# xxxupeng/stereo_toolbox

Hardware: AMD Instinct MI355X
Metric: stereo pairs/sec @ 540x960 D=192 (GwcNet_GC fwd+bwd) (higher is better)
Workload: dtype f32; 1 GPU; GwcNet_GC(maxdisp=192) train step: fwd+bwd+allreduce+Adam, 576x960 pairs (reference pad_to_2x shape), batch 1/GPU, fp32, synthetic randn inputs, deterministic filler weights; global_batch=1, parallelism=dp1, grad_sync=none (single rank: flat fp32 buffer packed, no collective), launch=eager, optimizer=torch.optim.Adam(fused=True)

## Files before the change

include/stx_hip.h:

```cpp
#ifndef STX_HIP_H
#define STX_HIP_H
#ifdef __cplusplus
extern "C" {
#endif

const char* stx_last_error(void);
const char* stx_build_info(void);
int stx_get_tuning(const char* name);
int stx_set_tuning(const char* name, int value);

int stx_cost_volume_fwd(const float* Lg, const float* Rg, int Cg, int G, const float* Lc, const float* Rc, int Cc,
                        const float* scale, float* vol, int B, int H, int W, int D, int mask_left, void* stream);
int stx_group_normalize_fwd(const float* x, float* y, int B, int C, int G, int HW, float out_scale, void* stream);
int stx_group_normalize_bwd(const float* x, const float* gy, float* gx, int B, int C, int G, int HW, float out_scale, void* stream);
int stx_cost_volume_bwd(const float* gvol, const float* Lg, const float* Rg, int Cg, int G, int Cc, float* gLg,
                        float* gRg, float* gLc, float* gRc, int B, int H, int W, int D, int mask_left, void* stream);

int stx_head_fwd(const float* cost, float* disp, float* stats, int B, int Dc, int Hc, int Wc, int D, int H, int W,
                 void* stream);
long long stx_head_bwd_workspace_floats(int B, int Dc, int H, int W);
int stx_head_bwd(const float* gdisp, const float* cost, const float* disp, const float* stats, float* gcost,
                 float* workspace, int B, int Dc, int Hc, int Wc, int D, int H, int W, void* stream);
int stx_head_fwd2(const float* cost, float* disp, float* stats, int B, int Dc, int Hc, int Wc, int D, int H, int W,
                  int align_corners, void* stream);
int stx_head_bwd2(const float* gdisp, const float* cost, const float* disp, const float* stats, float* gcost,
                  float* workspace, int B, int Dc, int Hc, int Wc, int D, int H, int W, int align_corners, void* stream);
int stx_softargmax_fwd(const float* x, float* out, int B, int D, int HW, void* stream);
int stx_argmax_fwd(const float* x, long long* out, int B, int D, int HW, void* stream);
int stx_unimodal_fwd(const float* x, float* out, int B, int D, int HW, void* stream);
int stx_dominant_modal_fwd(const float* x, float* out, int B, int D, int HW, void* stream);
int stx_modal_fwd(const float* x, float* out, float* aux, int B, int D, int HW, int kind, void* stream);
int stx_modal_bwd(const float* g, const float* out, const float* aux, float* gx, int B, int D, int HW, void* stream);
int stx_split_mode(const float* x, float* mode, unsigned char* mask, int B, int D, int HW, void* stream);
int stx_softmax_d_fwd(const float* x, float* y, int B, int D, int HW, void* stream);

long long stx_conv3d_packed_floats(int K, int N, int T);
int stx_conv3d_pack_weight(const float* w, float* wp, int A, int B, int T, int mode, void* stream);
int stx_conv3d_fwd_blocks(int Do, int Ho, int Wo);
long long stx_conv3d_fwd_stat_rows(int B, int Di, int Hi, int Wi, int Cin, int Cout, int ks, int stride);
int stx_conv3d_fwd(const float* x, const float* wp, float* out, const float* scale, const float* bias,
                   const float* residual, float* stats, int B, int Di, int Hi, int Wi, int Cin, int Cout, int ks,
                   int stride, int relu, void* stream);
int stx_deconv3d_fwd_blocks(int Di, int Hi, int Wi);
int stx_deconv3d_fwd(const float* x, const float* wp, float* out, const float* scale, const float* bias,
                     const float* residual, float* stats, int B, int Di, int Hi, int Wi, int Cin, int Cout, int Do,
                     int Ho, int Wo, int relu, void* stream);
long long stx_conv3d_wgrad_workspace_floats(int B, int Dc, int Hc, int Wc, int CF, int CC, int ks, int stride);
int stx_conv3d_wgrad(const float* fine, const float* coarse, float* dw, float* workspace, int B, int Df, int Hf, int Wf,
                     int CF, int Dc, int Hc, int Wc, int CC, int ks, int stride, void* stream);

int stx_conv3d_wgrad_bn_supported(int B, int D, int H, int W, int CF, int CC);
int stx_conv3d_wgrad_bn(const float* x, const float* gy, const float* z, const float* scale, const float* shift, const float* mean,
                        const float* invstd, const float* gamma, const float* sums, float inv_n, int act, float* dz, float* dw,
                        float* workspace, int B, int D, int H, int W, int CF, int CC, void* stream);

int stx_conv2d_supported(int Cin, int Cout);
long long stx_conv2d_stat_rows(int groups);
int stx_conv2d_fwd(const float* x, const float* w, float* out, float* stats, int B, int H, int W, int Cin, int Cout, int dgrad,
                   int groups, void* stream);

int stx_conv3d_c1_fwd(const float* x, const float* w, const float* residual, float* out, int B, int D, int H, int W,
                      int Cin, void* stream);
long long stx_conv3d_c1_wgrad_workspace_floats(int Cin);
int stx_conv3d_c1_wgrad(const float* x, const float* gy, float* dw, float* workspace, int B, int D, int H, int W,
                        int Cin, void* stream);
int stx_conv3d_c1_dgrad(const float* gy, const float* w, float* gx, int B, int D, int H, int W, int Cin, void* stream);

int stx_mish_fwd(const float* x, float* y, long long n, void* stream);
int stx_mish_bwd(const float* gy, const float* x, float* gx, long long n, void* stream);
int stx_depth_to_space(const float* y, float* out, int B, int D, int H, int W, int C, int inverse, void* stream);
int stx_gate_fwd(const float* cv, const float* att, float* out, int B, int D, long long HW, int C, void* stream);
int stx_gate_bwd(const float* g, const float* cv, const float* att, float* gcv, float* gatt, int B, int D, long long HW,
                 int C, void* stream);

int stx_concat_channels(const float* in0, const float* in1, const float* in2, const float* in3, int C0, int C1, int C2, int C3,
                        float* out, long long nvox, void* stream);
int stx_split_channels(const float* in, float* out0, float* out1, float* out2, float* out3, int C0, int C1, int C2, int C3,
                       long long nvox, void* stream);
int stx_transpose(const float* in, float* out, int N, int rows, int cols, void* stream);

int stx_dwconv_hw_fwd(const float* x, const float* w, const int* dil, float* out, int B, int D, int H, int W, int C,
                      int flip, void* stream);
long long stx_dwconv_hw_wgrad_workspace_floats(int C);
int stx_dwconv_hw_wgrad(const float* x, const float* gy, const int* dil, float* dw, float* workspace, int B, int D,
                        int H, int W, int C, void* stream);
int stx_cost_volume_scale_bwd(const float* gvol, const float* Lc, const float* Rc, float* gscale, int B, int Cc, int H,
                              int W, int D, int mask_left, void* stream);
int stx_scale_channels(const float* x, const float* s, float* out, long long nvox, int C, void* stream);
int stx_ac_volume_bwd(const float* gvol, const float* Lc, const float* Rc, const float* prob, float* gL, float* gR,
                      float* gprob, int B, int Cc, int H, int W, int D, int mask_left, void* stream);

int stx_bn_reduce_blocks(void);
int stx_bn_stats_rows(long long nvox, int C);
int stx_bn_stats(const float* z, float* partials, long long nvox, int C, int groups, void* stream);
int stx_bn_finalize(const float* partials, int nrows, int C, double count, const float* gamma, const float* beta,
                    float* running_mean, float* running_var, float momentum, float eps, float* scale, float* shift,
                    float* mean, float* invstd, void* stream);
int stx_bn_finalize_groups(const float* partials, int nrows, int C, double count, const float* gamma, const float* beta,
                           float* running_mean, float* running_var, float momentum, float eps, float* out, int groups,
                           void* stream);
int stx_bn_apply(const float* z1, const float* scale1, const float* shift1, const float* z2, const float* scale2,
                 const float* shift2, float* out, long long nvox, int C, int relu, int groups, void* stream);
int stx_bn_bwd_reduce(const float* gy, const float* y, const float* z1, const float* mean1, const float* invstd1,
                      const float* z2, const float* mean2, const float* invstd2, float* partials, float* sums,
                      long long nvox, int C, int relu, void* stream);
int stx_bn_bwd_apply(const float* gy, const float* y, const float* z1, const float* mean1, const float* invstd1,
                     const float* gamma1, const float* z2, const float* mean2, const float* invstd2,
                     const float* gamma2, const float* sums, float* dz1, float* dz2, float* gout, long long nvox, int C,
                     int relu, void* stream);
int stx_bn_bwd_reduce2(const float* gy, const float* y, const float* z1, const float* mean1, const float* invstd1,
                       const float* z2, const float* mean2, const float* invstd2, const float* scale1,
                       const float* shift1, const float* scale2, const float* shift2, float* partials, float* sums,
                       long long nvox, int C, int relu, int groups, void* stream);
int stx_bn_bwd_apply2(const float* gy, const float* y, const float* z1, const float* mean1, const float* invstd1,
                      const float* gamma1, const float* z2, const float* mean2, const float* invstd2,
                      const float* gamma2, const float* scale1, const float* shift1, const float* scale2,
                      const float* shift2, const float* sums, float* dz1, float* dz2, float* gout, long long nvox,
                      int C, int relu, int groups, void* stream);

int stx_pad_normalize_u8(const unsigned char* img, float* out, int B, int H, int W, int Hp, int Wp, int top,
                         const float* mean3, const float* std3, void* stream);

int stx_sampled_volume_fwd(const float* Lg, const float* Rg, int Cg, int G, const float* Lc, const float* Rc, int Cc,
                           const float* samples, float* vol, int B, int H, int W, int S, int CTp, void* stream);
int stx_sampled_volume_bwd(const float* gvol, const float* Lg, const float* Rg, int Cg, int G, int Cc,
                           const float* samples, float* gLg, float* gRg, float* gLc, float* gRc, int B, int H, int W,
                           int S, int CTp, void* stream);

int stx_warp_fwd(const float* x, const float* disp, float* out, int B, int C, int H, int W, void* stream);
int stx_warp_bwd(const float* gout, const float* x, const float* disp, float* gx, float* gdisp, int B, int C, int H, int W,
                 void* stream);
int stx_corr_volume_fwd(const float* ref, const float* tgt, float* vol, int B, int C, int H, int W, int maxdisp, int groups,
                        void* stream);
int stx_corr_volume_bwd(const float* gvol, const float* ref, const float* tgt, float* gref, float* gtgt, int B, int C, int H,
                        int W, int maxdisp, int groups, void* stream);
int stx_disparity_variance_fwd(const float* x, const float* disp, const float* samples, float* out, int B, int D, int HW,
                               void* stream);
int stx_disparity_variance_bwd(const float* g, const float* x, const float* disp, const float* samples, float* gx, float* gdisp,
                               float* gsamples, int B, int D, int HW, void* stream);

long long stx_geo_pyramid_floats(long long rows, int len, int C, int levels);
int stx_geo_corr_fwd(const float* fmap1, const float* fmap2, float* cpyr, int B, int C, int H, int W1, int W2, int levels,
                     void* stream);
int stx_geo_corr_bwd(const float* gcpyr, const float* fmap1, const float* fmap2, float* gfmap1, float* gfmap2, int B, int C, int H,
                     int W1, int W2, int levels, void* stream);
int stx_geo_pyramid_fwd(const float* vol, float* gpyr, int B, int D, int H, int W, int C, int levels, void* stream);
int stx_geo_pyramid_bwd(const float* ggpyr, float* gvol, int B, int D, int H, int W, int C, int levels, void* stream);
int stx_geo_lookup_fwd(const float* gpyr, const float* cpyr, const float* disp, const float* coords, float* out, int B, int H,
                       int W, int D, int C, int W2, int levels, int radius, void* stream);
int stx_geo_lookup_bwd(const float* gout, const float* disp, const float* coords, float* ggpyr, float* gcpyr, int B, int H, int W,
                       int D, int C, int W2, int levels, int radius, void* stream);
int stx_context_upsample_fwd(const float* disp_low, const float* up_weights, float* out, int B, int h, int w, void* stream);
int stx_context_upsample_bwd(const float* g, const float* disp_low, const float* up_weights, float* gdisp, float* gweights, int B,
                             int h, int w, void* stream);

long long stx_corr1d_pyramid_floats(long long rows, int W2, int levels);
int stx_corr1d_pyramid_fwd(const float* fmap1, const float* fmap2, float* cpyr, int B, int C, int H, int W1, int W2, int levels,
                           float scale, void* stream);
int stx_corr1d_pyramid_bwd(const float* gcpyr, const float* fmap1, const float* fmap2, float* gfmap1, float* gfmap2, int B, int C,
                           int H, int W1, int W2, int levels, float scale, void* stream);
int stx_corr1d_lookup_fwd(const float* cpyr, const float* base, const float* disp, const float* jobs, int njobs, float* out, int B,
                          int H, int W1, int W2, int levels, void* stream);
int stx_corr1d_lookup_bwd(const float* gout, const float* base, const float* disp, const float* jobs, int njobs, float* gcpyr,
                          int B, int H, int W1, int W2, int levels, void* stream);

int stx_allpairs_estimates_fwd(const float* vol, int which, float* disp_l, float* conf_l, float* disp_r, float* conf_r, float* stats,
                               int B, int H, int W1, int W2, void* stream);
int stx_allpairs_estimates_bwd(const float* g_disp_l, const float* g_conf_l, const float* g_disp_r, const float* g_conf_r,
                               const float* vol, const float* stats, float* gvol, int B, int H, int W1, int W2, void* stream);
int stx_corr1d_volume_pyramid_fwd(const float* vol, const float* tdisp, const float* tconf, float atten, float* cpyr, int B, int H,
                                  int W1, int W2, int levels, void* stream);
int stx_corr1d_volume_pyramid_bwd(const float* gcpyr, const float* tdisp, const float* tconf, float atten, float* gvol, int B, int H,
                                  int W1, int W2, int levels, void* stream);
int stx_truncate_mask_fwd(const float* disp, const float* conf, int has_th, float conf_th, float atten, float* mask, int B, int H,
                          int W, void* stream);

int stx_photo_warp_fwd(const float* right, const float* disp, float* warped, float* valid, int B, int C, int H, int W, void* stream);
int stx_photo_warp_bwd(const float* gwarped, const float* right, const float* disp, float* gdisp, int B, int C, int H, int W,
                       void* stream);
int stx_ssim_fwd(const float* x, const float* y, float* out, int B, int C, int H, int W, int window, void* stream);
long long stx_ssim_bwd_workspace_floats(int B, int C, int H, int W);
int stx_ssim_bwd(const float* g_out, const float* x, const float* y, float* gx, float* gy, float* workspace, int B, int C, int H, int W,
                 int window, void* stream);
int stx_photometric_fwd(const float* left, const float* right, const float* disp, double ssim_weight, int enable_mask, float* loss,
                        int B, int C, int H, int W, void* stream);
long long stx_photometric_bwd_workspace_floats(int B, int C, int H, int W);
int stx_photometric_bwd(const float* gloss, const float* left, const float* right, const float* disp, double ssim_weight,
                        int enable_mask, float* gdisp, float* workspace, int B, int C, int H, int W, void* stream);
int stx_auto_mask_fwd(const float* left, const float* right, const float* disp, int denorm, unsigned char* mask, int B, int C, int H,
                      int W, void* stream);
long long stx_smoothness_workspace_floats(int B, int H, int W);
int stx_smoothness_fwd(const float* disp, const float* img, float* out, float* stats, float* workspace, int B, int C, int H, int W,
                       void* stream);
int stx_smoothness_bwd(const float* gout, const float* disp, const float* img, const float* stats, float* gdisp, int B, int C, int H,
                       int W, void* stream);

#ifdef __cplusplus
}
#endif
#endif
```

stereo_toolbox_amd/_capi.py:

```python
import ctypes
import os
import threading

import torch

_P = ctypes.c_void_p
_I = ctypes.c_int
_F = ctypes.c_float
_L = ctypes.c_longlong

SIGNATURES = {
    "stx_get_tuning": [ctypes.c_char_p],
    "stx_set_tuning": [ctypes.c_char_p, _I],
    "stx_cost_volume_fwd": [_P, _P, _I, _I, _P, _P, _I, _P, _P, _I, _I, _I, _I, _I, _P],
    "stx_cost_volume_bwd": [_P, _P, _P, _I, _I, _I, _P, _P, _P, _P, _I, _I, _I, _I, _I, _P],
    "stx_group_normalize_fwd": [_P, _P, _I, _I, _I, _I, _F, _P],
    "stx_group_normalize_bwd": [_P, _P, _P, _I, _I, _I, _I, _F, _P],
    "stx_head_fwd": [_P, _P, _P, _I, _I, _I, _I, _I, _I, _I, _P],
    "stx_head_bwd_workspace_floats": [_I, _I, _I, _I],
    "stx_head_bwd": [_P, _P, _P, _P, _P, _P, _I, _I, _I, _I, _I, _I, _I, _P],
    "stx_head_fwd2": [_P, _P, _P, _I, _I, _I, _I, _I, _I, _I, _I, _P],
    "stx_head_bwd2": [_P, _P, _P, _P, _P, _P, _I, _I, _I, _I, _I, _I, _I, _I, _P],
    "stx_softargmax_fwd": [_P, _P, _I, _I, _I, _P],
    "stx_argmax_fwd": [_P, _P, _I, _I, _I, _P],
    "stx_softmax_d_fwd": [_P, _P, _I, _I, _I, _P],
    "stx_unimodal_fwd": [_P, _P, _I, _I, _I, _P],
    "stx_dominant_modal_fwd": [_P, _P, _I, _I, _I, _P],
    "stx_modal_fwd": [_P, _P, _P, _I, _I, _I, _I, _P],
    "stx_modal_bwd": [_P, _P, _P, _P, _I, _I, _I, _P],
    "stx_split_mode": [_P, _P, _P, _I, _I, _I, _P],
    "stx_conv3d_packed_floats": [_I, _I, _I],
    "stx_conv3d_pack_weight": [_P, _P, _I, _I, _I, _I, _P],
    "stx_conv3d_fwd_blocks": [_I, _I, _I],
    "stx_conv3d_fwd_stat_rows": [_I, _I, _I, _I, _I, _I, _I, _I],
    "stx_deconv3d_fwd_blocks": [_I, _I, _I],
    "stx_conv3d_fwd": [_P, _P, _P, _P, _P, _P, _P, _I, _I, _I, _I, _I, _I, _I, _I, _I, _P],
    "stx_deconv3d_fwd": [_P, _P, _P, _P, _P, _P, _P, _I, _I, _I, _I, _I, _I, _I, _I, _I, _I, _P],
    "stx_conv3d_wgrad_workspace_floats": [_I, _I, _I, _I, _I, _I, _I, _I],
    "stx_conv3d_wgrad": [_P, _P, _P, _P, _I, _I, _I, _I, _I, _I, _I, _I, _I, _I, _I, _P],
    "stx_conv3d_wgrad_bn_supported": [_I, _I, _I, _I, _I, _I],
    "stx_conv3d_wgrad_bn": [_P] * 9 + [_F, _I, _P, _P, _P, _I, _I, _I, _I, _I, _I, _P],
    "stx_conv2d_supported": [_I, _I],
    "stx_conv2d_stat_rows": [_I],
    "stx_conv2d_fwd": [_P, _P, _P, _P, _I, _I, _I, _I, _I, _I, _I, _P],
    "stx_conv3d_c1_fwd": [_P, _P, _P, _P, _I, _I, _I, _I, _I, _P],
    "stx_conv3d_c1_wgrad_workspace_floats": [_I],
    "stx_conv3d_c1_wgrad": [_P, _P, _P, _P, _I, _I, _I, _I, _I, _P],
    "stx_conv3d_c1_dgrad": [_P, _P, _P, _I, _I, _I, _I, _I, _P],
    "stx_mish_fwd": [_P, _P, _L, _P],
    "stx_mish_bwd": [_P, _P, _P, _L, _P],
    "stx_depth_to_space": [_P, _P, _I, _I, _I, _I, _I, _I, _P],
    "stx_gate_fwd": [_P, _P, _P, _I, _I, _L, _I, _P],
    "stx_gate_bwd": [_P, _P, _P, _P, _P, _I, _I, _L, _I, _P],
    "stx_concat_channels": [_P, _P, _P, _P, _I, _I, _I, _I, _P, _L, _P],
    "stx_split_channels": [_P, _P, _P, _P, _P, _I, _I, _I, _I, _L, _P],
    "stx_transpose": [_P, _P, _I, _I, _I, _P],
    "stx_dwconv_hw_fwd": [_P, _P, _P, _P, _I, _I, _I, _I, _I, _I, _P],
    "stx_dwconv_hw_wgrad_workspace_floats": [_I],
    "stx_dwconv_hw_wgrad": [_P, _P, _P, _P, _P, _I, _I, _I, _I, _I, _P],
    "stx_cost_volume_scale_bwd": [_P, _P, _P, _P, _I, _I, _I, _I, _I, _I, _P],
    "stx_scale_channels": [_P, _P, _P, _L, _I, _P],
    "stx_ac_volume_bwd": [_P, _P, _P, _P, _P, _P, _P, _I, _I, _I, _I, _I, _I, _P],
    "stx_pad_normalize_u8": [_P, _P, _I, _I, _I, _I, _I, _I, _P, _P, _P],
    "stx_warp_fwd": [_P, _P, _P, _I, _I, _I, _I, _P],
    "stx_warp_bwd": [_P, _P, _P, _P, _P, _I, _I, _I, _I, _P],
    "stx_corr_volume_fwd": [_P, _P, _P, _I, _I, _I, _I, _I, _I, _P],
    "stx_corr_volume_bwd": [_P, _P, _P, _P, _P, _I, _I, _I, _I, _I, _I, _P],
    "stx_disparity_variance_fwd": [_P, _P, _P, _P, _I, _I, _I, _P],
    "stx_disparity_variance_bwd": [_P, _P, _P, _P, _P, _P, _P, _I, _I, _I, _P],
    "stx_sampled_volume_fwd": [_P, _P, _I, _I, _P, _P, _I, _P, _P, _I, _I, _I, _I, _I, _P],
    "stx_sampled_volume_bwd": [_P, _P, _P, _I, _I, _I, _P, _P, _P, _P, _P, _I, _I, _I, _I, _I, _P],
    "stx_geo_pyramid_floats": [_L, _I, _I, _I],
    "stx_geo_corr_fwd": [_P, _P, _P, _I, _I, _I, _I, _I, _I, _P],
    "stx_geo_corr_bwd": [_P, _P, _P, _P, _P, _I, _I, _I, _I, _I, _I, _P],
    "stx_geo_pyramid_fwd": [_P, _P, _I, _I, _I, _I, _I, _I, _P],
    "stx_geo_pyramid_bwd": [_P, _P, _I, _I, _I, _I, _I, _I, _P],
    "stx_geo_lookup_fwd": [_P, _P, _P, _P, _P, _I, _I, _I, _I, _I, _I, _I, _I, _P],
    "stx_geo_lookup_bwd": [_P, _P, _P, _P, _P, _I, _I, _I, _I, _I, _I, _I, _I, _P],
    "stx_context_upsample_fwd": [_P, _P, _P, _I, _I, _I, _P],
    "stx_context_upsample_bwd": [_P, _P, _P, _P, _P, _I, _I, _I, _P],
    "stx_corr1d_pyramid_floats": [_L, _I, _I],
    "stx_corr1d_pyramid_fwd": [_P, _P, _P, _I, _I, _I, _I, _I, _I, _F, _P],
    "stx_corr1d_pyramid_bwd": [_P, _P, _P, _P, _P, _I, _I, _I, _I, _I, _I, _F, _P],
    "stx_corr1d_lookup_fwd": [_P, _P, _P, _P, _I, _P, _I, _I, _I, _I, _I, _P],
    "stx_corr1d_lookup_bwd": [_P, _P, _P, _P, _I, _P, _I, _I, _I, _I, _I, _P],
    "stx_allpairs_estimates_fwd": [_P, _I, _P, _P, _P, _P, _P, _I, _I, _I, _I, _P],
    "stx_allpairs_estimates_bwd": [_P, _P, _P, _P, _P, _P, _P, _I, _I, _I, _I, _P],
    "stx_corr1d_volume_pyramid_fwd": [_P, _P, _P, _F, _P, _I, _I, _I, _I, _I, _P],
    "stx_corr1d_volume_pyramid_bwd": [_P, _P, _P, _F, _P, _I, _I, _I, _I, _I, _P],
    "stx_truncate_mask_fwd": [_P, _P, _I, _F, _F, _P, _I, _I, _I, _P],
    "stx_photo_warp_fwd": [_P, _P, _P, _P, _I, _I, _I, _I, _P],
    "stx_photo_warp_bwd": [_P, _P, _P, _P, _I, _I, _I, _I, _P],
    "stx_ssim_fwd": [_P, _P, _P, _I, _I, _I, _I, _I, _P],
    "stx_ssim_bwd_workspace_floats": [_I, _I, _I, _I],
    "stx_ssim_bwd": [_P, _P, _P, _P, _P, _P, _I, _I, _I, _I, _I, _P],
    "stx_photometric_fwd": [_P, _P, _P, ctypes.c_double, _I, _P, _I, _I, _I, _I, _P],
    "stx_photometric_bwd_workspace_floats": [_I, _I, _I, _I],
    "stx_photometric_bwd": [_P, _P, _P, _P, ctypes.c_double, _I, _P, _P, _I, _I, _I, _I, _P],
    "stx_auto_mask_fwd": [_P, _P, _P, _I, _P, _I, _I, _I, _I, _P],
    "stx_smoothness_workspace_floats": [_I, _I, _I],
    "stx_smoothness_fwd": [_P, _P, _P, _P, _P, _I, _I, _I, _I, _P],
    "stx_smoothness_bwd": [_P, _P, _P, _P, _P, _I, _I, _I, _I, _P],
    "stx_bn_reduce_blocks": [],
    "stx_bn_stats_rows": [_L, _I],
    "stx_bn_stats": [_P, _P, _L, _I, _I, _P],
    "stx_bn_finalize": [_P, _I, _I, ctypes.c_double, _P, _P, _P, _P, _F, _F, _P, _P, _P, _P, _P],
    "stx_bn_finalize_groups": [_P, _I, _I, ctypes.c_double, _P, _P, _P, _P, _F, _F, _P, _I, _P],
    "stx_bn_apply": [_P, _P, _P, _P, _P, _P, _P, _L, _I, _I, _I, _P],
    "stx_bn_bwd_reduce": [_P, _P, _P, _P, _P, _P, _P, _P, _P, _P, _L, _I, _I, _P],
    "stx_bn_bwd_apply": [_P, _P, _P, _P, _P, _P, _P, _P, _P, _P, _P, _P, _P, _P, _L, _I, _I, _P],
    "stx_bn_bwd_reduce2": [_P] * 14 + [_L, _I, _I, _I, _P],
    "stx_bn_bwd_apply2": [_P] * 18 + [_L, _I, _I, _I, _P],
}
_RET_CHARP = ("stx_last_error", "stx_build_info")


class StxError(RuntimeError):
    pass


class StxLib:

    def __init__(self, path):
        if not os.path.exists(path):
            raise StxError(
                f"HIP library not found: {path}. Build it with `python -m stereo_toolbox_amd.build` "
                "(hipcc, gfx950). There is no CPU fallback for the cost-volume hot path.")
        self.path = path
        self._dll = ctypes.CDLL(path)
        for name in _RET_CHARP:
            fn = getattr(self._dll, name)
            fn.restype = ctypes.c_char_p
            fn.argtypes = []
        self._fns = {}
        for name, argtypes in SIGNATURES.items():
            fn = getattr(self._dll, name, None)
            if fn is None:
                continue
            fn.restype = ctypes.c_longlong if name.endswith(("_floats", "_stat_rows")) else _I
            fn.argtypes = argtypes
            self._fns[name] = fn

    def has(self, name):
        return name in self._fns

    def build_info(self):
        return self._dll.stx_build_info().decode()

    def get_tuning(self, name):
        return self._fns["stx_get_tuning"](name.encode())

    def set_tuning(self, name, value):
        old = self.get_tuning(name)
        if old < 0 or self._fns["stx_set_tuning"](name.encode(), int(value)) != 0:
            raise StxError(f"unknown tuning switch {name}")
        return old

    def raw(self, name):
        return self._fns[name]

    def call(self, name, *args):
        fn = self._fns.get(name)
        if fn is None:
            raise StxError(f"{self.path} does not export {name}")
        rc = fn(*args)
        if rc != 0:
            raise StxError(f"{name} failed ({rc}): {self._dll.stx_last_error().decode()}")


_LIB = None
_LOCK = threading.Lock()
LIB_PATH = os.environ.get("STX_HIP_LIB") or os.path.join(os.path.dirname(os.path.abspath(__file__)), "lib", "libstx_hip.so")


def get_lib():
    global _LIB
    if _LIB is None:
        with _LOCK:
            if _LIB is None:
                _LIB = StxLib(LIB_PATH)
    return _LIB
```

stereo_toolbox_amd/csrc/bn.hip:

```cpp
#include "stx_common.h"
#include <stdlib.h>

namespace {

constexpr int BN_THREADS = 256;
constexpr int BN_RED_BLOCKS = 1024;

__device__ __forceinline__ double bn_block_sum(double v, double* red, int tid) {
    red[tid] = v;
    __syncthreads();
    for (int s = BN_THREADS / 2; s > 0; s >>= 1) {
        if (tid < s) red[tid] += red[tid + s];
        __syncthreads();
    }
    const double r = red[0];
    __syncthreads();
    return r;
}

__global__ __launch_bounds__(BN_THREADS) void bn_finalize_kernel(
    const float* __restrict__ partials, int nrows, int C, double count, const float* __restrict__ gamma,
    const float* __restrict__ beta, float* __restrict__ running_mean, float* __restrict__ running_var,
    float momentum, float eps, float* __restrict__ scale, float* __restrict__ shift, float* __restrict__ mean_out,
    float* __restrict__ invstd_out, int groups) {
// ... 257 lines not shown
        const size_t go = (size_t)blockIdx.y * nquads * 4, gc = (size_t)blockIdx.y * C;
        gy += go; z1 += go; dz1 += go; mean1 += gc; invstd1 += gc; sums += 3 * gc;
        if (y) y += go;
        if (z2) z2 += go;
        if (dz2) dz2 += go;
        if (gout) gout += go;
        if (mean2) { mean2 += gc; invstd2 += gc; }
        if (sc1) { sc1 += gc; sh1 += gc; }
        if (sc2) { sc2 += gc; sh2 += gc; }
    }
    const bool has2 = z2 && mean2 && dz2;
    const bool remask = relu && !y;
    for (size_t i = (size_t)blockIdx.x * BN_THREADS + threadIdx.x; i < nquads; i += (size_t)gridDim.x * BN_THREADS) {
        const int c = (int)(i % CQ) * 4;
        float4 g = stx_ld4(gy + i * 4);
        const float4 a = stx_ld4(z1 + i * 4);
        float4 a2v = make_float4(0.f, 0.f, 0.f, 0.f);
        if (has2) a2v = stx_ld4(z2 + i * 4);
        if (relu) {
            float4 yy;
            if (remask) {
                const float4 p1 = stx_ld4(sc1 + c), q1 = stx_ld4(sh1 + c);
                yy.x = fmaf(a.x, p1.x, q1.x); yy.y = fmaf(a.y, p1.y, q1.y); yy.z = fmaf(a.z, p1.z, q1.z); yy.w = fmaf(a.w, p1.w, q1.w);
                if (has2) {
                    const float4 p2 = stx_ld4(sc2 + c), q2 = stx_ld4(sh2 + c);
                    yy.x += fmaf(a2v.x, p2.x, q2.x); yy.y += fmaf(a2v.y, p2.y, q2.y);
                    yy.z += fmaf(a2v.z, p2.z, q2.z); yy.w += fmaf(a2v.w, p2.w, q2.w);
                }
            } else {
                yy = stx_ld4(y + i * 4);
            }
            g.x = stx_act_bwd(g.x, yy.x, relu); g.y = stx_act_bwd(g.y, yy.y, relu);
            g.z = stx_act_bwd(g.z, yy.z, relu); g.w = stx_act_bwd(g.w, yy.w, relu);
        }
        if (gout) stx_st4(gout + i * 4, g);
        const float4 sg = stx_ld4(sums + c);
        {
            const float4 m = stx_ld4(mean1 + c), is = stx_ld4(invstd1 + c);
            const float4 gm = gamma1 ? stx_ld4(gamma1 + c) : make_float4(1.f, 1.f, 1.f, 1.f);
            const float4 sx = stx_ld4(sums + C + c);
            float4 d;
            d.x = gm.x * is.x * (g.x - sg.x * inv_n - (a.x - m.x) * is.x * sx.x * inv_n);
            d.y = gm.y * is.y * (g.y - sg.y * inv_n - (a.y - m.y) * is.y * sx.y * inv_n);
            d.z = gm.z * is.z * (g.z - sg.z * inv_n - (a.z - m.z) * is.z * sx.z * inv_n);
            d.w = gm.w * is.w * (g.w - sg.w * inv_n - (a.w - m.w) * is.w * sx.w * inv_n);
            stx_st4(dz1 + i * 4, d);
        }
        if (has2) {
            const float4 a = a2v, m = stx_ld4(mean2 + c), is = stx_ld4(invstd2 + c);
            const float4 gm = gamma2 ? stx_ld4(gamma2 + c) : make_float4(1.f, 1.f, 1.f, 1.f);
            const float4 sx = stx_ld4(sums + 2 * C + c);
            float4 d;
            d.x = gm.x * is.x * (g.x - sg.x * inv_n - (a.x - m.x) * is.x * sx.x * inv_n);
            d.y = gm.y * is.y * (g.y - sg.y * inv_n - (a.y - m.y) * is.y * sx.y * inv_n);
            d.z = gm.z * is.z * (g.z - sg.z * inv_n - (a.z - m.z) * is.z * sx.z * inv_n);
            d.w = gm.w * is.w * (g.w - sg.w * inv_n - (a.w - m.w) * is.w * sx.w * inv_n);
            stx_st4(dz2 + i * 4, d);
        }
    }
}

int bn_grid(size_t nquads) {
    size_t g = (nquads + BN_THREADS - 1) / BN_THREADS;
    return (int)(g > 4096 ? 4096 : (g < 1 ? 1 : g));
}

}

extern "C" int stx_bn_reduce_blocks(void) {
    stx_begin(); return BN_RED_BLOCKS; }

static int bn_finalize_launch(const float* partials, int nrows, int C, double count, const float* gamma, const float* beta,
                              float* running_mean, float* running_var, float momentum, float eps, float* scale, float* shift,
                              float* mean, float* invstd, int groups, void* stream) {
    if (C % 4 == 0 && nrows >= 256)
        hipLaunchKernelGGL(bn_finalize4_kernel, dim3(C / 4), dim3(BN_FIN_THREADS), 0, (hipStream_t)stream, partials, nrows, C,
                           count, gamma, beta, running_mean, running_var, momentum, eps, scale, shift, mean, invstd, groups);
    else
        hipLaunchKernelGGL(bn_finalize_kernel, dim3(C), dim3(BN_THREADS), 0, (hipStream_t)stream, partials, nrows, C, count,
                           gamma, beta, running_mean, running_var, momentum, eps, scale, shift, mean, invstd, groups);
    return stx_check_launch("bn_finalize");
}

extern "C" int stx_bn_finalize(const float* partials, int nrows, int C, double count, const float* gamma,
                               const float* beta, float* running_mean, float* running_var, float momentum, float eps,
                               float* scale, float* shift, float* mean, float* invstd, void* stream) {
    stx_begin();
    STX_REQUIRE(partials && nrows > 0 && C > 0 && count > 0 && scale && shift && mean && invstd, "bn_finalize: bad args");
    return bn_finalize_launch(partials, nrows, C, count, gamma, beta, running_mean, running_var, momentum, eps, scale, shift,
                              mean, invstd, 1, stream);
}

extern "C" int stx_bn_finalize_groups(const float* partials, int nrows, int C, double count, const float* gamma,
                                      const float* beta, float* running_mean, float* running_var, float momentum, float eps,
                                      float* out, int groups, void* stream) {
    stx_begin();
    STX_REQUIRE(partials && nrows > 0 && C > 0 && count > 0 && out && groups >= 1, "bn_finalize_groups: bad args");
    const size_t gc = (size_t)groups * C;
    return bn_finalize_launch(partials, nrows, C, count, gamma, beta, running_mean, running_var, momentum, eps, out, out + gc,
                              out + 2 * gc, out + 3 * gc, groups, stream);
}

extern "C" int stx_bn_stats_rows(long long nvox, int C) {
    stx_begin();
    if (C < 4 || C % 4 != 0 || C / 4 > BN_THREADS || nvox < 1) return 0;
    const long long vpb = BN_THREADS / (C / 4);
    const long long g = (nvox + 4 * vpb - 1) / (4 * vpb);
    return (int)(g > 256 ? 256 : (g < 1 ? 1 : g));
}

extern "C" int stx_bn_stats(const float* z, float* partials, long long nvox, int C, int groups, void* stream) {
    stx_begin();
    STX_REQUIRE(z && partials && nvox > 0 && groups >= 1 && groups <= 65535, "bn_stats: bad args");
    STX_REQUIRE(C >= 4 && C % 4 == 0 && C / 4 <= BN_THREADS, "bn_stats: C=%d unsupported (a multiple of 4, at most 1024)", C);
    hipLaunchKernelGGL(bn_stats_kernel, dim3(stx_bn_stats_rows(nvox, C), groups), dim3(BN_THREADS), 0, (hipStream_t)stream, z,
                       partials, (size_t)nvox, C);
    return stx_check_launch("bn_stats");
}

extern "C" int stx_bn_apply(const float* z1, const float* scale1, const float* shift1, const float* z2,
                            const float* scale2, const float* shift2, float* out, long long nvox, int C, int relu,
                            int groups, void* stream) {
    stx_begin();
    STX_REQUIRE(z1 && scale1 && shift1 && out && nvox > 0 && C > 0 && C % 4 == 0, "bn_apply: bad args (C=%d)", C);
    STX_REQUIRE(!scale2 || (z2 && shift2), "bn_apply: second affine needs z2 and shift2");
    STX_REQUIRE(groups >= 1 && groups <= 65535, "bn_apply: groups=%d", groups);
    const size_t nquads = (size_t)nvox * (C / 4);
    hipLaunchKernelGGL(bn_apply_kernel, dim3(bn_grid(nquads), groups), dim3(BN_THREADS), 0, (hipStream_t)stream, z1, scale1,
                       shift1, z2, scale2, shift2, out, nquads, C / 4, relu);
    return stx_check_launch("bn_apply");
}

extern "C" int stx_bn_bwd_reduce2(const float* gy, const float* y, const float* z1, const float* mean1,
                                  const float* invstd1, const float* z2, const float* mean2, const float* invstd2,
                                  const float* scale1, const float* shift1, const float* scale2, const float* shift2,
                                  float* partials, float* sums, long long nvox, int C, int relu, int groups, void* stream) {
    stx_begin();
    STX_REQUIRE(gy && z1 && mean1 && invstd1 && partials && sums && nvox > 0, "bn_bwd_reduce: null operand");
    STX_REQUIRE(groups >= 1 && groups <= 65535, "bn_bwd_reduce: groups=%d", groups);
    STX_REQUIRE(C >= 4 && C % 4 == 0 && C / 4 <= BN_THREADS, "bn_bwd_reduce: C=%d unsupported (a multiple of 4, at most 1024)", C);
    STX_REQUIRE(!relu || y || (scale1 && shift1 && (!(z2 && mean2) || (scale2 && shift2))),
                "bn_bwd_reduce: the relu mask needs y or the forward pass's scale / shift vectors");
    STX_REQUIRE(relu != 2 || !y, "bn_bwd_reduce: Mish (activation code 2) differentiates the pre-activation value: pass y = NULL and the scale / shift vectors");
    hipStream_t st = (hipStream_t)stream;
    const int nblk = ((long long)nvox * C <= (9ll << 19)) ? BN_RED_BLOCKS / 4 : BN_RED_BLOCKS;
    hipLaunchKernelGGL(bn_bwd_reduce_kernel, dim3(nblk, groups), dim3(BN_THREADS), 0, st, gy, y, z1, mean1, invstd1,
                       z2, mean2, invstd2, scale1, shift1, scale2, shift2, partials, (size_t)nvox, C, relu);
    int rc = stx_check_launch("bn_bwd_reduce");
    if (rc) return rc;
    hipLaunchKernelGGL(bn_colsum_kernel, dim3(3 * C), dim3(BN_THREADS), 0, st, partials, nblk, 3 * C, sums, groups);
    return stx_check_launch("bn_colsum");
}

extern "C" int stx_bn_bwd_apply2(const float* gy, const float* y, const float* z1, const float* mean1,
                                 const float* invstd1, const float* gamma1, const float* z2, const float* mean2,
                                 const float* invstd2, const float* gamma2, const float* scale1, const float* shift1,
                                 const float* scale2, const float* shift2, const float* sums, float* dz1, float* dz2,
                                 float* gout, long long nvox, int C, int relu, int groups, void* stream) {
    stx_begin();
    STX_REQUIRE(gy && z1 && mean1 && invstd1 && sums && dz1 && nvox > 0 && C % 4 == 0, "bn_bwd_apply: bad args");
    STX_REQUIRE(groups >= 1 && groups <= 65535, "bn_bwd_apply: groups=%d", groups);
    STX_REQUIRE(!relu || y || (scale1 && shift1 && (!(z2 && mean2 && dz2) || (scale2 && shift2))),
                "bn_bwd_apply: the relu mask needs y or the forward pass's scale / shift vectors");
    STX_REQUIRE(relu != 2 || !y, "bn_bwd_apply: Mish (activation code 2) differentiates the pre-activation value: pass y = NULL and the scale / shift vectors");
    const size_t nquads = (size_t)nvox * (C / 4);
    hipLaunchKernelGGL(bn_bwd_apply_kernel, dim3(bn_grid(nquads), groups), dim3(BN_THREADS), 0, (hipStream_t)stream, gy, y, z1,
                       mean1, invstd1, gamma1, z2, mean2, invstd2, gamma2, scale1, shift1, scale2, shift2, sums, dz1, dz2,
                       gout, nquads, C, relu, (float)(1.0 / (double)nvox));
    return stx_check_launch("bn_bwd_apply");
}

extern "C" int stx_bn_bwd_reduce(const float* gy, const float* y, const float* z1, const float* mean1,
                                 const float* invstd1, const float* z2, const float* mean2, const float* invstd2,
                                 float* partials, float* sums, long long nvox, int C, int relu, void* stream) {
    return stx_bn_bwd_reduce2(gy, y, z1, mean1, invstd1, z2, mean2, invstd2, nullptr, nullptr, nullptr, nullptr, partials,
                              sums, nvox, C, relu, 1, stream);
}

extern "C" int stx_bn_bwd_apply(const float* gy, const float* y, const float* z1, const float* mean1,
                                const float* invstd1, const float* gamma1, const float* z2, const float* mean2,
                                const float* invstd2, const float* gamma2, const float* sums, float* dz1, float* dz2,
                                float* gout, long long nvox, int C, int relu, void* stream) {
    return stx_bn_bwd_apply2(gy, y, z1, mean1, invstd1, gamma1, z2, mean2, invstd2, gamma2, nullptr, nullptr, nullptr,
                             nullptr, sums, dz1, dz2, gout, nvox, C, relu, 1, stream);
}
```

stereo_toolbox_amd/csrc/conv3d.hip:

```cpp
#include "stx_common.h"
#include <stdlib.h>

namespace {

constexpr int CONV_THREADS = 256;

struct ConvArgs {
    const float* x;
    const float* wp;
    float* out;
    const float* scale;
    const float* bias;
    const float* residual;
    float* stats;
    int Di, Hi, Wi, Cin;
    int Do, Ho, Wo, Cout;
    int relu;
    int nDt, nHt, nWt;
};

__device__ __forceinline__ int xcd_remap(int bid, int nblk) {
    const int q = nblk >> 3, r = nblk & 7;
    const int xcd = bid & 7, k = bid >> 3;
    const int base = (xcd < r) ? xcd * (q + 1) : r * (q + 1) + (xcd - r) * q;
// ... 290 lines not shown
#pragma unroll
                    for (int nt = 0; nt < NT; ++nt) bcur[q][nt] = bnxt[q][nt];
#pragma unroll
                    for (int m = 0; m < MT; ++m) acur[q][m] = anxt[q][m];
                }
            }
        }
    }

    float s1[NTW], s2[NTW];
#pragma unroll
    for (int nt = 0; nt < NTW; ++nt) { s1[nt] = 0.f; s2[nt] = 0.f; }
#pragma unroll
    for (int m = 0; m < MT; ++m) {
        const int mtile = wrow * MT + m;
        const int od = od0 + mtile / TH, oh = oh0 + mtile % TH;
        int nrows = (od < a.Do && oh < a.Ho) ? (a.Wo - ow0) : 0;
        nrows = nrows > 32 ? 32 : nrows;
        const size_t vox0 = (((size_t)b * a.Do + od) * a.Ho + oh) * a.Wo + ow0;
#pragma unroll
        for (int nt = 0; nt < NTW; ++nt) {
            const int n = (wcol * NTW + nt) * 32 + i;
            const float sc = (a.scale && n < a.Cout) ? a.scale[n] : 1.f;
            const float bs = (a.bias && n < a.Cout) ? a.bias[n] : 0.f;
            conv_epilogue_block(a, acc[m][nt], vox0, 1, nrows, n, sc, bs, lane, s1[nt], s2[nt]);
        }
    }
    if (a.stats) conv_write_stats<NT, WN>(a, s1, s2, tile, tid, (size_t)blockIdx.y * gridDim.x + blockIdx.x);
}

template <int KS, int S, int TD, int TH, int NT, int CK, int WN = 1>
__global__ __launch_bounds__(CONV_THREADS, (CK == 8 && S == 1) ? 2 : 1) void conv3d_pgemm_kernel(ConvArgs a, int ntiles_total) {
    constexpr int PAD = KS / 2;
    constexpr int ED = (TD - 1) * S + KS, EH = (TH - 1) * S + KS, EW = 31 * S + KS;
    constexpr int EWH = (EW + 1) / 2;
    constexpr int EWS = (S == 2) ? 2 * EWH : EW;
    constexpr int MT = TD * TH / 4 * WN;
    constexpr int NTW = NT / WN;
    constexpr int VS = CK + 4;
    constexpr int NF4 = CK / 4;
    constexpr int NE = ED * EH * EW * NF4;
    constexpr int NST = (NE + CONV_THREADS - 1) / CONV_THREADS;
    constexpr int T = KS * KS * KS, NQC = CK / 8;
    static_assert(TD * TH % 4 == 0, "tile must split over 4 waves");
    static_assert(NT % WN == 0 && 4 % WN == 0, "wave grid");
    STX_DYN_SMEM(smem);
    float* tile = reinterpret_cast<float*>(smem);

    const int tid = threadIdx.x, lane = tid & 63, wave = __builtin_amdgcn_readfirstlane(tid >> 6);
    const int i = lane & 31, half = lane >> 5;
    const int NQ = a.Cin / 8, nchunk = a.Cin / CK;
    const int tiles_per_b = a.nDt * a.nHt * a.nWt;
    const long long wg = xcd_remap(blockIdx.x, gridDim.x);
    const int t_lo = __builtin_amdgcn_readfirstlane((int)((long long)ntiles_total * wg / gridDim.x));
    const int t_hi = __builtin_amdgcn_readfirstlane((int)((long long)ntiles_total * (wg + 1) / gridDim.x));

    const int wrow = wave / WN, wcol = wave % WN;
    int abase[MT];
#pragma unroll
    for (int m = 0; m < MT; ++m) {
        const int mtile = wrow * MT + m;
        const int td = mtile / TH, th = mtile % TH;
        abase[m] = ((td * S * EH + th * S) * EWS + i) * VS + 4 * half;
    }
    float4 stg[NST];
    auto tile_origin = [&](int t, int& b, int& od0, int& oh0, int& ow0) {
        b = t / tiles_per_b;
        const int r = t - b * tiles_per_b;
        const int wt = r % a.nWt, ht = (r / a.nWt) % a.nHt, dt = r / (a.nWt * a.nHt);
        od0 = dt * TD; oh0 = ht * TH; ow0 = wt * 32;
    };
    using HM = HaloMap<ED, EH, EW, NF4>;
    HM hm;
    hm.init(tid, a.Hi, a.Wi, a.Cin);
    auto load_item = [&](int t, int c0) {
        int b, od0, oh0, ow0;
        tile_origin(t, b, od0, oh0, ow0);
        const int id0 = od0 * S - PAD, ih0 = oh0 * S - PAD, iw0 = ow0 * S - PAD;
        unsigned vo[NST];
        hm.offsets(id0, ih0, iw0, a.Di, a.Hi, a.Wi, vo);
        const stx_bufrsrc xrs = HM::rsrc(a.x, b, id0, ih0, iw0, a.Di, a.Hi, a.Wi, a.Cin);
#pragma unroll
        for (int k = 0; k < NST; ++k) stg[k] = stx_buf_ld4(xrs, vo[k], (unsigned)c0 * 4u);
    };
    auto store_item = [&]() {
#pragma unroll
        for (int k = 0; k < NST; ++k) {
            const int e = tid + k * CONV_THREADS;
            const int v = e / NF4, f = e - v * NF4;
            const int wx = v % EW, hy = (v / EW) % EH, dz = v / (EW * EH);
            const int slot = (S == 2) ? (wx & 1) * EWH + (wx >> 1) : wx;
            if (e < NE) stx_st4(tile + ((dz * EH + hy) * EWS + slot) * VS + 4 * f, stg[k]);
        }
    };

    float s1[NTW], s2[NTW];
#pragma unroll
    for (int nt = 0; nt < NTW; ++nt) { s1[nt] = 0.f; s2[nt] = 0.f; }
    f32x16 acc[MT][NTW];
    float4 bring[3][NQC][NTW];
    static_assert(KS == 3, "the pipelined kernel serves 3x3x3 only");
    const float* wbase = a.wp + (size_t)lane * 4 + (size_t)wcol * NTW * 256;
    if (t_lo < t_hi) {
        load_item(t_lo, 0);
        conv_ring_prologue<NTW, NQC, NT>(wbase, NQ, bring);
    }
    for (int t = t_lo; t < t_hi; ++t) {
#pragma unroll
        for (int m = 0; m < MT; ++m)
#pragma unroll
            for (int nt = 0; nt < NTW; ++nt) acc[m][nt] = zero16();
        for (int ch = 0; ch < nchunk; ++ch) {
            __syncthreads();
            store_item();
            __syncthreads();
            {
                const int nch = ch + 1 < nchunk ? ch + 1 : 0;
                const int ntl = ch + 1 < nchunk ? t : t + 1;
                if (ntl < t_hi) load_item(ntl, nch * CK);
            }
            const float* wq = wbase + (size_t)(ch * (CK / 8)) * NT * 256;
            const float* wq_next = ch + 1 < nchunk ? wq + (size_t)NQC * NT * 256 : (t + 1 < t_hi ? wbase : nullptr);
            conv_chunk_taps27<S, MT, NTW, NQC, EH, EWS, EWH, VS, NT>(tile, abase, wq, wq_next, NQ, acc, bring);
        }
        int b, od0, oh0, ow0;
        tile_origin(t, b, od0, oh0, ow0);
#pragma unroll
        for (int m = 0; m < MT; ++m) {
            const int mtile = wrow * MT + m;
            const int od = od0 + mtile / TH, oh = oh0 + mtile % TH;
            int nrows = (od < a.Do && oh < a.Ho) ? (a.Wo - ow0) : 0;
            nrows = nrows > 32 ? 32 : nrows;
            const size_t vox0 = (((size_t)b * a.Do + od) * a.Ho + oh) * a.Wo + ow0;
#pragma unroll
            for (int nt = 0; nt < NTW; ++nt) {
                const int n = (wcol * NTW + nt) * 32 + i;
                const float sc = (a.scale && n < a.Cout) ? a.scale[n] : 1.f;
                const float bs = (a.bias && n < a.Cout) ? a.bias[n] : 0.f;
                conv_epilogue_block(a, acc[m][nt], vox0, 1, nrows, n, sc, bs, lane, s1[nt], s2[nt]);
            }
        }
    }
    if (a.stats) conv_write_stats<NT, WN>(a, s1, s2, tile, tid, (size_t)blockIdx.x);
}

struct MarchArgs {
    ConvArgs c;
    int ncols;
    int ablate;
    int xs, xo;
    int os, oo, ncout;
    int wq_total, wq_off, wnt_total, wnt_off;
    const float* acc_in;
};

constexpr int MW2_MW = 16, MW2_R = 2, MW2_TH = 8, MW2_EH = 10, MW2_EW = 18, MW2_VS = 36;
constexpr int MW2_SLOT = MW2_EH * MW2_EW * MW2_VS;
constexpr int MW2_NF4 = (MW2_EH * MW2_EW * 8 + 255) / 256;
constexpr int MW2_WFLOATS = 27 * 4 * 256;

template <int BS, int EPI = 1>
__global__ __launch_bounds__(256) void conv3d_marchw_kernel(MarchArgs ma) {
    const ConvArgs& a = ma.c;
    STX_DYN_SMEM(smem);
    float* wl = reinterpret_cast<float*>(smem);
    float* planes = wl + MW2_WFLOATS;
    const int tid = threadIdx.x, lane = tid & 63, wave = tid >> 6;
    const int i = lane & 31, half = lane >> 5;
    const int th = wave;
    auto n_lane = [&]() { return i; };

    for (int e = tid; e < MW2_WFLOATS / 4; e += 256) {
        const int tq = e >> 6, l4 = e & 63;
        const int tap = tq >> 2, q = tq & 3;
        const size_t src = (((size_t)tap * ma.wq_total + ma.wq_off + q) * ma.wnt_total + ma.wnt_off) * 256 + 4 * l4;
        stx_st4(wl + 4 * e, stx_ld4(a.wp + src));
    }

    int b = 0, oh0 = 0, ow0 = 0;
    const long long units = (long long)ma.ncols * a.Do;
    const long long wg = xcd_remap(blockIdx.x, gridDim.x);
    int u = __builtin_amdgcn_readfirstlane((int)(units * wg / gridDim.x));
    const int u_end = __builtin_amdgcn_readfirstlane((int)(units * (wg + 1) / gridDim.x));

    float4 stg[MW2_NF4];
    unsigned svoff[MW2_NF4], ovoff = 0, ovalid = 0;
    const unsigned xplane_bytes = (unsigned)a.Hi * (unsigned)a.Wi * (unsigned)ma.xs * 4u;
    const unsigned oplane_bytes = (unsigned)a.Ho * (unsigned)a.Wo * (unsigned)ma.os * 4u;
    auto column_offsets = [&]() {
#pragma unroll
        for (int k = 0; k < MW2_NF4; ++k) {
            const int idx = tid + k * 256;
            const int v = idx >> 3, f = idx & 7;
            const int wx = v % MW2_EW, hy = v / MW2_EW;
            const int gh = oh0 - 1 + hy, gw = ow0 - 1 + wx;
            const bool ok = v < MW2_EH * MW2_EW && gh >= 0 && gh < a.Hi && gw >= 0 && gw < a.Wi;
            svoff[k] = ok ? (unsigned)(((gh * a.Wi + gw) * ma.xs + ma.xo + 4 * f) * 4) : STX_BUF_OOB;
        }
        const int ohb = oh0 + th * MW2_R, owb = ow0 + 4 * half;
        ovoff = (unsigned)((((ohb * a.Wo + owb) * ma.os) + ma.oo + n_lane()) * 4);
        ovalid = 0;
#pragma unroll
        for (int r = 0; r < 16; ++r) {
            const int c = (r & 3) + 8 * ((r >> 2) & 1), dh = r >> 3;
            if (ohb + dh < a.Ho && owb + c < a.Wo && n_lane() < ma.ncout) ovalid |= 1u << r;
        }
    };
    auto load_plane = [&](int pd, bool on) {
        const bool in = on && pd >= 0 && pd < a.Di;
        const stx_bufrsrc rs = stx_make_rsrc(a.x + ((size_t)b * a.Di + (in ? pd : 0)) * a.Hi * a.Wi * ma.xs, in ? xplane_bytes : 0u);
#pragma unroll
        for (int k = 0; k < MW2_NF4; ++k) stg[k] = stx_buf_ld4(rs, svoff[k], 0u);
    };
    auto store_plane = [&](float* buf) {
#pragma unroll
        for (int k = 0; k < MW2_NF4; ++k) {
            const int idx = tid + k * 256;
            const int v = idx >> 3, f = idx & 7;
            if (v < MW2_EH * MW2_EW) stx_st4(buf + v * MW2_VS + 4 * f, stg[k]);
        }
    };

    float s1 = 0.f, s2 = 0.f;
    const int abase = ((th * MW2_R + i / MW2_MW) * MW2_EW + i % MW2_MW) * MW2_VS + 4 * half;
    const float* wlane = wl + lane * 4;
    const int n = i;
    const float sc = (a.scale && n < ma.ncout) ? a.scale[ma.oo + n] : 1.f;
    const float bs = (a.bias && n < ma.ncout) ? a.bias[ma.oo + n] : 0.f;

    auto emit_row = [&](const f32x16& done0, const f32x16& done1, const f32x16& done, int r, int dprev) {
        const int row = (r & 3) + 8 * (r >> 2) + 4 * half;
        const int oh = oh0 + th * MW2_R + row / MW2_MW, ow = ow0 + row % MW2_MW;
        if (oh < a.Ho && ow < a.Wo && n < ma.ncout && ma.ablate != 2) {
            const size_t idx = ((((size_t)b * a.Do + dprev) * a.Ho + oh) * a.Wo + ow) * ma.os + ma.oo + n;
            float v = BS ? (done0[r] + done1[r]) + done[r] : done[r];
            if (ma.acc_in) v += ma.acc_in[idx];
            s1 += v;
            s2 = fmaf(v, v, s2);
            v = fmaf(v, sc, bs);
            if (a.residual) v += a.residual[idx];
            v = stx_act(v, a.relu);
            a.out[idx] = v;
        }
    };
    const bool relu_on = a.relu == 1;
    float accp[16];
    auto load_partials = [&](unsigned vmask, const stx_bufrsrc& rs) {
#pragma unroll
        for (int r = 0; r < 16; ++r) {
            const int c = (r & 3) + 8 * ((r >> 2) & 1), dh = r >> 3;
            accp[r] = stx_buf_ld1(rs, ((vmask >> r) & 1u) ? ovoff : STX_BUF_OOB, (unsigned)((dh * a.Wo + c) * ma.os * 4));
        }
    };
    auto emit_row_plain = [&](const f32x16& done0, const f32x16& done1, const f32x16& done, int r, unsigned vmask,
                              const stx_bufrsrc& ors) {
        const int c = (r & 3) + 8 * ((r >> 2) & 1), dh = r >> 3;
        const bool ok = EPI == 5 ? vmask != 0u : (bool)((vmask >> r) & 1u);
        float v = BS ? (done0[r] + done1[r]) + done[r] : done[r];
        if (EPI == 2) v += accp[r];
        v = ok ? v : 0.f;
        s1 += v;
        s2 = fmaf(v, v, s2);
        if (EPI != 4 && EPI != 5) {
            v = fmaf(v, sc, bs);
            if (EPI == 3) v += accp[r];
            const float vr = fmaxf(v, 0.f);
            v = relu_on ? vr : v;
        }
        stx_buf_st1(ors, (EPI == 5 || ok) ? ovoff : STX_BUF_OOB, (unsigned)((dh * a.Wo + c) * ma.os * 4), v);
    };

    auto tap_plane = [&](const float* pbuf, int kd, f32x16& acc, bool fresh, bool with_epi, const f32x16& done0, const f32x16& done1,
                         const f32x16& done, int dprev, int epi0, unsigned vmask, const stx_bufrsrc& ors) {
        float4 av[2][4], bv[2][4];
        auto load_tap = [&](int t9, int buf) {
            const int kh = t9 / 3, kw = t9 % 3;
            const float* sl = pbuf + abase + (kh * MW2_EW + kw) * MW2_VS;
            const float* wt = wlane + (kd * 9 + t9) * 1024;
#pragma unroll
            for (int q = 0; q < 4; ++q) {
                av[buf][q] = stx_ld4(sl + 8 * q);
                bv[buf][q] = stx_ld4(wt + q * 256);
            }
        };
        load_tap(0, 0);
#pragma unroll
        for (int t9 = 0; t9 < 9; ++t9) {
            if (t9 + 1 < 9) load_tap(t9 + 1, (t9 + 1) & 1);
            const int cb = t9 & 1;
#pragma unroll
            for (int q = 0; q < 4; ++q) {
                acc = __builtin_amdgcn_mfma_f32_32x32x2f32(av[cb][q].x, bv[cb][q].x, (fresh && t9 == 0 && q == 0) ? zero16() : acc, 0, 0, 0);
                acc = __builtin_amdgcn_mfma_f32_32x32x2f32(av[cb][q].y, bv[cb][q].y, acc, 0, 0, 0);
                acc = __builtin_amdgcn_mfma_f32_32x32x2f32(av[cb][q].z, bv[cb][q].z, acc, 0, 0, 0);
                acc = __builtin_amdgcn_mfma_f32_32x32x2f32(av[cb][q].w, bv[cb][q].w, acc, 0, 0, 0);
            }
            const int r = epi0 + t9;
            if (EPI != 1) {
                if (epi0 >= 0 && r < 16) emit_row_plain(done0, done1, done, r, vmask, ors);
            }
            if (t9 + 1 < 9) {
#pragma unroll
                for (int g = 0; g < 8; ++g) {
                    STX_SCHED_GROUP(0x008, 2);
                    STX_SCHED_GROUP(0x100, 1);
                    if (EPI != 1) STX_SCHED_GROUP(0x002, 2);
                }
            }
            if (EPI == 1 && with_epi && r < 16) emit_row(done0, done1, done, r, dprev);
            STX_SCHED_BARRIER();
        }
    };
    auto step = [&](int p, int d_lo, int d_hi, const float* pbuf, float* nbuf, bool stage, f32x16& pA, f32x16& pB,
                    f32x16& pC, f32x16& pD, f32x16& pE, f32x16& pF) {
        const bool live = p >= 0 && p < a.Di;
        const bool vOld = p - 1 >= d_lo && p - 1 < d_hi, vMid = p >= d_lo && p < d_hi, vNew = p + 1 >= d_lo && p + 1 < d_hi;
        const bool st_on = vOld && ma.ablate != 2;
        const unsigned vmask = st_on ? ovalid : 0u;
        const stx_bufrsrc ors = stx_make_rsrc(a.out + ((size_t)b * a.Do + (st_on ? p - 1 : 0)) * a.Ho * a.Wo * ma.os,
                                              st_on ? oplane_bytes : 0u);
        if (EPI == 2) load_partials(vmask, ors);
        if (EPI == 3)
            load_partials(vmask, stx_make_rsrc(a.residual + ((size_t)b * a.Do + (st_on ? p - 1 : 0)) * a.Ho * a.Wo * ma.os,
                                               st_on ? oplane_bytes : 0u));
        if (live && vOld) tap_plane(pbuf, 2, pC, BS != 0, false, pA, pB, pC, 0, -1, 0u, ors);
        else if (BS) pC = zero16();
        if (stage) store_plane(nbuf);
        if (live && vMid) tap_plane(pbuf, 1, pE, BS != 0, vOld, pA, pB, pC, p - 1, 0, vmask, ors);
        else if (BS) pE = zero16();
        if (!(live && vMid) && vOld) {
#pragma unroll
            for (int r = 0; r < 9; ++r) {
                if (EPI != 1) emit_row_plain(pA, pB, pC, r, vmask, ors);
                else emit_row(pA, pB, pC, r, p - 1);
            }
        }
        if (live && vNew) tap_plane(pbuf, 0, pF, true, vOld, pA, pB, pC, p - 1, 9, vmask, ors);
        else pF = zero16();
        if (!(live && vNew) && vOld) {
#pragma unroll
            for (int r = 9; r < 16; ++r) {
                if (EPI != 1) emit_row_plain(pA, pB, pC, r, vmask, ors);
                else emit_row(pA, pB, pC, r, p - 1);
            }
        }
    };

    __syncthreads();
    f32x16 r0 = zero16(), r1 = zero16(), r2 = zero16(), r3 = zero16(), r4 = zero16(), r5 = zero16();
    while (u < u_end) {
        int d_lo, d_hi;
        {
            const int col = u / a.Do;
            d_lo = u - col * a.Do;
            const int left = u_end - u;
            d_hi = (a.Do - d_lo < left) ? a.Do : d_lo + left;
            u += d_hi - d_lo;
            const int wt = col % a.nWt, ht = (col / a.nWt) % a.nHt;
            b = col / (a.nWt * a.nHt);
            oh0 = ht * MW2_TH; ow0 = wt * MW2_MW;
        }
        column_offsets();
        __syncthreads();
        load_plane(d_lo - 1, true);
        store_plane(planes);
        __syncthreads();
        int par = 0;
        auto advance = [&](int p, f32x16& pA, f32x16& pB, f32x16& pC, f32x16& pD, f32x16& pE, f32x16& pF) {
            const bool stage = p + 1 <= d_hi && ma.ablate != 1;
            load_plane(p + 1, stage);
            step(p, d_lo, d_hi, planes + par * MW2_SLOT, planes + (par ^ 1) * MW2_SLOT, stage, pA, pB, pC, pD, pE, pF);
            __syncthreads();
            par ^= 1;
        };
        if (BS) {
            for (int p = d_lo - 1; p <= d_hi; p += 3) {
                advance(p, r0, r1, r2, r3, r4, r5);
                if (p + 1 <= d_hi) advance(p + 1, r3, r4, r1, r5, r2, r0);
                if (p + 2 <= d_hi) advance(p + 2, r5, r2, r4, r0, r1, r3);
            }
        } else {
            for (int p = d_lo - 1; p <= d_hi; p += 3) {
                advance(p, r3, r4, r0, r5, r1, r2);
                if (p + 1 <= d_hi) advance(p + 1, r3, r4, r1, r5, r2, r0);
                if (p + 2 <= d_hi) advance(p + 2, r3, r4, r2, r5, r0, r1);
            }
        }
    }
    if (a.stats) {
        s1 += __shfl_xor(s1, 32);
        s2 += __shfl_xor(s2, 32);
        __syncthreads();
        if (lane < 32) {
            planes[(wave * 32 + lane) * 2 + 0] = s1;
            planes[(wave * 32 + lane) * 2 + 1] = s2;
        }
        __syncthreads();
        if (tid < 32 && tid < ma.ncout) {
            float t1 = 0.f, t2 = 0.f;
#pragma unroll
            for (int w = 0; w < 4; ++w) {
                t1 += planes[(w * 32 + tid) * 2 + 0];
                t2 += planes[(w * 32 + tid) * 2 + 1];
            }
            const size_t slab = (size_t)blockIdx.x;
            a.stats[slab * 2 * a.Cout + ma.oo + tid] = t1;
            a.stats[slab * 2 * a.Cout + a.Cout + ma.oo + tid] = t2;
        }
    }
}

struct DcEntries { int n; int slot[14], tap[14], dd[14], dh[14], dw[14]; };
constexpr DcEntries dc_entries(int cset) {
    DcEntries e{};
    const int tab[2][4] = {{7, 4, 2, 0}, {3, 5, 6, 1}};
    int n = 0;
    for (int c = 0; c < 4; ++c) {
        const int cls = tab[cset][c];
        const int pd = (cls >> 2) & 1, ph = (cls >> 1) & 1, pw = cls & 1;
        for (int sd = 0; sd <= pd; ++sd)
            for (int sh = 0; sh <= ph; ++sh)
                for (int sw = 0; sw <= pw; ++sw) {
                    const int kd = pd ? (sd ? 2 : 0) : 1, kh = ph ? (sh ? 2 : 0) : 1, kw = pw ? (sw ? 2 : 0) : 1;
                    e.slot[n] = c;
                    e.tap[n] = (kd * 3 + kh) * 3 + kw;
                    e.dd[n] = pd ? (sd ? 0 : 1) : 0;
                    e.dh[n] = ph ? (sh ? 0 : 1) : 0;
                    e.dw[n] = pw ? (sw ? 0 : 1) : 0;
                    ++n;
                }
    }
    e.n = n;
    return e;
}

template <int CSET, int NT, int CK>
__device__ __forceinline__ void deconv_chunk_taps(const float* atile, const float* wq, int NQ, f32x16 (&acc)[4][NT]) {
    constexpr DcEntries E = dc_entries(CSET);
    constexpr int EH = 3, EW = 33, VS = CK + 4, QS = CK / 8;
    float4 bv[2][QS][NT], av[2][QS];
    auto load_b = [&](int t, int buf) {
        const float* wtap = wq + (size_t)E.tap[t] * NQ * NT * 256;
#pragma unroll
        for (int q = 0; q < QS; ++q)
#pragma unroll
            for (int nt = 0; nt < NT; ++nt) bv[buf][q][nt] = stx_ld4(wtap + (size_t)(q * NT + nt) * 256);
    };
    auto load_a = [&](int t, int buf) {
        const int toff = ((E.dd[t] * EH + E.dh[t]) * EW + E.dw[t]) * VS;
#pragma unroll
        for (int q = 0; q < QS; ++q) av[buf][q] = stx_ld4(atile + toff + q * 8);
    };
    load_b(0, 0);
#pragma unroll
    for (int t = 0; t < E.n; ++t) {
        if (t + 1 < E.n) load_b(t + 1, (t + 1) & 1);
        STX_SCHED_BARRIER();
        load_a(t, t & 1);
#pragma unroll
        for (int q = 0; q < QS; ++q) {
            const float4 a4 = av[t & 1][q];
#pragma unroll
            for (int nt = 0; nt < NT; ++nt) {
                const float4 b = bv[t & 1][q][nt];
                acc[E.slot[t]][nt] = __builtin_amdgcn_mfma_f32_32x32x2f32(a4.x, b.x, acc[E.slot[t]][nt], 0, 0, 0);
                acc[E.slot[t]][nt] = __builtin_amdgcn_mfma_f32_32x32x2f32(a4.y, b.y, acc[E.slot[t]][nt], 0, 0, 0);
                acc[E.slot[t]][nt] = __builtin_amdgcn_mfma_f32_32x32x2f32(a4.z, b.z, acc[E.slot[t]][nt], 0, 0, 0);
                acc[E.slot[t]][nt] = __builtin_amdgcn_mfma_f32_32x32x2f32(a4.w, b.w, acc[E.slot[t]][nt], 0, 0, 0);
            }
        }
        STX_SCHED_BARRIER();
    }
}

template <int NT, int CK>
__global__ __launch_bounds__(CONV_THREADS, NT == 1 ? 3 : 2) void deconv3d_igemm_kernel(ConvArgs a) {
    constexpr int TH = 2;
    constexpr int ED = 2, EH = TH + 1, EW = 33;
    constexpr int VS = CK + 4, NF4 = CK / 4;
    STX_DYN_SMEM(smem);
    float* tile = reinterpret_cast<float*>(smem);

    const int tid = threadIdx.x, lane = tid & 63;
    const int wave = NT == 1 ? __builtin_amdgcn_readfirstlane(tid >> 6) : (tid >> 6);
    const int i = lane & 31, half = lane >> 5;
    const int bid = xcd_remap(blockIdx.x, gridDim.x), b = blockIdx.y;
    const int wt = bid % a.nWt, ht = (bid / a.nWt) % a.nHt, dt = bid / (a.nWt * a.nHt);
    const int md0 = dt, mh0 = ht * TH, mw0 = wt * 32;
    const int NQ = a.Cin / 8;
    const int th = wave >> 1, cset = wave & 1;
    const int cls_tab[2][4] = {{7, 4, 2, 0}, {3, 5, 6, 1}};

    f32x16 acc[4][NT];
#pragma unroll
    for (int c = 0; c < 4; ++c)
#pragma unroll
        for (int nt = 0; nt < NT; ++nt) acc[c][nt] = zero16();
    const int abase = ((th * EW) + i) * VS + 4 * half;
// ... 182 lines not shown
            }
#pragma unroll
        for (int k = 0; k < NCL; ++k) {
            const int idx = tid + k * NTHR;
            if (idx < NV * 8) stx_st4(ctile + (idx >> 3) * 32 + 4 * (idx & 7), sc[k]);
        }
    };

    if (PIPE && (int)blockIdx.x < a.ntiles) load_tile(blockIdx.x, a.ablate != 1);
    for (int tile = blockIdx.x; tile < a.ntiles; tile += gridDim.x) {
        if (!PIPE) load_tile(tile, a.ablate != 1);
        __syncthreads();
        if (a.ablate != 1) store_tile();
        __syncthreads();
        if (PIPE) {
            const int nxt = tile + (int)gridDim.x;
            load_tile(nxt < a.ntiles ? nxt : tile, nxt < a.ntiles && a.ablate != 1);
        }
        if (a.ablate == 2) continue;
        if (KS == 1) {
            for (int p = wave; p < NV / 2; p += NW) {
                const int v = 2 * p + half;
                const int lw = v % TW, lh = v / TW;
                const float bv = ctile[v * 32 + i];
                const float av = ftile[(lh * EWS + lw) * 32 + i];
                acc[0] = __builtin_amdgcn_mfma_f32_32x32x2f32(av, bv, acc[0], 0, 0, 0);
            }
        } else {
            int toff[NTAP];
#pragma unroll
            for (int t = 0; t < NTAP; ++t) {
                const int tap = (t * NW + wave < T) ? t * NW + wave : 0;
                const int kd = tap / 9, kh = (tap / 3) % 3, kw = tap % 3;
                toff[t] = (S == 2) ? ((kd * EH + kh) * EWS + (kw & 1) * EWH + (kw >> 1)) * 32
                                   : ((kd * EH + kh) * EWS + kw) * 32;
            }
            float av[2][NTAP], bv[2];
            auto load_pair = [&](int p, int buf) {
                const int v = 2 * p + half;
                const int lw = v % TW, lh = v / TW;
                const int vb = ((lh * S) * EWS + lw) * 32 + i;
                bv[buf] = ctile[v * 32 + i];
#pragma unroll
                for (int t = 0; t < NTAP; ++t) av[buf][t] = ftile[vb + toff[t]];
            };
            auto mma_pair = [&](int buf) {
#pragma unroll
                for (int t = 0; t < NTAP; ++t)
                    if (t * NW + wave < T) acc[t] = __builtin_amdgcn_mfma_f32_32x32x2f32(av[buf][t], bv[buf], acc[t], 0, 0, 0);
            };
            load_pair(0, 0);
            for (int p = 0; p < NV / 2; p += 2) {
                load_pair(p + 1, 1);
                STX_SCHED_BARRIER();
                mma_pair(0);
                STX_SCHED_BARRIER();
                load_pair((p + 2 < NV / 2) ? p + 2 : 0, 0);
                STX_SCHED_BARRIER();
                mma_pair(1);
                STX_SCHED_BARRIER();
            }
        }
    }
    constexpr int ROWS = (KS == 1) ? NW : T;
    float* dst = a.slab + ((size_t)blockIdx.y * gridDim.x + blockIdx.x) * ROWS * 1024;
#pragma unroll
    for (int t = 0; t < NTAP; ++t) {
        const int row = (KS == 1) ? wave : t * NW + wave;
        if (KS == 1 ? (t == 0) : (row < T)) {
#pragma unroll
            for (int r = 0; r < 16; ++r) {
                const int cf = (r & 3) + 8 * (r >> 2) + 4 * half;
                dst[(size_t)row * 1024 + cf * 32 + i] = acc[t][r];
            }
        }
    }
}

__global__ __launch_bounds__(CONV_THREADS) void conv3d_wgrad_reduce4_kernel(const float* __restrict__ slab,
                                                                            float* __restrict__ dw, int CF, int CC,
                                                                            int T, int nchunks, int rows_per_chunk) {
    __shared__ float red[16][64];
    const int lane = threadIdx.x & 63, wave = threadIdx.x >> 6;
    const int part = wave * 4 + (lane >> 4), ql = lane & 15;
    const int idx0 = blockIdx.x * 64 + ql * 4;
    const int cc_l = idx0 & 31, cf_l = (idx0 >> 5) & 31;
    const int tap = (idx0 >> 10) % T, pair = (idx0 >> 10) / T;
    const float* p;
    size_t stride;
    int n;
    if (rows_per_chunk == T) {
        p = slab + ((size_t)pair * nchunks * T + tap) * 1024 + cf_l * 32 + cc_l;
        stride = (size_t)T * 1024; n = nchunks;
    } else {
        p = slab + ((size_t)pair * nchunks * rows_per_chunk) * 1024 + cf_l * 32 + cc_l;
        stride = 1024; n = nchunks * rows_per_chunk;
    }
    float4 s = make_float4(0.f, 0.f, 0.f, 0.f);
#pragma unroll 4
    for (int c = part; c < n; c += 16) {
        const float4 v = stx_ld4(p + (size_t)c * stride);
        s.x += v.x; s.y += v.y; s.z += v.z; s.w += v.w;
    }
    stx_st4(&red[part][ql * 4], s);
    __syncthreads();
    if (wave == 0) {
        float t = 0.f;
#pragma unroll
        for (int k = 0; k < 16; ++k) t += red[k][lane];
        const int idx = blockIdx.x * 64 + lane;
        const int cc = idx & 31, cf = (idx >> 5) & 31;
        const int ncf = CF / 32, cfb = pair % ncf, ccb = pair / ncf;
        dw[((size_t)(ccb * 32 + cc) * CF + cfb * 32 + cf) * T + tap] = t;
    }
}

template <typename K, typename... Args>
int launch_with_lds(K kernel, dim3 grid, size_t lds, hipStream_t st, Args... args) {
    if (int rc = stx_lds_require((const void*)kernel, lds, "conv3d")) return rc;
    static const bool report = getenv("STX_REPORT_OCCUPANCY") != nullptr;
    if (report) {
        int nb = -1;
        hipOccupancyMaxActiveBlocksPerMultiprocessor(&nb, (const void*)kernel, CONV_THREADS, lds);
        fprintf(stderr, "[stx] conv3d launch: grid %u x %u, %zu B LDS, %d workgroups per CU\n", grid.x, grid.y, lds, nb);
    }
    hipLaunchKernelGGL(kernel, grid, dim3(CONV_THREADS), lds, st, args...);
    return 0;
}

constexpr int CONV_TD = 2, CONV_TH = 2;

template <int KS, int S>
size_t conv_lds_bytes(int CK, int NT) {
    const int ED = (CONV_TD - 1) * S + KS, EH = (CONV_TH - 1) * S + KS, EW = 31 * S + KS;
    const int EWS = (S == 2) ? 2 * ((EW + 1) / 2) : EW;
    size_t t = (size_t)ED * EH * EWS * (CK + 4) * 4;
    size_t red = (size_t)4 * NT * 32 * 2 * 4;
    return t > red ? t : red;
}

template <int S>
void (*pgemm_kernel(int wn))(ConvArgs, int) {
    return wn == 4 ? conv3d_pgemm_kernel<3, S, CONV_TD, CONV_TH, 4, 8, 4>
         : wn == 2 ? conv3d_pgemm_kernel<3, S, CONV_TD, CONV_TH, 4, 8, 2> : conv3d_pgemm_kernel<3, S, CONV_TD, CONV_TH, 4, 8>;
}

void (*march_kernel(int bs, int epi))(MarchArgs) {
    switch (epi) {
    case 0: return bs ? conv3d_marchw_kernel<1, 0> : conv3d_marchw_kernel<0, 0>;
    case 2: return bs ? conv3d_marchw_kernel<1, 2> : conv3d_marchw_kernel<0, 2>;
    case 3: return bs ? conv3d_marchw_kernel<1, 3> : conv3d_marchw_kernel<0, 3>;
    case 4: return bs ? conv3d_marchw_kernel<1, 4> : conv3d_marchw_kernel<0, 4>;
    case 5: return bs ? conv3d_marchw_kernel<1, 5> : conv3d_marchw_kernel<0, 5>;
    default: return bs ? conv3d_marchw_kernel<1, 1> : conv3d_marchw_kernel<0, 1>;
    }
}

template <int KS, int S>
int conv_dispatch(const ConvArgs& a, int NT, int CK, dim3 grid, hipStream_t st) {
    const size_t lds = conv_lds_bytes<KS, S>(CK, NT);
#define CONV_CASE(NT_, CK_)                                                                                        \
    if (NT == NT_ && CK == CK_)                                                                                    \
        return launch_with_lds(conv3d_igemm_kernel<KS, S, CONV_TD, CONV_TH, NT_, CK_>, grid, lds, st, a);
    if constexpr (KS == 1) { CONV_CASE(1, 32) CONV_CASE(2, 32) CONV_CASE(4, 32) }
    if constexpr (KS == 3) {
        if (NT == 2 && CK == 8 && stx_tune(STX_TUNE_CONV_WN) >= 2)
            return launch_with_lds(conv3d_igemm_kernel<KS, S, CONV_TD, CONV_TH, 2, 8, 4, 2>, grid, lds, st, a);
    }
    CONV_CASE(1, 8) CONV_CASE(2, 8) CONV_CASE(4, 8)
#undef CONV_CASE
    return stx_set_error(STX_ERR_ARG, "conv3d: unsupported NT=%d CK=%d", NT, CK);
}

}

static int conv_pick_ck(int Cin, int ks) { return (ks == 1 && Cin % 32 == 0) ? 32 : 8; }
static int conv_nt(int N) { return N <= 32 ? 1 : (N <= 64 ? 2 : 4); }

extern "C" long long stx_conv3d_packed_floats(int K, int N, int T) {
    return (long long)T * (K / 8) * conv_nt(N) * 256;
}

extern "C" int stx_conv3d_pack_weight(const float* w, float* wp, int A, int Bd, int T, int mode, void* stream) {
    stx_begin();
    STX_REQUIRE(w && wp && A > 0 && Bd > 0 && (T == 1 || T == 27), "conv3d_pack_weight: bad args");
    STX_REQUIRE(mode >= 0 && mode <= 2, "conv3d_pack_weight: mode %d", mode);
    const int K = (mode == 0) ? Bd : A, N = (mode == 0) ? A : Bd;
    STX_REQUIRE(K % 8 == 0 && N <= 128, "conv3d_pack_weight: GEMM-K channels (%d) must be a multiple of 8, N (%d) <= 128", K, N);
    const int NT = conv_nt(N);
    const size_t total = (size_t)T * (K / 8) * NT * 256;
    hipLaunchKernelGGL(conv3d_pack_kernel, dim3((unsigned)((total + CONV_THREADS - 1) / CONV_THREADS)),
                       dim3(CONV_THREADS), 0, (hipStream_t)stream, w, wp, A, Bd, T, mode, K, N, NT, total);
    return stx_check_launch("conv3d_pack_weight");
}

static int march_wgs(long long units) {
    long long g = 256;
    if (g > units / 3) g = units / 3;
    return g < 1 ? 1 : (int)g;
}

extern "C" int stx_conv3d_fwd_blocks(int Do, int Ho, int Wo) {
    stx_begin();
    const int a = stx_cdiv(Do, CONV_TD) * stx_cdiv(Ho, CONV_TH) * stx_cdiv(Wo, 32);
    const int m = Do * stx_cdiv(Ho, 4) * stx_cdiv(Wo, 32);
    const int m16 = Do * stx_cdiv(Ho, 8) * stx_cdiv(Wo, 16);
    return a > m ? (a > m16 ? a : m16) : (m > m16 ? m : m16);
}
extern "C" int stx_deconv3d_fwd_blocks(int Di, int Hi, int Wi) {
    stx_begin(); return Di * stx_cdiv(Hi, 2) * stx_cdiv(Wi, 32); }

struct ConvPlan { int kind; int march_wgs; int pgrid; long long rows; };
static int persistent_grid(size_t lds, long long ntiles) {
    int per_cu = (int)(STX_LDS_MAX / (lds + 512));
    per_cu = per_cu < 1 ? 1 : (per_cu > 2 ? 2 : per_cu);
    const long long g = 256ll * per_cu;
    return (int)(g > ntiles ? ntiles : g);
}
static ConvPlan conv_plan(int B, int Di, int Hi, int Wi, int Cin, int Cout, int ks, int stride) {
    const int pad = ks / 2;
    const int Do = (Di + 2 * pad - ks) / stride + 1, Ho = (Hi + 2 * pad - ks) / stride + 1, Wo = (Wi + 2 * pad - ks) / stride + 1;
    ConvPlan p{2, 0, 0, 0};
    if (ks == 3 && stride == 1 && ((Cin == 32 && Cout <= 64) || (Cin == 64 && Cout <= 32) ||
                                   (Cin == 64 && Cout <= 64 && stx_tune(STX_TUNE_CONV_L1_MARCH)))) {
        const long long ncols = (long long)B * stx_cdiv(Ho, MW2_TH) * stx_cdiv(Wo, MW2_MW);
        if (ncols * Do < (1ll << 31) && (long long)Hi * Wi * Cin * 4 < (1ll << 31) && (long long)Ho * Wo * Cout * 4 < (1ll << 31)) {
            p.kind = 0; p.march_wgs = march_wgs(ncols * Do); p.rows = p.march_wgs;
            return p;
        }
    }
    const long long tiles = (long long)stx_cdiv(Do, CONV_TD) * stx_cdiv(Ho, CONV_TH) * stx_cdiv(Wo, 32);
    if (conv_nt(Cout) == 4 && ks == 3 && tiles * B < (1ll << 31)) {
        const size_t lds = stride == 1 ? conv_lds_bytes<3, 1>(8, 4) : conv_lds_bytes<3, 2>(8, 4);
        p.kind = 1; p.pgrid = persistent_grid(lds, tiles * B); p.rows = p.pgrid;
        return p;
    }
    p.rows = tiles * B;
    return p;
}

extern "C" long long stx_conv3d_fwd_stat_rows(int B, int Di, int Hi, int Wi, int Cin, int Cout, int ks, int stride) {
    stx_begin();
    if (B < 1 || Di < 1 || Hi < 1 || Wi < 1 || Cin < 1 || Cout < 1 || !((ks == 3 && (stride == 1 || stride == 2)) || (ks == 1 && stride == 1)))
        return 0;
    return conv_plan(B, Di, Hi, Wi, Cin, Cout, ks, stride).rows;
}

extern "C" int stx_conv3d_fwd(const float* x, const float* wp, float* out, const float* scale, const float* bias,
                              const float* residual, float* stats, int B, int Di, int Hi, int Wi, int Cin, int Cout,
                              int ks, int stride, int relu, void* stream) {
    stx_begin();
    STX_REQUIRE(x && wp && out && B > 0 && Di > 0 && Hi > 0 && Wi > 0, "conv3d_fwd: bad shape");
    STX_REQUIRE(Cin % 8 == 0 && Cout >= 1 && Cout <= 128, "conv3d_fwd: Cin=%d (need %%8) Cout=%d (need <=128)", Cin, Cout);
    STX_REQUIRE((ks == 3 && (stride == 1 || stride == 2)) || (ks == 1 && stride == 1),
                "conv3d_fwd: kernel %d stride %d unsupported", ks, stride);
    ConvArgs a;
    a.x = x; a.wp = wp; a.out = out; a.scale = scale; a.bias = bias; a.residual = residual; a.stats = stats;
    a.Di = Di; a.Hi = Hi; a.Wi = Wi; a.Cin = Cin; a.Cout = Cout; a.relu = relu;
    const int pad = ks / 2;
    a.Do = (Di + 2 * pad - ks) / stride + 1;
    a.Ho = (Hi + 2 * pad - ks) / stride + 1;
    a.Wo = (Wi + 2 * pad - ks) / stride + 1;
    a.nDt = stx_cdiv(a.Do, CONV_TD); a.nHt = stx_cdiv(a.Ho, CONV_TH); a.nWt = stx_cdiv(a.Wo, 32);
    const int NT = conv_nt(Cout);
    hipStream_t st = (hipStream_t)stream;
    const ConvPlan plan = conv_plan(B, Di, Hi, Wi, Cin, Cout, ks, stride);
    if (plan.kind == 0) {
        MarchArgs m2;
        m2.c = a;
        m2.c.nHt = stx_cdiv(a.Ho, MW2_TH);
        m2.c.nWt = stx_cdiv(a.Wo, MW2_MW);
        m2.ncols = B * m2.c.nHt * m2.c.nWt;
        m2.ablate = stx_tune(STX_TUNE_MARCH_ABLATE);
        {
            const int nb2 = plan.march_wgs;
            const size_t lds2 = ((size_t)MW2_WFLOATS + 2 * (size_t)MW2_SLOT) * 4;
            const int bs = stx_tune(STX_TUNE_MARCH_BS), epi_fast = stx_tune(STX_TUNE_MARCH_EPI);
            const bool whole = a.Ho % MW2_TH == 0 && a.Wo % MW2_MW == 0;
            m2.xs = Cin; m2.os = Cout; m2.wq_total = Cin / 8; m2.wnt_total = conv_nt(Cout);
            const int nk = Cin / 32, nn = stx_cdiv(Cout, 32);
            for (int ns = 0; ns < nn; ++ns)
                for (int kslice = 0; kslice < nk; ++kslice) {
                    MarchArgs m = m2;
                    m.xo = 32 * kslice; m.wq_off = 4 * kslice;
                    m.oo = 32 * ns; m.wnt_off = ns; m.ncout = Cout - 32 * ns < 32 ? Cout - 32 * ns : 32;
                    m.acc_in = kslice > 0 ? out : nullptr;
                    if (kslice + 1 < nk) {
                        m.c.scale = nullptr; m.c.bias = nullptr; m.c.residual = nullptr; m.c.stats = nullptr; m.c.relu = 0;
                    }
                    const bool plain = epi_fast && !(m.c.residual && m.acc_in) && m.c.relu < 2;
                    const bool raw = !m.acc_in && !m.c.residual && !m.c.scale && !m.c.bias && m.c.relu == 0;
                    const int epi = plain ? (raw ? (whole && m.ncout == 32 ? 5 : 4) : m.acc_in ? 2 : (m.c.residual ? 3 : 0)) : 1;
                    if (int rc = launch_with_lds(march_kernel(bs, epi), dim3(nb2), lds2, st, m)) return rc;
                }
            return stx_check_launch("conv3d_fwd(march)");
        }
    }
    STX_REQUIRE(halo_range_ok(Di, Hi, Wi, Cin), "conv3d_fwd: a batch item of %d x %d x %d x %d floats exceeds the 2 GiB "
                "buffer-descriptor range", Di, Hi, Wi, Cin);
    const int CK = (stride == 2) ? 8 : conv_pick_ck(Cin, ks);
    dim3 grid(a.nDt * a.nHt * a.nWt, B);
    int rc;
    if (plan.kind == 1) {
        const long long nt_all = (long long)grid.x * B;
        {
            const size_t lds = stride == 1 ? conv_lds_bytes<3, 1>(8, 4) : conv_lds_bytes<3, 2>(8, 4);
            const int wn = stx_tune(STX_TUNE_CONV_WN) == 4 ? 4 : (stx_tune(STX_TUNE_CONV_WN) == 3 ? 2 : 1);
            rc = launch_with_lds(stride == 1 ? pgemm_kernel<1>(wn) : pgemm_kernel<2>(wn), dim3(plan.pgrid), lds, st, a, (int)nt_all);
            if (rc) return rc;
            return stx_check_launch("conv3d_fwd(pipelined)");
        }
    }
    if (ks == 3 && stride == 1) rc = conv_dispatch<3, 1>(a, NT, CK, grid, st);
    else if (ks == 3 && NT == 2 && stx_tune(STX_TUNE_CONV_S2_DENSE)) {
        if (stx_tune(STX_TUNE_CONV_WN) >= 2)
            rc = launch_with_lds(conv3d_igemm_kernel<3, 2, CONV_TD, CONV_TH, 2, 8, 0, 2>, grid, (size_t)5 * 5 * 66 * 8 * 4, st, a);
        else
        rc = launch_with_lds(conv3d_igemm_kernel<3, 2, CONV_TD, CONV_TH, 2, 8, 0>, grid, (size_t)5 * 5 * 66 * 8 * 4, st, a);
    }
    else if (ks == 3) rc = conv_dispatch<3, 2>(a, NT, CK, grid, st);
    else rc = conv_dispatch<1, 1>(a, NT, CK, grid, st);
    if (rc) return rc;
    return stx_check_launch("conv3d_fwd");
}

extern "C" int stx_deconv3d_fwd(const float* x, const float* wp, float* out, const float* scale, const float* bias,
                                const float* residual, float* stats, int B, int Di, int Hi, int Wi, int Cin, int Cout,
                                int Do, int Ho, int Wo, int relu, void* stream) {
    stx_begin();
    STX_REQUIRE(x && wp && out && B > 0 && Di > 0 && Hi > 0 && Wi > 0, "deconv3d_fwd: bad shape");
    STX_REQUIRE(Cin % 32 == 0 && Cout >= 1 && Cout <= 64, "deconv3d_fwd: Cin=%d (need %%32) Cout=%d (need <=64)", Cin, Cout);
    STX_REQUIRE(Do <= 2 * Di && Do >= 2 * Di - 1 && Ho <= 2 * Hi && Ho >= 2 * Hi - 1 && Wo <= 2 * Wi && Wo >= 2 * Wi - 1,
                "deconv3d_fwd: output dims must be 2*in or 2*in-1");
    ConvArgs a;
    a.x = x; a.wp = wp; a.out = out; a.scale = scale; a.bias = bias; a.residual = residual; a.stats = stats;
    a.Di = Di; a.Hi = Hi; a.Wi = Wi; a.Cin = Cin; a.Cout = Cout; a.relu = relu;
    a.Do = Do; a.Ho = Ho; a.Wo = Wo;
    a.nDt = Di; a.nHt = stx_cdiv(Hi, 2); a.nWt = stx_cdiv(Wi, 32);
    STX_REQUIRE(halo_range_ok(Di, Hi, Wi, Cin), "deconv3d_fwd: a batch item of %d x %d x %d x %d floats exceeds the 2 GiB "
                "buffer-descriptor range", Di, Hi, Wi, Cin);
    dim3 grid(a.nDt * a.nHt * a.nWt, B);
    hipStream_t st = (hipStream_t)stream;
    const size_t lds = (size_t)2 * 3 * 33 * (8 + 4) * 4;
    int rc = conv_nt(Cout) == 1 ? launch_with_lds(deconv3d_igemm_kernel<1, 8>, grid, lds, st, a)
                                : launch_with_lds(deconv3d_igemm_kernel<2, 8>, grid, lds, st, a);
    if (rc) return rc;
    return stx_check_launch("deconv3d_fwd");
}

static bool wgrad_pipe(int ks, int stride, int npairs) { return ks == 3 && (stride == 2 || npairs <= 2); }
static void wgrad_tile(int ks, int stride, int Wc, bool pipe, int* TH, int* TW) {
    *TH = pipe ? 4 : 2; *TW = (stride == 2) ? 16 : 32;
    if (ks == 3 && stride == 1 && stx_cdiv(Wc, 16) * 16 < stx_cdiv(Wc, 32) * 32) { *TH = 4; *TW = 16; }
}
static int wgrad_chunks(int ntiles, int npairs, bool pipe) {
    int c = (pipe ? 256 : 512) / npairs;
    if (c < 1) c = 1;
    if (c > ntiles) c = ntiles;
    const int forced = stx_tune(STX_TUNE_WGRAD_GRID);
    if (forced > 0 && forced < c) c = forced;
    return c;
}

struct StxWgradBn {
    const float* z; float* dz;
    const float *scale, *shift, *mean, *invstd, *gamma, *sum_g, *sum_gx;
    float inv_n; int act;
};
int stx_wgrad_march_launch(const float* x, const float* gy, float* slab, int B, int D, int H, int W, int CF, int CC, int nchunks,
                           void* stream, const StxWgradBn* bn);
int stx_wgrad_march_chunks(int B, int D, int H, int W, int npairs);
int stx_wgrad_march_s2_launch(const float* f, const float* c, float* slab, int B, int Df, int Hf, int Wf, int CF, int Dc, int Hc,
                              int Wc, int CC, int nchunks, void* stream);

extern "C" long long stx_conv3d_wgrad_workspace_floats(int B, int Dc, int Hc, int Wc, int CF, int CC, int ks,
                                                       int stride) {
    const int npairs = (CF / 32) * (CC / 32);
    if (npairs < 1 || B < 1 || Dc < 1 || Hc < 1 || Wc < 1) return 0;
    const int rows = (ks == 1) ? 8 : 27;
    const bool pipe = wgrad_pipe(ks, stride, npairs);
    int TH, TW;
    wgrad_tile(ks, stride, Wc, pipe, &TH, &TW);
    int c = wgrad_chunks(B * Dc * stx_cdiv(Hc, TH) * stx_cdiv(Wc, TW), npairs, pipe);
    if (ks == 3) {
        const int cm = stx_wgrad_march_chunks(B, Dc, Hc, Wc, npairs);
        if (cm > c) c = cm;
    }
    return (long long)npairs * c * rows * 1024;
}

extern "C" int stx_conv3d_wgrad(const float* f, const float* c, float* dw, float* workspace, int B, int Df, int Hf,
                                int Wf, int CF, int Dc, int Hc, int Wc, int CC, int ks, int stride, void* stream) {
    stx_begin();
    STX_REQUIRE(f && c && dw && workspace && B > 0, "conv3d_wgrad: null operand");
    STX_REQUIRE(CF >= 32 && CC >= 32 && CF % 32 == 0 && CC % 32 == 0,
                "conv3d_wgrad: channel counts (%d, %d) must be positive multiples of 32", CF, CC);
    STX_REQUIRE(Dc > 0 && Hc > 0 && Wc > 0, "conv3d_wgrad: empty volume");
    STX_REQUIRE((ks == 3 && (stride == 1 || stride == 2)) || (ks == 1 && stride == 1), "conv3d_wgrad: ks/stride");
    STX_REQUIRE((long long)Hf * Wf * CF * 4 < (1ll << 31) && (long long)Hc * Wc * CC * 4 < (1ll << 31),
                "conv3d_wgrad: a plane of %d x %d voxels exceeds the 2 GiB buffer-descriptor range", Hf, Wf);
    WgradArgs a;
    a.f = f; a.c = c; a.slab = workspace;
    a.B = B; a.Df = Df; a.Hf = Hf; a.Wf = Wf; a.CF = CF; a.Dc = Dc; a.Hc = Hc; a.Wc = Wc; a.CC = CC;
    const int npairs = (CF / 32) * (CC / 32);
    const bool pipe = wgrad_pipe(ks, stride, npairs);
    a.ablate = stx_tune(STX_TUNE_WGRAD_ABLATE);
    int TH, TW;
    wgrad_tile(ks, stride, Wc, pipe, &TH, &TW);
    a.nHt = stx_cdiv(Hc, TH); a.nWt = stx_cdiv(Wc, TW);
    a.ntiles = B * Dc * a.nHt * a.nWt;
    int nchunks = wgrad_chunks(a.ntiles, npairs, pipe);
    hipStream_t st = (hipStream_t)stream;
    const int T = ks == 1 ? 1 : 27;
    if (ks == 3 && (stx_tune(STX_TUNE_WGRAD_MARCH) & (stride == 1 ? 1 : 2))) {
        int mc = stx_wgrad_march_chunks(B, Dc, Hc, Wc, npairs);
        const int forced = stx_tune(STX_TUNE_WGRAD_GRID);
        if (forced > 0 && forced < mc) mc = forced;
        const int rc = stride == 1 ? stx_wgrad_march_launch(f, c, workspace, B, Dc, Hc, Wc, CF, CC, mc, stream, nullptr)
                                   : stx_wgrad_march_s2_launch(f, c, workspace, B, Df, Hf, Wf, CF, Dc, Hc, Wc, CC, mc, stream);
        if (rc > 0) return rc;
        if (rc == 0) {
            const int total = npairs * T * 1024;
            hipLaunchKernelGGL(conv3d_wgrad_reduce4_kernel, dim3(total / 64), dim3(CONV_THREADS), 0, st, workspace, dw, CF, CC, T,
                               mc, 27);
            return stx_check_launch("conv3d_wgrad_reduce");
        }
    }
    dim3 grid(nchunks, npairs);
#define WG_LAUNCH(KS_, S_, TH_, TW_, NW_, PIPE_, LDS_)                                                           \
    {                                                                                                             \
        const size_t lds = (LDS_);                                                                                \
        void (*wk)(WgradArgs) = conv3d_wgrad_kernel<KS_, S_, TH_, TW_, NW_, PIPE_>;                               \
        if (int rc = stx_lds_require((const void*)wk, lds, "conv3d_wgrad")) return rc;                            \
        hipLaunchKernelGGL(wk, grid, dim3(NW_ * 64), lds, st, a);                                                 \
    }
    if (ks == 3 && stride == 1) {
        if (TW == 16 && pipe) WG_LAUNCH(3, 1, 4, 16, 8, true, ((size_t)3 * 6 * 18 + 64) * 32 * 4)
        else if (TW == 16) WG_LAUNCH(3, 1, 4, 16, 8, false, ((size_t)3 * 6 * 18 + 64) * 32 * 4)
        else if (pipe) WG_LAUNCH(3, 1, 4, 32, 8, true, ((size_t)3 * 6 * 34 + 128) * 32 * 4)
        else WG_LAUNCH(3, 1, 2, 32, 8, false, ((size_t)3 * 4 * 34 + 64) * 32 * 4)
    } else if (ks == 3) {
        WG_LAUNCH(3, 2, 4, 16, 8, true, ((size_t)3 * 9 * 34 + 64) * 32 * 4)
    } else {
        WG_LAUNCH(1, 1, 2, 32, 4, false, ((size_t)2 * 32 + 64) * 32 * 4)
    }
#undef WG_LAUNCH
    int rc = stx_check_launch("conv3d_wgrad");
    if (rc) return rc;
    const int total = npairs * T * 1024;
    hipLaunchKernelGGL(conv3d_wgrad_reduce4_kernel, dim3(total / 64), dim3(CONV_THREADS), 0, st, workspace, dw, CF, CC, T,
                       nchunks, ks == 1 ? 4 : 27);
    return stx_check_launch("conv3d_wgrad_reduce");
}

extern "C" int stx_conv3d_wgrad_bn_supported(int B, int D, int H, int W, int CF, int CC) {
    stx_begin();
    return (stx_tune(STX_TUNE_WGRAD_MARCH) & 1) && B > 0 && D > 0 && H > 0 && W > 0 && CF >= 32 && CC >= 32 && CF % 32 == 0 &&
           CC % 32 == 0 && (long long)H * W * CF * 4 < (1ll << 31) && (long long)H * W * CC * 4 < (1ll << 31) &&
           (long long)B * stx_cdiv(H, 4) * stx_cdiv(W, 16) < (1ll << 31);
}

extern "C" int stx_conv3d_wgrad_bn(const float* x, const float* gy, const float* z, const float* scale, const float* shift,
                                   const float* mean, const float* invstd, const float* gamma, const float* sums, float inv_n,
                                   int act, float* dz, float* dw, float* workspace, int B, int D, int H, int W, int CF, int CC,
                                   void* stream) {
    stx_begin();
    STX_REQUIRE(x && gy && z && scale && shift && mean && invstd && sums && dz && dw && workspace, "conv3d_wgrad_bn: null operand");
    STX_REQUIRE(act == 0 || act == 1, "conv3d_wgrad_bn: activation code %d (0 or 1)", act);
    STX_REQUIRE(stx_conv3d_wgrad_bn_supported(B, D, H, W, CF, CC), "conv3d_wgrad_bn: shape (%d x %d x %d x %d, %d -> %d channels) is "
                "not served by the march kernel (ask stx_conv3d_wgrad_bn_supported)", B, D, H, W, CF, CC);
    const int npairs = (CF / 32) * (CC / 32);
    int mc = stx_wgrad_march_chunks(B, D, H, W, npairs);
    const int forced = stx_tune(STX_TUNE_WGRAD_GRID);
    if (forced > 0 && forced < mc) mc = forced;
    StxWgradBn bn;
    bn.z = z; bn.dz = dz; bn.scale = scale; bn.shift = shift; bn.mean = mean; bn.invstd = invstd; bn.gamma = gamma;
// ... 10 lines not shown
```

stereo_toolbox_amd/csrc/conv_c1.hip:

```cpp
#include "stx_common.h"
#include <stdlib.h>

namespace {

constexpr int C1_THREADS = 256;
constexpr int C1_TD = 2, C1_TH = 4, C1_TW = 32;
constexpr int C1_ED = C1_TD + 2, C1_EH = C1_TH + 2, C1_EW = C1_TW + 2;
constexpr int C1_CK = 16, C1_VS = C1_CK + 4;

struct C1Args {
    const float* x;
    const float* w;
    const float* gy;
    const float* res;
    float* out;
    int B, D, H, W, Cin;
    int nDt, nHt, nWt, ntiles;
};

__device__ __forceinline__ void c1_stage(const C1Args& a, float* tile, int b, int d0, int h0, int w0, int c0, int tid) {
    for (int idx = tid; idx < C1_ED * C1_EH * C1_EW * (C1_CK / 4); idx += C1_THREADS) {
        const int v = idx / (C1_CK / 4), f = idx - v * (C1_CK / 4);
        const int wx = v % C1_EW, hy = (v / C1_EW) % C1_EH, dz = v / (C1_EW * C1_EH);
        const int gd = d0 - 1 + dz, gh = h0 - 1 + hy, gw = w0 - 1 + wx;
// ... 86 lines not shown
                }
                acc[ck][0] += sA;
                acc[ck][1] += sB;
            }
        }
    }
    float* dst = a.out + (size_t)blockIdx.x * a.Cin * 27;
#pragma unroll
    for (int ck = 0; ck < 4; ++ck) {
        if (ck < nchunk) {
            dst[(ck * C1_CK + cl) * 27 + tapA] = acc[ck][0];
            if (tapB < 27) dst[(ck * C1_CK + cl) * 27 + tapB] = acc[ck][1];
        }
    }
}

__global__ __launch_bounds__(C1_THREADS) void c1_colsum_kernel(const float* __restrict__ partials, int nrows, int M,
                                                               float* __restrict__ sums) {
    __shared__ double red[C1_THREADS];
    const int m = blockIdx.x, tid = threadIdx.x;
    double s = 0.0;
    for (int r = tid; r < nrows; r += C1_THREADS) s += (double)partials[(size_t)r * M + m];
    red[tid] = s;
    __syncthreads();
    for (int k = C1_THREADS / 2; k > 0; k >>= 1) {
        if (tid < k) red[tid] += red[tid + k];
        __syncthreads();
    }
    if (tid == 0) sums[m] = (float)red[0];
}

constexpr size_t C1_TILE_BYTES = (size_t)C1_ED * C1_EH * C1_EW * C1_VS * 4;
constexpr int C1_WGRAD_BLOCKS = 512;


constexpr int C1D_TH = 4, C1D_TW = 32;
constexpr int C1D_EH = C1D_TH + 2, C1D_EW = C1D_TW + 2;

__global__ __launch_bounds__(C1_THREADS) void conv_c1_dgrad_kernel(const float* __restrict__ gy,
                                                                   const float* __restrict__ w, float* __restrict__ gx,
                                                                   int B, int D, int H, int W, int Cin, int nHt, int nWt) {
    __shared__ float gys[3 * C1D_EH * C1D_EW];
    __shared__ float ws[27 * 64];
    const int tid = threadIdx.x;
    int r = blockIdx.x;
    const int wt = r % nWt; r /= nWt;
    const int ht = r % nHt; r /= nHt;
    const int d = r % D;
    const int b = r / D;
    const int h0 = ht * C1D_TH, w0 = wt * C1D_TW;
    for (int idx = tid; idx < 3 * C1D_EH * C1D_EW; idx += C1_THREADS) {
        const int wx = idx % C1D_EW, hy = (idx / C1D_EW) % C1D_EH, dz = idx / (C1D_EW * C1D_EH);
        const int gd = d - 1 + dz, gh = h0 - 1 + hy, gw = w0 - 1 + wx;
        gys[idx] = (gd >= 0 && gd < D && gh >= 0 && gh < H && gw >= 0 && gw < W)
                       ? gy[(((size_t)b * D + gd) * H + gh) * W + gw] : 0.f;
    }
    for (int idx = tid; idx < 27 * Cin; idx += C1_THREADS) {
        const int c = idx % Cin, tap = idx / Cin;
        ws[tap * Cin + c] = w[(size_t)c * 27 + tap];
    }
    __syncthreads();
    const int CQ = Cin >> 2;
    for (int item = tid; item < CQ * (C1D_TH * C1D_TW / 4); item += C1_THREADS) {
        const int q = item % CQ, grp = item / CQ;
        const int lw = (grp % (C1D_TW / 4)) * 4, lh = grp / (C1D_TW / 4);
        float4 acc[4];
#pragma unroll
        for (int j = 0; j < 4; ++j) acc[j] = make_float4(0.f, 0.f, 0.f, 0.f);
#pragma unroll
        for (int kd = 0; kd < 3; ++kd)
#pragma unroll
            for (int kh = 0; kh < 3; ++kh) {
                const float* gp = gys + (((2 - kd) * C1D_EH) + (lh + 2 - kh)) * C1D_EW + lw;
                float g6[6];
#pragma unroll
                for (int j = 0; j < 6; ++j) g6[j] = gp[j];
#pragma unroll
                for (int kw = 0; kw < 3; ++kw) {
                    const float4 wv = stx_ld4(ws + ((kd * 3 + kh) * 3 + kw) * Cin + 4 * q);
#pragma unroll
                    for (int j = 0; j < 4; ++j) {
                        const float g = g6[j + 2 - kw];
                        acc[j].x = fmaf(g, wv.x, acc[j].x);
                        acc[j].y = fmaf(g, wv.y, acc[j].y);
                        acc[j].z = fmaf(g, wv.z, acc[j].z);
                        acc[j].w = fmaf(g, wv.w, acc[j].w);
                    }
                }
            }
        const int oh = h0 + lh;
        if (oh < H) {
            float* o = gx + ((((size_t)b * D + d) * H + oh) * W + w0 + lw) * Cin + 4 * q;
#pragma unroll
            for (int j = 0; j < 4; ++j)
                if (w0 + lw + j < W) stx_st4(o + (size_t)j * Cin, acc[j]);
        }
    }
}


__global__ __launch_bounds__(C1_THREADS) void conv_c1_dgrad_mfma_kernel(const float* __restrict__ gy,
                                                                        const float* __restrict__ w, float* __restrict__ gx,
                                                                        int B, int D, int H, int W, int nHt, int nWt, int ntiles) {
    __shared__ float gys[3 * C1D_EH * C1D_EW];
    const int tid = threadIdx.x, lane = tid & 63, wave = tid >> 6;
    const int i = lane & 31, half = lane >> 5;
    float wreg[14];
    int aoff[14];
#pragma unroll
    for (int j = 0; j < 14; ++j) {
        const int tap = 2 * j + half;
        const int tp = tap < 27 ? tap : 26;
        const int kd = tp / 9, kh = (tp / 3) % 3, kw = tp % 3;
        wreg[j] = tap < 27 ? w[(size_t)i * 27 + tap] : 0.f;
        aoff[j] = ((2 - kd) * C1D_EH + (wave + 2 - kh)) * C1D_EW + i + 2 - kw;
    }
    const unsigned plane_bytes = (unsigned)H * (unsigned)W * 128u;
    for (int tile = blockIdx.x; tile < ntiles; tile += gridDim.x) {
        int r_ = tile;
        const int wt = r_ % nWt; r_ /= nWt;
        const int ht = r_ % nHt; r_ /= nHt;
        const int d = r_ % D;
        const int b = r_ / D;
        const int h0 = ht * C1D_TH, w0 = wt * C1D_TW;
        __syncthreads();
        for (int idx = tid; idx < 3 * C1D_EH * C1D_EW; idx += C1_THREADS) {
            const int wx = idx % C1D_EW, hy = (idx / C1D_EW) % C1D_EH, dz = idx / (C1D_EW * C1D_EH);
            const int gd = d - 1 + dz, gh = h0 - 1 + hy, gw = w0 - 1 + wx;
            gys[idx] = (gd >= 0 && gd < D && gh >= 0 && gh < H && gw >= 0 && gw < W)
                           ? gy[(((size_t)b * D + gd) * H + gh) * W + gw] : 0.f;
        }
        __syncthreads();
        f32x16 acc;
#pragma unroll
        for (int r = 0; r < 16; ++r) acc[r] = 0.f;
        float av[14];
#pragma unroll
        for (int j = 0; j < 14; ++j) av[j] = gys[aoff[j]];
#pragma unroll
        for (int j = 0; j < 14; ++j) acc = __builtin_amdgcn_mfma_f32_32x32x2f32(av[j], wreg[j], acc, 0, 0, 0);
        const int oh = h0 + wave;
        const stx_bufrsrc ors = stx_make_rsrc(gx + ((size_t)b * D + d) * H * W * 32, plane_bytes);
        const unsigned vbase = (unsigned)((((oh < H ? oh : 0) * W + w0 + 4 * half) * 32 + i) * 4);
#pragma unroll
        for (int r = 0; r < 16; ++r) {
            const int m = (r & 3) + 8 * (r >> 2);
            const bool ok = oh < H && w0 + 4 * half + m < W;
            stx_buf_st1(ors, ok ? vbase : STX_BUF_OOB, (unsigned)(m * 128), acc[r]);
        }
    }
}


constexpr int C1M_TD = 2, C1M_TH = 8, C1M_TW = 32;
constexpr int C1M_ED = C1M_TD + 2, C1M_EH = C1M_TH + 2, C1M_EW = C1M_TW + 2;
constexpr int C1M_BLOCKS = 1024;

__global__ __launch_bounds__(C1_THREADS) void conv_c1_wgrad_mfma_kernel(const float* __restrict__ x,
                                                                        const float* __restrict__ gy,
                                                                        float* __restrict__ slab, int B, int D, int H,
                                                                        int W, int Cin, int nDt, int nHt, int nWt,
                                                                        int ntiles) {
    __shared__ float gys[C1M_ED * C1M_EH * C1M_EW];
    __shared__ float red[4][1024];
    const int tid = threadIdx.x, lane = tid & 63, wave = tid >> 6;
    const int i = lane & 31, half = lane >> 5;
    const int cb = blockIdx.y;
    const int kd = i / 9, kh = (i / 3) % 3, kw = i % 3;
    const int toff = (i < 27) ? ((2 - kd) * C1M_EH + (2 - kh)) * C1M_EW + (2 - kw) + half : half;
    f32x16 acc;
#pragma unroll
    for (int r = 0; r < 16; ++r) acc[r] = 0.f;
    for (int t = blockIdx.x; t < ntiles; t += gridDim.x) {
        int r = t;
        const int wt = r % nWt; r /= nWt;
        const int ht = r % nHt; r /= nHt;
        const int dt = r % nDt;
        const int b = r / nDt;
        const int d0 = dt * C1M_TD, h0 = ht * C1M_TH, w0 = wt * C1M_TW;
        __syncthreads();
        for (int idx = tid; idx < C1M_ED * C1M_EH * C1M_EW; idx += C1_THREADS) {
            const int wx = idx % C1M_EW, hy = (idx / C1M_EW) % C1M_EH, dz = idx / (C1M_EW * C1M_EH);
            const int gd = d0 - 1 + dz, gh = h0 - 1 + hy, gw = w0 - 1 + wx;
            gys[idx] = (gd >= 0 && gd < D && gh >= 0 && gh < H && gw >= 0 && gw < W)
                           ? gy[(((size_t)b * D + gd) * H + gh) * W + gw] : 0.f;
        }
        __syncthreads();
#pragma unroll 1
        for (int k = 0; k < 4; ++k) {
            const int row = wave * 4 + k;
            const int ld = row / C1M_TH, lh = row % C1M_TH;
            const int gd = d0 + ld, gh = h0 + lh;
            const bool rowok = gd < D && gh < H;
            const float* xr = x + ((((size_t)b * D + gd) * H + gh) * W + w0 + half) * Cin + cb * 32 + i;
            float av[16];
#pragma unroll
            for (int p = 0; p < 16; ++p)
                av[p] = (rowok && w0 + 2 * p + half < W) ? xr[(size_t)(2 * p) * Cin] : 0.f;
            const float* gp = gys + (ld * C1M_EH + lh) * C1M_EW + toff;
#pragma unroll
            for (int p = 0; p < 16; ++p) {
                float bv = gp[2 * p];
                bv = (i < 27) ? bv : 0.f;
                acc = __builtin_amdgcn_mfma_f32_32x32x2f32(av[p], bv, acc, 0, 0, 0);
            }
        }
    }
#pragma unroll
    for (int r = 0; r < 16; ++r) red[wave][((r & 3) + 8 * (r >> 2) + 4 * half) * 32 + i] = acc[r];
    __syncthreads();
    float* dst = slab + ((size_t)cb * gridDim.x + blockIdx.x) * 1024;
    for (int idx = tid; idx < 1024; idx += C1_THREADS)
        dst[idx] = (red[0][idx] + red[1][idx]) + (red[2][idx] + red[3][idx]);
}

__global__ __launch_bounds__(C1_THREADS) void c1m_reduce_kernel(const float* __restrict__ slab, int nrows,
                                                                float* __restrict__ dw) {
    __shared__ double red[C1_THREADS];
    const int m = blockIdx.x, tid = threadIdx.x;
    const int tap = m % 27, cfull = m / 27, cb = cfull >> 5, c = cfull & 31;
    const float* p = slab + (size_t)cb * nrows * 1024 + c * 32 + tap;
    double s = 0.0;
    for (int r = tid; r < nrows; r += C1_THREADS) s += (double)p[(size_t)r * 1024];
    red[tid] = s;
    __syncthreads();
    for (int k = C1_THREADS / 2; k > 0; k >>= 1) {
        if (tid < k) red[tid] += red[tid + k];
        __syncthreads();
    }
    if (tid == 0) dw[m] = (float)red[0];
}


constexpr int C1F_TH = 8, C1F_TW = 32;
constexpr int C1F_EH = C1F_TH + 2, C1F_EW = C1F_TW + 2, C1F_NV = C1F_EH * C1F_EW;
constexpr int C1F_MT = (C1F_NV + 31) / 32;
constexpr int C1F_WGS = 512;

__global__ __launch_bounds__(C1_THREADS) void conv_c1_fwd_mfma_kernel(const float* __restrict__ x,
                                                                      const float* __restrict__ w,
                                                                      const float* __restrict__ res,
                                                                      float* __restrict__ out, int B, int D, int H, int W,
                                                                      int nHt, int nWt, int ncols) {
    STX_DYN_SMEM(smem);
    float* Ps = reinterpret_cast<float*>(smem);
    const int tid = threadIdx.x, lane = tid & 63, wave = __builtin_amdgcn_readfirstlane(tid >> 6);
    const int i = lane & 31, half = lane >> 5;
    float wreg[16];
#pragma unroll
    for (int s_ = 0; s_ < 16; ++s_) wreg[s_] = (i < 27) ? w[(size_t)(16 * half + s_) * 27 + i] : 0.f;
    const int lh = tid / C1F_TW, lw = tid % C1F_TW;

    constexpr int MTW = (C1F_MT + 3) / 4;
    const long long units = (long long)ncols * D;
    int u = __builtin_amdgcn_readfirstlane((int)(units * blockIdx.x / gridDim.x));
    const int u_end = __builtin_amdgcn_readfirstlane((int)(units * (blockIdx.x + 1) / gridDim.x));
    const unsigned plane_bytes = (unsigned)H * (unsigned)W * 32u * 4u;
    while (u < u_end) {
        const int col = u / D;
        const int d_lo = u - col * D;
        const int left = u_end - u;
        const int d_hi = (D - d_lo < left) ? D : d_lo + left;
        u += d_hi - d_lo;
        const int wt = col % nWt, ht = (col / nWt) % nHt, b = col / (nWt * nHt);
        const int h0 = ht * C1F_TH, w0 = wt * C1F_TW;
        const int oh = h0 + lh, ow = w0 + lw;
        const bool ook = oh < H && ow < W;
        unsigned voff[MTW];
#pragma unroll
        for (int t = 0; t < MTW; ++t) {
            const int hv = (wave + 4 * t) * 32 + i;
            const int hy = hv / C1F_EW, wx = hv - hy * C1F_EW;
            const int gh = h0 - 1 + hy, gw = w0 - 1 + wx;
            const bool ok = wave + 4 * t < C1F_MT && hv < C1F_NV && gh >= 0 && gh < H && gw >= 0 && gw < W;
            voff[t] = ok ? (unsigned)(((gh * W + gw) * 32 + 16 * half) * 4) : STX_BUF_OOB;
        }
        float4 nxt[MTW][4];
        auto load_plane = [&](int p) {
            const bool in = p >= 0 && p < D && p <= d_hi;
            const stx_bufrsrc rs = stx_make_rsrc(x + ((size_t)b * D + (in ? p : 0)) * H * W * 32, in ? plane_bytes : 0u);
#pragma unroll
            for (int t = 0; t < MTW; ++t)
#pragma unroll
                for (int q = 0; q < 4; ++q) nxt[t][q] = stx_buf_ld4(rs, voff[t], 16u * q);
        };
        float accA = 0.f, accB = 0.f;
        load_plane(d_lo - 1);
        __syncthreads();
        for (int p = d_lo - 1; p <= d_hi; ++p) {
            float* Pb = Ps + ((p + 2) & 1) * (C1F_NV * 27);
            const bool pin = p >= 0 && p < D;
            float4 cur[MTW][4];
#pragma unroll
            for (int t = 0; t < MTW; ++t)
#pragma unroll
                for (int q = 0; q < 4; ++q) cur[t][q] = nxt[t][q];
            load_plane(p + 1);
            if (pin) {
#pragma unroll
                for (int t = 0; t < MTW; ++t) {
                    const int m = wave + 4 * t;
                    if (m < C1F_MT) {
                        f32x16 acc;
#pragma unroll
                        for (int r = 0; r < 16; ++r) acc[r] = 0.f;
#pragma unroll
                        for (int q = 0; q < 4; ++q) {
                            acc = __builtin_amdgcn_mfma_f32_32x32x2f32(cur[t][q].x, wreg[4 * q + 0], acc, 0, 0, 0);
                            acc = __builtin_amdgcn_mfma_f32_32x32x2f32(cur[t][q].y, wreg[4 * q + 1], acc, 0, 0, 0);
                            acc = __builtin_amdgcn_mfma_f32_32x32x2f32(cur[t][q].z, wreg[4 * q + 2], acc, 0, 0, 0);
                            acc = __builtin_amdgcn_mfma_f32_32x32x2f32(cur[t][q].w, wreg[4 * q + 3], acc, 0, 0, 0);
                        }
                        if (i < 27) {
#pragma unroll
                            for (int r = 0; r < 16; ++r) {
                                const int v = m * 32 + (r & 3) + 8 * (r >> 2) + 4 * half;
                                if (v < C1F_NV) Pb[v * 27 + i] = acc[r];
                            }
                        }
                    }
                }
            }
            __syncthreads();
            float s0 = 0.f, s1 = 0.f, s2 = 0.f;
            if (pin) {
#pragma unroll
                for (int kh = 0; kh < 3; ++kh)
#pragma unroll
                    for (int kw = 0; kw < 3; ++kw) {
                        const float* pp = Pb + ((lh + kh) * C1F_EW + lw + kw) * 27 + kh * 3 + kw;
                        s0 += pp[0];
                        s1 += pp[9];
                        s2 += pp[18];
                    }
            }
            const float done = accA + s2;
            const int od = p - 1;
            if (od >= d_lo && od < d_hi && ook) {
                const size_t o = (((size_t)b * D + od) * H + oh) * W + ow;
                out[o] = res ? done + res[o] : done;
            }
            accA = accB + s1;
            accB = s0;
        }
    }
}

}

extern "C" int stx_conv3d_c1_fwd(const float* x, const float* w, const float* residual, float* out, int B, int D,
                                 int H, int W, int Cin, void* stream) {
    stx_begin();
    STX_REQUIRE(x && w && out && B > 0 && D > 0 && H > 0 && W > 0, "conv3d_c1_fwd: bad shape");
    STX_REQUIRE(Cin % C1_CK == 0, "conv3d_c1_fwd: Cin=%d must be a multiple of %d", Cin, C1_CK);
    if (Cin == 32 && (long long)H * W * 128 < (1ll << 31)) {
        const int nHt = stx_cdiv(H, C1F_TH), nWt = stx_cdiv(W, C1F_TW);
        const long long ncols = (long long)B * nHt * nWt, units = ncols * D;
        STX_REQUIRE(units < (1ll << 31), "conv3d_c1_fwd: volume too large");
        long long g = C1F_WGS;
        if (g > units / 4) g = units / 4 > 0 ? units / 4 : 1;
        const size_t lds = (size_t)2 * C1F_NV * 27 * 4;
        if (int rc = stx_lds_require((const void*)conv_c1_fwd_mfma_kernel, lds, "conv3d_c1_fwd(mfma)")) return rc;
        hipLaunchKernelGGL(conv_c1_fwd_mfma_kernel, dim3((unsigned)g), dim3(C1_THREADS), lds, (hipStream_t)stream, x, w,
                           residual, out, B, D, H, W, nHt, nWt, (int)ncols);
        return stx_check_launch("conv3d_c1_fwd(mfma)");
    }
    C1Args a;
    a.x = x; a.w = w; a.gy = nullptr; a.res = residual; a.out = out;
    a.B = B; a.D = D; a.H = H; a.W = W; a.Cin = Cin;
    a.nDt = stx_cdiv(D, C1_TD); a.nHt = stx_cdiv(H, C1_TH); a.nWt = stx_cdiv(W, C1_TW);
    a.ntiles = B * a.nDt * a.nHt * a.nWt;
    if (int rc = stx_lds_require((const void*)conv_c1_fwd_kernel, C1_TILE_BYTES, "conv3d_c1_fwd")) return rc;
    hipLaunchKernelGGL(conv_c1_fwd_kernel, dim3(a.ntiles), dim3(C1_THREADS), C1_TILE_BYTES, (hipStream_t)stream, a);
    return stx_check_launch("conv3d_c1_fwd");
}

extern "C" long long stx_conv3d_c1_wgrad_workspace_floats(int Cin) {
    const long long valu = (long long)C1_WGRAD_BLOCKS * Cin * 27;
    const long long mfma = (long long)C1M_BLOCKS * 1024 * ((Cin + 31) / 32);
    return valu > mfma ? valu : mfma;
}

extern "C" int stx_conv3d_c1_wgrad(const float* x, const float* gy, float* dw, float* workspace, int B, int D, int H,
                                   int W, int Cin, void* stream) {
    stx_begin();
    STX_REQUIRE(x && gy && dw && workspace && B > 0, "conv3d_c1_wgrad: null operand");
    STX_REQUIRE(Cin % C1_CK == 0 && Cin <= 4 * C1_CK, "conv3d_c1_wgrad: Cin=%d must be 16..64 in steps of 16", Cin);
    if (Cin % 32 == 0) {
        const int nDt = stx_cdiv(D, C1M_TD), nHt = stx_cdiv(H, C1M_TH), nWt = stx_cdiv(W, C1M_TW);
        const long long nt = (long long)B * nDt * nHt * nWt;
        STX_REQUIRE(nt < (1ll << 31), "conv3d_c1_wgrad: volume too large");
        const int nblk = nt < C1M_BLOCKS ? (int)nt : C1M_BLOCKS;
        hipStream_t st = (hipStream_t)stream;
        hipLaunchKernelGGL(conv_c1_wgrad_mfma_kernel, dim3(nblk, Cin / 32), dim3(C1_THREADS), 0, st, x, gy, workspace, B,
                           D, H, W, Cin, nDt, nHt, nWt, (int)nt);
        int rc = stx_check_launch("conv3d_c1_wgrad(mfma)");
        if (rc) return rc;
        hipLaunchKernelGGL(c1m_reduce_kernel, dim3(Cin * 27), dim3(C1_THREADS), 0, st, workspace, nblk, dw);
        return stx_check_launch("conv3d_c1_wgrad(reduce)");
    }
    C1Args a;
    a.x = x; a.w = nullptr; a.gy = gy; a.res = nullptr; a.out = workspace;
    a.B = B; a.D = D; a.H = H; a.W = W; a.Cin = Cin;
    a.nDt = stx_cdiv(D, C1_TD); a.nHt = stx_cdiv(H, C1_TH); a.nWt = stx_cdiv(W, C1_TW);
    a.ntiles = B * a.nDt * a.nHt * a.nWt;
    const int nblk = a.ntiles < C1_WGRAD_BLOCKS ? a.ntiles : C1_WGRAD_BLOCKS;
    const size_t lds = C1_TILE_BYTES + 256 * 4;
    hipStream_t st = (hipStream_t)stream;
    if (int rc = stx_lds_require((const void*)conv_c1_wgrad_kernel, lds, "conv3d_c1_wgrad")) return rc;
    hipLaunchKernelGGL(conv_c1_wgrad_kernel, dim3(nblk), dim3(C1_THREADS), lds, st, a);
    if (int rc = stx_check_launch("conv3d_c1_wgrad")) return rc;
    hipLaunchKernelGGL(c1_colsum_kernel, dim3(Cin * 27), dim3(C1_THREADS), 0, st, workspace, nblk, Cin * 27, dw);
    return stx_check_launch("conv3d_c1_colsum");
}

extern "C" int stx_conv3d_c1_dgrad(const float* gy, const float* w, float* gx, int B, int D, int H, int W, int Cin,
                                   void* stream) {
    stx_begin();
    STX_REQUIRE(gy && w && gx && B > 0 && D > 0 && H > 0 && W > 0, "conv3d_c1_dgrad: bad shape");
    STX_REQUIRE(Cin % 4 == 0 && Cin <= 64, "conv3d_c1_dgrad: Cin=%d must be a multiple of 4, <= 64", Cin);
    const int nHt = stx_cdiv(H, C1D_TH), nWt = stx_cdiv(W, C1D_TW);
    const long long nt = (long long)B * D * nHt * nWt;
    if (Cin == 32 && (long long)H * W * 128 < (1ll << 31) && nt < (1ll << 31)) {
        const long long g = nt < 256 * 8 ? nt : 256 * 8;
        hipLaunchKernelGGL(conv_c1_dgrad_mfma_kernel, dim3((unsigned)g), dim3(C1_THREADS), 0, (hipStream_t)stream, gy, w, gx, B, D,
                           H, W, nHt, nWt, (int)nt);
        return stx_check_launch("conv3d_c1_dgrad(mfma)");
    }
    hipLaunchKernelGGL(conv_c1_dgrad_kernel, dim3((unsigned)((size_t)B * D * nHt * nWt)), dim3(C1_THREADS), 0,
                       (hipStream_t)stream, gy, w, gx, B, D, H, W, Cin, nHt, nWt);
    return stx_check_launch("conv3d_c1_dgrad");
}
```

stereo_toolbox_amd/ops.py:

```python
import ctypes

import torch

from ._capi import StxError, get_lib

_P = ctypes.c_void_p


class _DevPtr(ctypes.c_void_p):
    """A device pointer that remembers the device of the tensor it came from: _call() reads the launch device off its
    own arguments, so nothing survives between launches (an exception between building the arguments and the launch
    cannot leak state into the next one)."""


def _stream(dev=None):
    return _P(torch.cuda.current_stream(dev).cuda_stream)


def _p(t):
    if t is None:
        return None
    p = _DevPtr(t.data_ptr())
    p.dev = t.device
    return p


def on_device(t):
    return t.is_cuda


def _chk(t, name, dims=None):
    if t is None:
        return
    if not t.is_cuda:
        raise StxError(f"{name}: expected a ROCm device tensor, got {t.device} -- the cost-volume hot path has "
                       "no CPU fallback (the CPU oracle lives in oracle/ and is test-only)")
    if t.dtype != torch.float32:
        raise StxError(f"{name}: expected float32, got {t.dtype}")
    if not t.is_contiguous():
        raise StxError(f"{name}: expected a dense contiguous tensor, strides {t.stride()}")
    if dims is not None and t.dim() != dims:
        raise StxError(f"{name}: expected {dims} dims, got shape {tuple(t.shape)}")


def _call(name, *args):
    dev = None
    for a in args:
        if isinstance(a, _DevPtr):
            if dev is None:
                dev = a.dev
            elif a.dev != dev:
                raise StxError(f"{name}: operands live on different devices ({dev} and {a.dev})")
    if dev is not None and dev.type == "cuda" and dev.index != torch.cuda.current_device():
        with torch.cuda.device(dev):
            get_lib().call(name, *args, _stream(dev))
    else:
        get_lib().call(name, *args, _stream(dev))


_LOW = (torch.float16, torch.bfloat16)


def _to_fp32(v):
    if isinstance(v, torch.Tensor):
        return v.float() if v.dtype in _LOW else v
    if isinstance(v, dict):
        return {k: _to_fp32(x) for k, x in v.items()}
    if isinstance(v, (list, tuple)):
        return type(v)(_to_fp32(x) for x in v)
    return v


def autocast_active():
    return torch.is_autocast_enabled("cuda") or torch.is_autocast_enabled("cpu")


def fp32_region(fn):
    import functools

    @functools.wraps(fn)
    def wrapped(*args, **kwargs):
        if not autocast_active():
            return fn(*args, **kwargs)
        with torch.autocast("cuda", enabled=False), torch.autocast("cpu", enabled=False):
            return fn(*_to_fp32(args), **_to_fp32(kwargs))
    return wrapped


def to_ncdhw(x):
    return x.permute(0, 4, 1, 2, 3)


def to_ndhwc(x):
    return x.permute(0, 2, 3, 4, 1).contiguous()


class _Workspace:

    def __init__(self):
        self.bufs = {}

    def get(self, tag, nfloats, device):
        sid = torch.cuda.current_stream(device).cuda_stream if device.type == "cuda" else 0
        key = (device.index, sid, tag)
        b = self.bufs.get(key)
        if b is None or b.numel() < nfloats:
            b = torch.empty(int(nfloats), dtype=torch.float32, device=device)
            self.bufs[key] = b
        return b


_WS = _Workspace()


_CACHE_ENABLED = True


def set_weight_cache(enabled):
    global _CACHE_ENABLED
    _CACHE_ENABLED = bool(enabled)


def invalidate_caches(model):
    for m in model.modules():
        m.__dict__.pop("_stx_fold", None)
    for p in model.parameters():
        p.__dict__.pop("_stx_packed", None)


def pack_weight(w, mode, owner=None):
    _chk(w, "weight", 5)
    if owner is not None and _CACHE_ENABLED:
        cache = owner.__dict__.setdefault("_stx_packed", {})
        hit = cache.get(mode)
        if hit is not None and hit[0] == (owner._version, owner.data_ptr()):
            return hit[1]
    A, Bd = w.shape[0], w.shape[1]
    T = w.shape[2] * w.shape[3] * w.shape[4]
    K, N = (Bd, A) if mode == 0 else (A, Bd)
    n = get_lib().raw("stx_conv3d_packed_floats")(K, N, T)
    wp = torch.empty(n, dtype=torch.float32, device=w.device)
    _call("stx_conv3d_pack_weight", _p(w), _p(wp), A, Bd, T, mode)
    if owner is not None and _CACHE_ENABLED:
        cache[mode] = ((owner._version, owner.data_ptr()), wp)
    return wp


def _pad_channels(t, C):
    if t.shape[-1] == C:
        return t
    out = t.new_zeros(*t.shape[:-1], C)
    out[..., : t.shape[-1]] = t
    return out


def pad_input_channels(x, w):
    Cin = x.shape[-1]
    Cp = (Cin + 7) // 8 * 8
    if Cp == Cin:
        return x, w
    wp = w.new_zeros(w.shape[0], Cp, *w.shape[2:])
    wp[:, :Cin] = w
    return _pad_channels(x, Cp), wp


def pad_weight_channels(w, Cp):
    if w.shape[1] == Cp:
        return w
    wp = w.new_zeros(w.shape[0], Cp, *w.shape[2:])
    wp[:, : w.shape[1]] = w
    return wp


def conv_out_dims(D, H, W, ks, stride):
    pad = ks // 2
    return tuple((d + 2 * pad - ks) // stride + 1 for d in (D, H, W))


def conv3d_forward(x, wp, Cout, ks, stride, scale=None, bias=None, residual=None, relu=False, want_stats=False):
    _chk(x, "x", 5)
    B, D, H, W, Cin = x.shape
    Do, Ho, Wo = conv_out_dims(D, H, W, ks, stride)
    out = torch.empty(B, Do, Ho, Wo, Cout, dtype=torch.float32, device=x.device)
    stats = None
    if want_stats:
        rows = get_lib().raw("stx_conv3d_fwd_stat_rows")(B, D, H, W, Cin, Cout, ks, stride)
        stats = torch.empty(rows, 2, Cout, dtype=torch.float32, device=x.device)
    _call("stx_conv3d_fwd", _p(x), _p(wp), _p(out), _p(scale), _p(bias), _p(residual), _p(stats), B, D, H, W, Cin,
          Cout, ks, stride, int(relu))
    return out, stats


def deconv3d_forward(x, wp, Cout, out_dims=None, scale=None, bias=None, residual=None, relu=False, want_stats=False):
    _chk(x, "x", 5)
    B, D, H, W, Cin = x.shape
    Do, Ho, Wo = out_dims if out_dims is not None else (2 * D, 2 * H, 2 * W)
    if Cout > 64:
        if Cout % 64 != 0:
            raise StxError(f"deconv3d_forward: Cout={Cout} > 64 must be a multiple of 64")
        nt = Cout // 32
        wv = wp.view(-1, Cin // 8, nt, 256)
        outs, sts = [], []
        for h in range(Cout // 64):
            sl = slice(64 * h, 64 * h + 64)
            o, st_ = deconv3d_forward(x, wv[:, :, 2 * h:2 * h + 2].contiguous(), 64, (Do, Ho, Wo),
                                      None if scale is None else scale[sl].contiguous(),
                                      None if bias is None else bias[sl].contiguous(),
                                      None if residual is None else residual[..., sl].contiguous(), relu, want_stats)
            outs.append(o)
            sts.append(st_)
        return torch.cat(outs, -1), (torch.cat(sts, -1) if want_stats else None)
    out = torch.empty(B, Do, Ho, Wo, Cout, dtype=torch.float32, device=x.device)
    stats = None
    if want_stats:
        nb = get_lib().raw("stx_deconv3d_fwd_blocks")(D, H, W)
        stats = torch.empty(B * nb, 2, Cout, dtype=torch.float32, device=x.device)
    _call("stx_deconv3d_fwd", _p(x), _p(wp), _p(out), _p(scale), _p(bias), _p(residual), _p(stats), B, D, H, W, Cin,
          Cout, Do, Ho, Wo, int(relu))
    return out, stats


def conv3d_wgrad(fine, coarse, ks, stride):
    B, Df, Hf, Wf, CF = fine.shape
    _, Dc, Hc, Wc, CC = coarse.shape
    n = get_lib().raw("stx_conv3d_wgrad_workspace_floats")(B, Dc, Hc, Wc, CF, CC, ks, stride)
    ws = _WS.get("wgrad", n, fine.device)
    dw = torch.empty(CC, CF, ks ** 3, dtype=torch.float32, device=fine.device)
    _call("stx_conv3d_wgrad", _p(fine), _p(coarse), _p(dw), _p(ws), B, Df, Hf, Wf, CF, Dc, Hc, Wc, CC, ks, stride)
    return dw


def conv3d_wgrad_bn(x, gy, pend):
    B, D, H, W, CF = x.shape
    CC = gy.shape[-1]
    n = get_lib().raw("stx_conv3d_wgrad_workspace_floats")(B, D, H, W, CF, CC, 3, 1)
    ws = _WS.get("wgrad", n, x.device)
    dw = torch.empty(CC, CF, 27, dtype=torch.float32, device=x.device)
    dz = torch.empty_like(gy)
    _call("stx_conv3d_wgrad_bn", _p(x), _p(gy), _p(pend.z), _p(pend.scale), _p(pend.shift), _p(pend.mean), _p(pend.invstd),
          _p(pend.gamma), _p(pend.sums), float(pend.inv_n), int(pend.act), _p(dz), _p(dw), _p(ws), B, D, H, W, CF, CC)
    return dw, dz


class _PendingBn:
    __slots__ = ("g", "z", "scale", "shift", "mean", "invstd", "gamma", "sums", "inv_n", "act")

    def materialize(self):
        C = self.z.shape[-1]
        nvox = self.z.numel() // C
        dz = torch.empty_like(self.z)
        _call("stx_bn_bwd_apply2", _p(self.g), None, _p(self.z), _p(self.mean), _p(self.invstd), _p(self.gamma), None, None,
              None, None, _p(self.scale), _p(self.shift), None, None, _p(self.sums), _p(dz), None, None, nvox, C, int(self.act), 1)
        return dz


_BN_DEFER = {"outstanding": 0, "armed": False}


def _bn_defer_check():
    n, _BN_DEFER["outstanding"], _BN_DEFER["armed"] = _BN_DEFER["outstanding"], 0, False
    if n:
        raise StxError(f"{n} deferred BatchNorm-backward record(s) were not consumed by their convolution's backward node: "
                       "the gradients of this backward pass are wrong (set STX_BN_BWD_IN_WGRAD=0 and report)")


def _defer_pending_bn(g, pend):
    g._stx_pending_bn = pend
    _BN_DEFER["outstanding"] += 1
    if not _BN_DEFER["armed"]:
        _BN_DEFER["armed"] = True
        torch.autograd.Variable._execution_engine.queue_callback(_bn_defer_check)


def bn_defer_reset_if_stale():
    if not _BN_DEFER["armed"]:
        return
    task_id = getattr(torch._C, "_current_graph_task_id", None)
    if task_id is None or task_id() == -1:
        _BN_DEFER["outstanding"], _BN_DEFER["armed"] = 0, False


def _take_pending_bn(g):
    pend = getattr(g, "_stx_pending_bn", None) if g is not None else None
    if pend is not None:
        del g._stx_pending_bn
        _BN_DEFER["outstanding"] -= 1
        if pend.g is not g:
            raise StxError("deferred BatchNorm backward: record attached to a different gradient tensor")
    return pend


def _is_c1(w, ks, stride, transposed):
    return (not transposed) and ks == 3 and stride == 1 and w.shape[0] == 1 and w.shape[1] % 16 == 0 and w.shape[1] <= 64


def conv3d_c1_forward(x, w, residual=None):
    _chk(x, "x", 5)
    _chk(w, "weight", 5)
    B, D, H, W, Cin = x.shape
    out = torch.empty(B, D, H, W, 1, dtype=torch.float32, device=x.device)
    _call("stx_conv3d_c1_fwd", _p(x), _p(w), _p(residual), _p(out), B, D, H, W, Cin)
    return out


def conv3d_c1_wgrad(x, gy):
    B, D, H, W, Cin = x.shape
    ws = _WS.get("c1wgrad", get_lib().raw("stx_conv3d_c1_wgrad_workspace_floats")(Cin), x.device)
    dw = torch.empty(1, Cin, 3, 3, 3, dtype=torch.float32, device=x.device)
    _call("stx_conv3d_c1_wgrad", _p(x), _p(gy), _p(dw), _p(ws), B, D, H, W, Cin)
    return dw


def conv3d_c1_dgrad(gy, w, Cin):
    B, D, H, W, _ = gy.shape
    gx = torch.empty(B, D, H, W, Cin, dtype=torch.float32, device=gy.device)
    _call("stx_conv3d_c1_dgrad", _p(gy), _p(w), _p(gx), B, D, H, W, Cin)
    return gx


class ConvRawFn(torch.autograd.Function):

    @staticmethod
    def forward(ctx, x, w, ks, stride, transposed, want_stats):
        _chk(x, "x", 5)
        ctx.cin_true = None
        ctx.x_prepadded = False
        if not transposed and x.shape[-1] != w.shape[1]:
            if x.shape[-1] != (w.shape[1] + 7) // 8 * 8:
                raise StxError(f"conv: input has {x.shape[-1]} channels, weight expects {w.shape[1]}")
            ctx.cin_true, ctx.x_prepadded = w.shape[1], True
            w = pad_weight_channels(w, x.shape[-1])
        elif not transposed and x.shape[-1] % 8 != 0:
            ctx.cin_true = x.shape[-1]
            x, w = pad_input_channels(x, w)
        if _is_c1(w, ks, stride, transposed) and not want_stats:
            z, stats = conv3d_c1_forward(x, w.contiguous()), None
        elif transposed:
            Cout = w.shape[1]
            z, stats = deconv3d_forward(x, pack_weight(w, 2), Cout, want_stats=want_stats)
        else:
            Cout = w.shape[0]
            z, stats = conv3d_forward(x, pack_weight(w, 0), Cout, ks, stride, want_stats=want_stats)
        ctx.save_for_backward(x, w)
        ctx.cfg = (ks, stride, transposed)
        if stats is None:
            stats = x.new_empty(0)
        ctx.mark_non_differentiable(stats)
        return z, stats

    @staticmethod
    def backward(ctx, gz, _gstats):
        x, w = ctx.saved_tensors
        ks, stride, transposed = ctx.cfg
        pend = _take_pending_bn(gz)
        gx = gw = None
        B, D, H, W, Cin = x.shape
        if pend is not None:
            if (ctx.needs_input_grad[1] and not transposed and ks == 3 and stride == 1 and ctx.cin_true is None
                    and get_lib().raw("stx_conv3d_wgrad_bn_supported")(B, D, H, W, Cin, w.shape[0])):
                gw_pre, gz = conv3d_wgrad_bn(x, gz, pend)
                gw_pre = gw_pre.reshape(w.shape)
            else:
                gw_pre, gz = None, pend.materialize()
        else:
            gw_pre = None
        gz = gz.contiguous()
        if transposed:
            Ci, Co = w.shape[0], w.shape[1]
            if ctx.needs_input_grad[0]:
                gx, _ = conv3d_forward(gz, pack_weight(w, 0), Ci, 3, 2)
            if ctx.needs_input_grad[1]:
                gz_w = gz if Co % 32 == 0 else _pad_channels(gz, (Co + 31) // 32 * 32)
                x_w = x if Ci % 32 == 0 else _pad_channels(x, (Ci + 31) // 32 * 32)
                gw = conv3d_wgrad(gz_w, x_w, 3, 2)[:Ci, :Co].reshape(w.shape)
        else:
            Co, Ci = w.shape[0], w.shape[1]
            c1 = _is_c1(w, ks, stride, transposed)
            gz_k, w_k = gz, w
            if Co % 8 != 0 and not c1:
                Cp = (Co + 7) // 8 * 8
                gz_k = _pad_channels(gz, Cp)
                w_k = w.new_zeros(Cp, *w.shape[1:])
                w_k[:Co] = w
            if ctx.needs_input_grad[0]:
                if c1:
                    gx = conv3d_c1_dgrad(gz, w.contiguous(), Ci)
                elif stride == 1 and Ci > 128:
                    parts = []
                    for lo in range(0, Ci, 128):
                        hi = min(Ci, lo + 128)
                        g, _ = conv3d_forward(gz_k, pack_weight(w_k[:, lo:hi].contiguous(), 1), hi - lo, ks, 1)
                        parts.append(g)
                    gx = torch.cat(parts, -1)
                elif stride == 1:
                    gx, _ = conv3d_forward(gz_k, pack_weight(w_k, 1), Ci, ks, 1)
                else:
                    if Co % 32:
                        Cp = (Co + 31) // 32 * 32
                        gz_k = _pad_channels(gz, Cp)
                        w_k = w.new_zeros(Cp, *w.shape[1:])
                        w_k[:Co] = w
                    gx, _ = deconv3d_forward(gz_k, pack_weight(w_k, 2), Ci, out_dims=(D, H, W))
            if gw_pre is not None:
                gw = gw_pre
            elif ctx.needs_input_grad[1]:
                if c1:
                    gw = conv3d_c1_wgrad(x, gz)
                else:
                    gz_w = gz if Co % 32 == 0 else _pad_channels(gz, (Co + 31) // 32 * 32)
                    x_w = x if Ci % 32 == 0 else _pad_channels(x, (Ci + 31) // 32 * 32)
                    gw = conv3d_wgrad(x_w, gz_w, ks, stride)[:Co, :Ci].reshape(w.shape)
        if ctx.cin_true is not None:
            if gx is not None and not ctx.x_prepadded:
                gx = gx[..., :ctx.cin_true].contiguous()
            if gw is not None:
                gw = gw[:, :ctx.cin_true].contiguous()
        return gx, gw, None, None, None, None


class SharedInputConvsFn(torch.autograd.Function):

    @staticmethod
    def forward(ctx, x, cfgs, *ws):
        _chk(x, "x", 5)
        outs = []
        for (ks, stride, want), w in zip(cfgs, ws):
            if x.shape[-1] != w.shape[1] or w.shape[1] % 8 or w.shape[0] % 8 or _is_c1(w, ks, stride, False):
                raise StxError(f"SharedInputConvsFn: weight {tuple(w.shape)} on an input of {x.shape[-1]} channels")
            z, stats = conv3d_forward(x, pack_weight(w, 0), w.shape[0], ks, stride, want_stats=want)
            if stats is None:
                stats = x.new_empty(0)
            ctx.mark_non_differentiable(stats)
            outs += [z, stats]
        ctx.save_for_backward(x, *ws)
        ctx.cfgs = cfgs
        return tuple(outs)

    @staticmethod
    def backward(ctx, *grads):
        x, ws = ctx.saved_tensors[0], ctx.saved_tensors[1:]
        B, D, H, W, Ci = x.shape
        gws = [None] * len(ws)
        gzs = []
        for k, g in enumerate(grads[0::2]):
            pend = _take_pending_bn(g)
            if pend is not None:
                ks, stride, _ = ctx.cfgs[k]
                if (ctx.needs_input_grad[2 + k] and ks == 3 and stride == 1
                        and get_lib().raw("stx_conv3d_wgrad_bn_supported")(B, D, H, W, Ci, ws[k].shape[0])):
                    gw, g = conv3d_wgrad_bn(x, g, pend)
                    gws[k] = gw.reshape(ws[k].shape)
                else:
                    g = pend.materialize()
            gzs.append(None if g is None else g.contiguous())
        gx = None
        if ctx.needs_input_grad[0]:
            rank = lambda k: (0 if ctx.cfgs[k][0] == 3 and ctx.cfgs[k][1] == 1 else (1 if ctx.cfgs[k][1] == 2 else 2))
            for k in sorted((k for k in range(len(ws)) if gzs[k] is not None), key=rank):
                (ks, stride, _), w, gz = ctx.cfgs[k], ws[k], gzs[k]
                if stride == 1:
                    gx, _ = conv3d_forward(gz, pack_weight(w, 1), Ci, ks, 1, residual=gx)
                else:
                    Co = w.shape[0]
                    gz_k, w_k = gz, w
                    if Co % 32:
                        Cp = (Co + 31) // 32 * 32
                        gz_k = _pad_channels(gz, Cp)
                        w_k = w.new_zeros(Cp, *w.shape[1:])
                        w_k[:Co] = w
                    gx, _ = deconv3d_forward(gz_k, pack_weight(w_k, 2), Ci, out_dims=(D, H, W), residual=gx)
        for k, (w, gz) in enumerate(zip(ws, gzs)):
            if gz is None or not ctx.needs_input_grad[2 + k] or gws[k] is not None:
                continue
            ks, stride, _ = ctx.cfgs[k]
            Co = w.shape[0]
            gz_w = gz if Co % 32 == 0 else _pad_channels(gz, (Co + 31) // 32 * 32)
            x_w = x if Ci % 32 == 0 else _pad_channels(x, (Ci + 31) // 32 * 32)
            gws[k] = conv3d_wgrad(x_w, gz_w, ks, stride)[:Co, :Ci].reshape(w.shape)
        return (gx, None, *gws)


_D4_SEL = ((3, 1, 4), (4, 2, 0))


def embed_deconv4_weight(w):
    Ci, Co = w.shape[0], w.shape[1]
    wz = torch.cat((w, w.new_zeros(Ci, Co, 1, 4, 4)), 2)
    wz = torch.cat((wz, wz.new_zeros(Ci, Co, 5, 1, 4)), 3)
    wz = torch.cat((wz, wz.new_zeros(Ci, Co, 5, 5, 1)), 4)
    parts = []
    for pd in (0, 1):
        for ph in (0, 1):
            for pw in (0, 1):
                sel = wz[:, :, list(_D4_SEL[pd])][:, :, :, list(_D4_SEL[ph])][:, :, :, :, list(_D4_SEL[pw])]
                parts.append(sel.transpose(0, 1))
    return torch.cat(parts, 0).contiguous()


class DepthToSpaceFn(torch.autograd.Function):

    @staticmethod
    def forward(ctx, y):
        y = y.contiguous()
        _chk(y, "y", 5)
        B, D, H, W, C8 = y.shape
        C = C8 // 8
        out = torch.empty(B, 2 * D, 2 * H, 2 * W, C, dtype=torch.float32, device=y.device)
        _call("stx_depth_to_space", _p(y), _p(out), B, D, H, W, C, 0)
        return out

    @staticmethod
    def backward(ctx, g):
        g = g.contiguous()
        B, D2, H2, W2, C = g.shape
        gy = torch.empty(B, D2 // 2, H2 // 2, W2 // 2, 8 * C, dtype=torch.float32, device=g.device)
        _call("stx_depth_to_space", _p(g), _p(gy), B, D2 // 2, H2 // 2, W2 // 2, C, 1)
        return gy


def _d4_chunks(Co):
    per = max(1, min(8, 128 // Co))
    return [(c0, min(8, c0 + per)) for c0 in range(0, 8, per)]


def deconv4_raw(x, w, want_stats):
    Co = w.shape[1]
    if Co % 4:
        raise StxError(f"ConvTranspose3d(k4): {Co} output channels (need a multiple of 4)")
    w3 = embed_deconv4_weight(w)
    ys = [ConvRawFn.apply(x, w3[c0 * Co:c1 * Co], 3, 1, False, False)[0] for c0, c1 in _d4_chunks(Co)]
    z = DepthToSpaceFn.apply(ys[0] if len(ys) == 1 else torch.cat(ys, -1))
    return z, (bn_stats(z.detach()) if want_stats else z.new_empty(0))


@fp32_region
def deconv4_forward(x, w, scale=None, bias=None, relu=0, owner=None):
    _chk(x, "x", 5)
    Co = w.shape[1]
    if Co % 4:
        raise StxError(f"ConvTranspose3d(k4): {Co} output channels (need a multiple of 4)")
    cache = owner.__dict__.setdefault("_stx_packed", {}) if (owner is not None and _CACHE_ENABLED) else None
    key = (owner._version, owner.data_ptr()) if owner is not None else None
    hit = cache.get("d4") if cache is not None else None
    if hit is not None and hit[0] == key:
        packed = hit[1]
    else:
        w3 = embed_deconv4_weight(w)
        packed = [pack_weight(w3[c0 * Co:c1 * Co].contiguous(), 0) for c0, c1 in _d4_chunks(Co)]
        if cache is not None:
            cache["d4"] = (key, packed)
    ys = []
    for (c0, c1), wp in zip(_d4_chunks(Co), packed):
        n = c1 - c0
        ys.append(conv3d_forward(x, wp, n * Co, 3, 1, None if scale is None else scale.repeat(n),
                                 None if bias is None else bias.repeat(n), None, relu)[0])
    B, D, H, W, _ = x.shape
    y = ys[0] if len(ys) == 1 else torch.cat(ys, -1)
    out = torch.empty(B, 2 * D, 2 * H, 2 * W, Co, dtype=torch.float32, device=x.device)
    _call("stx_depth_to_space", _p(y), _p(out), B, D, H, W, Co, 0)
    return out


class GateFn(torch.autograd.Function):

    @staticmethod
    def forward(ctx, cv, att):
        out = gate(cv.detach(), att.detach())
        ctx.save_for_backward(cv, att)
        return out

    @staticmethod
    def backward(ctx, g):
        cv, att = ctx.saved_tensors
        g = g.contiguous()
        B, D, H, W, C = cv.shape
        gcv = torch.empty_like(cv) if ctx.needs_input_grad[0] else None
        gatt = torch.empty_like(att) if ctx.needs_input_grad[1] else None
        if gcv is not None or gatt is not None:
            _call("stx_gate_bwd", _p(g), _p(cv), _p(att), _p(gcv), _p(gatt), B, D, H * W, C)
        return gcv, gatt

# ... 63 lines not shown
            ptrs = [_p(o) for o in dst] + [None] * (4 - len(dst))
            cs = ctx.cs + [0] * (4 - len(dst))
            _call("stx_split_channels", _p(g), *ptrs, *cs, nvox)
        return tuple(outs)


@fp32_region
def cat_channels(parts):
    parts = [p.contiguous() for p in parts]
    if not 2 <= len(parts) <= 4:
        raise StxError(f"cat_channels: {len(parts)} parts (2 to 4)")
    lead = parts[0].shape[:-1]
    for p in parts:
        if p.shape[:-1] != lead or p.shape[-1] % 4 or p.dtype != torch.float32 or p.device != parts[0].device:
            raise StxError(f"cat_channels: parts {[tuple(q.shape) for q in parts]} (equal leading shape, fp32, widths % 4 == 0)")
    return CatChannelsFn.apply(*parts)


def conv2d_supported(conv):
    return (conv.kernel_size == (3, 3) and conv.stride == (1, 1) and conv.padding == (1, 1) and conv.dilation == (1, 1)
            and conv.groups == 1 and conv.bias is None and conv.in_channels in (32, 64) and conv.out_channels in (32, 64))


def _ohwi(w):
    v = w.permute(0, 2, 3, 1)
    return v if v.is_contiguous() else v.contiguous()


def conv2d_forward(x, w, dgrad=False, groups=1, want_stats=False):
    _chk(x, "x", 4)
    wo = _ohwi(w)
    _chk(wo, "weight", 4)
    B, H, W, Cin = x.shape
    Co, Ci = w.shape[0], w.shape[1]
    Kin, Nout = (Co, Ci) if dgrad else (Ci, Co)
    if Cin != Kin or B % groups:
        raise StxError(f"conv2d: input {tuple(x.shape)} against weight {tuple(w.shape)} (dgrad={dgrad}, groups={groups})")
    out = torch.empty(B, H, W, Nout, dtype=torch.float32, device=x.device)
    part = None
    if want_stats:
        rows = int(get_lib().raw("stx_conv2d_stat_rows")(groups))
        part = torch.empty(rows, 2, Nout, dtype=torch.float32, device=x.device)
    _call("stx_conv2d_fwd", _p(x), _p(wo), _p(out), _p(part), B, H, W, Kin, Nout, int(dgrad), groups)
    if part is not None and groups > 1:
        part = part.view(groups, rows // groups, 2, Nout)
    return out, part


class Conv2dFn(torch.autograd.Function):

    @staticmethod
    def forward(ctx, x, w, groups):
        xl = x.permute(0, 2, 3, 1)
        if not xl.is_contiguous():
            xl = xl.contiguous()
        z, part = conv2d_forward(xl, w, False, groups, True)
        ctx.save_for_backward(x, w)
        ctx.mark_non_differentiable(part)
        return z, part

    @staticmethod
    def backward(ctx, gz, _gpart):
        x, w = ctx.saved_tensors
        gz = gz.contiguous()
        gx = gw = None
        if ctx.needs_input_grad[0]:
            gx = conv2d_forward(gz, w, True)[0].permute(0, 3, 1, 2)
        if ctx.needs_input_grad[1]:
            gw = torch.ops.aten.convolution_backward(gz.permute(0, 3, 1, 2), x, w, None, (1, 1), (1, 1), (1, 1), False, (0, 0), 1,
                                                     (False, True, False))[1]
        return gx, gw, None


def bn_finalize(partials, count, gamma, beta, running_mean, running_var, momentum, eps, groups=1):
    C = partials.shape[-1]
    out = torch.empty(4, groups, C, dtype=torch.float32, device=partials.device)
    _call("stx_bn_finalize_groups", _p(partials), partials.shape[-3], C, float(count), _p(gamma), _p(beta),
          _p(running_mean), _p(running_var), float(momentum), float(eps), _p(out), groups)
    return list(out.unbind(0)) if groups > 1 else list(out[:, 0].unbind(0))


@fp32_region
def bn_stats(z, groups=1):
    _chk(z, "z")
    C = z.shape[-1]
    nvox = z.numel() // C // groups
    if groups < 1 or z.shape[0] % groups:
        raise StxError(f"bn_stats: leading axis {z.shape[0]} does not split into {groups} groups")
    rows = get_lib().raw("stx_bn_stats_rows")(nvox, C)
    if rows <= 0:
        raise StxError(f"bn_stats: C={C} unsupported")
    part = torch.empty(groups, rows, 2, C, dtype=torch.float32, device=z.device)
    _call("stx_bn_stats", _p(z), _p(part), nvox, C, groups)
    return part if groups > 1 else part[0]


def _sync_bn_partials(partials, count, group, world):
    import torch.distributed as dist
    tot = partials.double().sum(0)
    dist.all_reduce(tot, group=group)
    hi = tot.float()
    lo = (tot - hi.double()).float()
    return torch.stack((hi, lo)).contiguous(), count * world


@fp32_region
def bn_apply(z1, scale1, shift1, z2=None, scale2=None, shift2=None, relu=False, groups=1):
    out = torch.empty_like(z1)
    C = z1.shape[-1]
    _call("stx_bn_apply", _p(z1), _p(scale1), _p(shift1), _p(z2), _p(scale2), _p(shift2), _p(out),
          z1.numel() // C // groups, C, int(relu), groups)
    return out


class BnActFn(torch.autograd.Function):

    @staticmethod
    def forward(ctx, z1, gamma1, beta1, z2, gamma2, beta2, residual, relu, bn1, bn2, groups=1, defer=False):
        G = int(groups)
        ctx.defer = bool(defer)

        def affine(gamma, beta, bn):
            if bn["training"]:
                partials, count = bn["partials"], bn["count"]
                if bn.get("sync"):
                    if G > 1:
                        raise StxError("BnActFn: SyncBatchNorm with groups is not wired (SyncBN runs the views separately)")
                    partials, count = _sync_bn_partials(partials, count, *bn["sync"])
                return bn_finalize(partials, count, gamma, beta, bn["running_mean"], bn["running_var"], bn["momentum"],
                                   bn["eps"], G)
            invstd = torch.rsqrt(bn["running_var"] + bn["eps"])
            scale = gamma * invstd
            res = (scale, beta - bn["running_mean"] * scale, bn["running_mean"].clone(), invstd)
            return res if G == 1 else [t.unsqueeze(0).expand(G, -1).contiguous() for t in res]

        relu = int(relu)
        if relu == 2 and residual is not None:
            raise StxError("BnActFn: Mish with a plain residual is not wired (no model of the family uses it)")
        if G < 1 or z1.shape[0] % G:
            raise StxError(f"BnActFn: leading axis {z1.shape[0]} does not split into {G} groups")
        sc1, sh1, m1, i1 = affine(gamma1, beta1, bn1)
        two = z2 is not None
        if two:
            sc2, sh2, m2, i2 = affine(gamma2, beta2, bn2)
            y = bn_apply(z1, sc1, sh1, z2, sc2, sh2, relu, G)
        else:
            sc2 = sh2 = m2 = i2 = None
            y = bn_apply(z1, sc1, sh1, residual, None, None, relu, G)
        ctx.relu, ctx.two, ctx.has_res, ctx.groups = relu, two, residual is not None, G
        ctx.train1 = bn1["training"]
        ctx.train2 = bn2["training"] if two else False
        ctx.sync = bn1.get("sync") or (bn2.get("sync") if two else None)
        ctx.remask = bool(relu) and residual is None
        keep_y = y if (relu and not ctx.remask) else None
        ctx.save_for_backward(z1, gamma1, m1, i1, z2, gamma2, m2, i2, keep_y, sc1 if ctx.remask else None,
                              sh1 if ctx.remask else None, sc2 if (ctx.remask and two) else None,
                              sh2 if (ctx.remask and two) else None)
        return y

    @staticmethod
    def backward(ctx, gy):
        z1, gamma1, m1, i1, z2, gamma2, m2, i2, y, sc1, sh1, sc2, sh2 = ctx.saved_tensors
        gy = gy.contiguous()
        G = ctx.groups
        C = z1.shape[-1]
        nvox = z1.numel() // C // G
        lib = get_lib()
        NB = lib.raw("stx_bn_reduce_blocks")()
        part = _WS.get("bnred", G * NB * 3 * C, z1.device)
        sums_all = torch.empty(G + (1 if G > 1 else 0), 3, C, dtype=torch.float32, device=z1.device)
        sums = sums_all[:G]
        _call("stx_bn_bwd_reduce2", _p(gy), _p(y), _p(z1), _p(m1), _p(i1), _p(z2) if ctx.two else None,
              _p(m2) if ctx.two else None, _p(i2) if ctx.two else None, _p(sc1), _p(sh1), _p(sc2), _p(sh2), _p(part),
              _p(sums_all), nvox, C, int(ctx.relu), G)
        if not ctx.needs_input_grad[0] and not ctx.two and not ctx.has_res:
            tot = sums_all[G] if G > 1 else sums_all[0]
            return (None, tot[1], tot[0], None, None, None, None, None, None, None, None, None)
        if (ctx.defer and not ctx.two and not ctx.has_res and ctx.relu in (0, 1) and ctx.train1 and not ctx.sync and G == 1
                and (not ctx.relu or ctx.remask)):
            alias = gy.view_as(gy)
            pend = _PendingBn()
            pend.g, pend.z, pend.scale, pend.shift, pend.mean, pend.invstd = alias, z1, sc1, sh1, m1, i1
            pend.gamma, pend.sums, pend.inv_n, pend.act = gamma1, sums, 1.0 / nvox, int(ctx.relu)
            if pend.scale is None:
                pend.scale = pend.shift = m1
            _defer_pending_bn(alias, pend)
            tot = sums_all[0]
            return (alias, tot[1], tot[0], None, None, None, None, None, None, None, None, None)
        dz1 = torch.empty_like(z1)
        dz2 = torch.empty_like(z2) if ctx.two else None
        gres = torch.empty_like(z1) if (ctx.has_res and ctx.relu) else None
        use = sums
        if ctx.sync:
            import torch.distributed as dist
            use = sums.clone()
            dist.all_reduce(use, group=ctx.sync[0])
            use /= ctx.sync[1]
        if not ctx.train1 or (ctx.two and not ctx.train2):
            use = torch.zeros_like(sums)
        _call("stx_bn_bwd_apply2", _p(gy), _p(y), _p(z1), _p(m1), _p(i1), _p(gamma1), _p(z2) if ctx.two else None,
              _p(m2) if ctx.two else None, _p(i2) if ctx.two else None, _p(gamma2) if ctx.two else None, _p(sc1), _p(sh1),
              _p(sc2), _p(sh2), _p(use), _p(dz1), _p(dz2), _p(gres), nvox, C, int(ctx.relu), G)
        if ctx.has_res and not ctx.relu:
            gres = gy
        tot = sums_all[G] if G > 1 else sums_all[0]
        return (dz1, tot[1], tot[0], dz2, tot[2] if ctx.two else None, tot[0].clone() if ctx.two else None, gres,
                None, None, None, None, None)


class MishFn(torch.autograd.Function):

    @staticmethod
    def forward(ctx, x):
        x = x.contiguous()
        _chk(x, "x")
        y = torch.empty_like(x)
        _call("stx_mish_fwd", _p(x), _p(y), x.numel())
        ctx.save_for_backward(x)
        return y

    @staticmethod
    def backward(ctx, gy):
        (x,) = ctx.saved_tensors
        gy = gy.contiguous()
        gx = torch.empty_like(x)
        _call("stx_mish_bwd", _p(gy), _p(x), _p(gx), x.numel())
        return gx


@fp32_region
def mish(x):
    if torch.is_grad_enabled() and x.requires_grad:
        return MishFn.apply(x)
    x = x.contiguous()
    _chk(x, "x")
    y = torch.empty_like(x)
    _call("stx_mish_fwd", _p(x), _p(y), x.numel())
    return y


def _cv_shapes(Lg, Lc, num_groups):
    ref = Lg if Lg is not None else Lc
    B, _, H, W = ref.shape
    Cg = Lg.shape[1] if Lg is not None else 0
    Cc = Lc.shape[1] if Lc is not None else 0
    G = num_groups if Lg is not None else 0
    return B, H, W, Cg, G, Cc


@fp32_region
def cost_volume_forward(Lg, Rg, Lc, Rc, maxdisp, num_groups, mask_left=True, scale=None):
    for n, t in (("ref gwc", Lg), ("tgt gwc", Rg), ("ref concat", Lc), ("tgt concat", Rc)):
        _chk(t, n, 4)
    B, H, W, Cg, G, Cc = _cv_shapes(Lg, Lc, num_groups)
    if G:
        assert Cg % G == 0
    vol = torch.empty(B, maxdisp, H, W, G + 2 * Cc, dtype=torch.float32, device=(Lg if Lg is not None else Lc).device)
    _call("stx_cost_volume_fwd", _p(Lg), _p(Rg), Cg, G, _p(Lc), _p(Rc), Cc, _p(scale), _p(vol), B, H, W, maxdisp,
          int(mask_left))
    return vol


class CostVolumeFn(torch.autograd.Function):

    @staticmethod
    def forward(ctx, Lg, Rg, Lc, Rc, maxdisp, num_groups, mask_left):
        ctx.save_for_backward(Lg, Rg)
        ctx.cfg = (maxdisp, num_groups, mask_left, None if Lc is None else Lc.shape)
        return cost_volume_forward(Lg, Rg, Lc, Rc, maxdisp, num_groups, mask_left)

    @staticmethod
    def backward(ctx, gvol):
        Lg, Rg = ctx.saved_tensors
        maxdisp, num_groups, mask_left, cshape = ctx.cfg
        gvol = gvol.contiguous()
        B, D, H, W, CT = gvol.shape
        Cg = Lg.shape[1] if Lg is not None else 0
        G = num_groups if Lg is not None else 0
        Cc = cshape[1] if cshape is not None else 0
        gLg = torch.empty_like(Lg) if G else None
        gRg = torch.empty_like(Rg) if G else None
        gLc = gvol.new_empty(cshape) if Cc else None
        gRc = gvol.new_empty(cshape) if Cc else None
        _call("stx_cost_volume_bwd", _p(gvol), _p(Lg), _p(Rg), Cg, G, Cc, _p(gLg), _p(gRg), _p(gLc), _p(gRc), B, H, W,
              D, int(mask_left))
        return gLg, gRg, gLc, gRc, None, None, None


class GroupNormalizeFn(torch.autograd.Function):

    @staticmethod
    def forward(ctx, x, num_groups, out_scale):
        x = x.contiguous()
        _chk(x, "x", 4)
        B, C, H, W = x.shape
        y = torch.empty_like(x)
        _call("stx_group_normalize_fwd", _p(x), _p(y), B, C, num_groups, H * W, float(out_scale))
        ctx.save_for_backward(x)
        ctx.cfg = (num_groups, float(out_scale))
        return y

    @staticmethod
    def backward(ctx, gy):
        (x,) = ctx.saved_tensors
        gy = gy.contiguous()
        B, C, H, W = x.shape
        gx = torch.empty_like(x)
        _call("stx_group_normalize_bwd", _p(x), _p(gy), _p(gx), B, C, ctx.cfg[0], H * W, ctx.cfg[1])
        return gx, None, None


@fp32_region
def group_normalize(x, num_groups, out_scale=1.0):
    assert x.dim() == 4 and x.shape[1] % num_groups == 0, f"C:{x.shape[1]}, num_groups:{num_groups}"
    return GroupNormalizeFn.apply(channel_major(x), num_groups, out_scale)


@fp32_region
def cost_volume(Lg, Rg, Lc, Rc, maxdisp, num_groups, mask_left=True, normalize=False):
    if normalize and Lg is not None:
        Lg = group_normalize(Lg, num_groups, float(Lg.shape[1] // num_groups))
        Rg = group_normalize(Rg, num_groups, 1.0)
    ts = [channel_major(t) if t is not None else None for t in (Lg, Rg, Lc, Rc)]
    if torch.is_grad_enabled() and any(t is not None and t.requires_grad for t in ts):
        return CostVolumeFn.apply(*ts, maxdisp, num_groups, mask_left)
    return cost_volume_forward(*ts, maxdisp, num_groups, mask_left)

# ... 1029 lines not shown
```

Baseline: 0.1784 pairs/s.

## Fuse batch-norm backward reductions into the following conv's dgrad epilogue

When a BN+ReLU output feeds a 3x3x3 stride-1 conv with 32 channels (or a single-output conv), that conv's dgrad kernel now reads the BN input z and computes the masked per-channel gradient sums (sum g and sum g*xhat) in its epilogue, writing per-block rows. BN backward then runs only a small column-sum over those rows instead of a full stx_bn_bwd_reduce2 pass over gy, y and z. This removes one full read pass over large 5D activations per eligible BN layer. In exchange the dgrad kernel gains an extra z load and more registers, and a Python-side record validates tensor identity and version, falling back to the old path when they do not match.

```diff
diff --git a/include/stx_hip.h b/include/stx_hip.h
--- a/include/stx_hip.h
+++ b/include/stx_hip.h
@@ -65,6 +65,15 @@
 int stx_conv3d_c1_wgrad(const float* x, const float* gy, float* dw, float* workspace, int B, int D, int H, int W,
                         int Cin, void* stream);
 int stx_conv3d_c1_dgrad(const float* gy, const float* w, float* gx, int B, int D, int H, int W, int Cin, void* stream);
+
+int stx_conv3d_dgrad_bnsums_rows(int B, int D, int H, int W, int C);
+int stx_conv3d_dgrad_bnsums(const float* gy, const float* wp, float* gx, const float* z, const float* scale, const float* shift,
+                            const float* mean, const float* invstd, int act, float* rows, int B, int D, int H, int W, int C,
+                            void* stream);
+int stx_conv3d_c1_dgrad_bnsums_rows(int B, int D, int H, int W, int Cin);
+int stx_conv3d_c1_dgrad_bnsums(const float* gy, const float* w, float* gx, const float* z, const float* scale, const float* shift,
+                               const float* mean, const float* invstd, int act, float* rows, int B, int D, int H, int W, int Cin,
+                               void* stream);
 
 int stx_mish_fwd(const float* x, float* y, long long n, void* stream);
 int stx_mish_bwd(const float* gy, const float* x, float* gx, long long n, void* stream);
@@ -117,6 +126,7 @@
                       const float* gamma2, const float* scale1, const float* shift1, const float* scale2,
                       const float* shift2, const float* sums, float* dz1, float* dz2, float* gout, long long nvox,
                       int C, int relu, int groups, void* stream);
+int stx_bn_colsum(const float* partials, int nrows, int M, float* sums, void* stream);
 
 int stx_pad_normalize_u8(const unsigned char* img, float* out, int B, int H, int W, int Hp, int Wp, int top,
                          const float* mean3, const float* std3, void* stream);
diff --git a/stereo_toolbox_amd/_capi.py b/stereo_toolbox_amd/_capi.py
--- a/stereo_toolbox_amd/_capi.py
+++ b/stereo_toolbox_amd/_capi.py
@@ -47,6 +47,10 @@
     "stx_conv3d_c1_wgrad_workspace_floats": [_I],
     "stx_conv3d_c1_wgrad": [_P, _P, _P, _P, _I, _I, _I, _I, _I, _P],
     "stx_conv3d_c1_dgrad": [_P, _P, _P, _I, _I, _I, _I, _I, _P],
+    "stx_conv3d_dgrad_bnsums_rows": [_I, _I, _I, _I, _I],
+    "stx_conv3d_dgrad_bnsums": [_P] * 8 + [_I, _P, _I, _I, _I, _I, _I, _P],
+    "stx_conv3d_c1_dgrad_bnsums_rows": [_I, _I, _I, _I, _I],
+    "stx_conv3d_c1_dgrad_bnsums": [_P] * 8 + [_I, _P, _I, _I, _I, _I, _I, _P],
     "stx_mish_fwd": [_P, _P, _L, _P],
     "stx_mish_bwd": [_P, _P, _P, _L, _P],
     "stx_depth_to_space": [_P, _P, _I, _I, _I, _I, _I, _I, _P],
@@ -111,6 +115,7 @@
     "stx_bn_bwd_apply": [_P, _P, _P, _P, _P, _P, _P, _P, _P, _P, _P, _P, _P, _P, _L, _I, _I, _P],
     "stx_bn_bwd_reduce2": [_P] * 14 + [_L, _I, _I, _I, _P],
     "stx_bn_bwd_apply2": [_P] * 18 + [_L, _I, _I, _I, _P],
+    "stx_bn_colsum": [_P, _I, _I, _P, _P],
 }
 _RET_CHARP = ("stx_last_error", "stx_build_info")
 
diff --git a/stereo_toolbox_amd/csrc/bn.hip b/stereo_toolbox_amd/csrc/bn.hip
--- a/stereo_toolbox_amd/csrc/bn.hip
+++ b/stereo_toolbox_amd/csrc/bn.hip
@@ -433,6 +433,13 @@
     return stx_check_launch("bn_colsum");
 }
 
+extern "C" int stx_bn_colsum(const float* partials, int nrows, int M, float* sums, void* stream) {
+    stx_begin();
+    STX_REQUIRE(partials && sums && nrows > 0 && M > 0, "bn_colsum: bad args");
+    hipLaunchKernelGGL(bn_colsum_kernel, dim3(M), dim3(BN_THREADS), 0, (hipStream_t)stream, partials, nrows, M, sums, 1);
+    return stx_check_launch("bn_colsum");
+}
+
 extern "C" int stx_bn_bwd_apply2(const float* gy, const float* y, const float* z1, const float* mean1,
                                  const float* invstd1, const float* gamma1, const float* z2, const float* mean2,
                                  const float* invstd2, const float* gamma2, const float* scale1, const float* shift1,
diff --git a/stereo_toolbox_amd/csrc/conv3d.hip b/stereo_toolbox_amd/csrc/conv3d.hip
--- a/stereo_toolbox_amd/csrc/conv3d.hip
+++ b/stereo_toolbox_amd/csrc/conv3d.hip
@@ -466,6 +466,8 @@
     int os, oo, ncout;
     int wq_total, wq_off, wnt_total, wnt_off;
     const float* acc_in;
+    const float* bn_z; const float* bn_scale; const float* bn_shift; const float* bn_mean; const float* bn_invstd;
+    int bn_act;
 };
 
 constexpr int MW2_MW = 16, MW2_R = 2, MW2_TH = 8, MW2_EH = 10, MW2_EW = 18, MW2_VS = 36;
@@ -536,11 +538,16 @@
     };
 
     float s1 = 0.f, s2 = 0.f;
+    constexpr bool BNS = EPI == 6 || EPI == 7;
+    constexpr bool RAW = EPI == 4 || EPI == 5 || BNS, WHOLE = EPI == 5 || EPI == 7;
+    float t1 = 0.f, t2 = 0.f;
     const int abase = ((th * MW2_R + i / MW2_MW) * MW2_EW + i % MW2_MW) * MW2_VS + 4 * half;
     const float* wlane = wl + lane * 4;
     const int n = i;
-    const float sc = (a.scale && n < ma.ncout) ? a.scale[ma.oo + n] : 1.f;
-    const float bs = (a.bias && n < ma.ncout) ? a.bias[ma.oo + n] : 0.f;
+    const float sc = BNS ? ma.bn_scale[n] : ((a.scale && n < ma.ncout) ? a.scale[ma.oo + n] : 1.f);
+    const float bs = BNS ? ma.bn_shift[n] : ((a.bias && n < ma.ncout) ? a.bias[ma.oo + n] : 0.f);
+    const float bmu = BNS ? ma.bn_mean[n] : 0.f, bis = BNS ? ma.bn_invstd[n] : 0.f;
+    const bool bn_masked = BNS && ma.bn_act != 0;
 
     auto emit_row = [&](const f32x16& done0, const f32x16& done1, const f32x16& done, int r, int dprev) {
         const int row = (r & 3) + 8 * (r >> 2) + 4 * half;
@@ -563,25 +570,32 @@
 #pragma unroll
         for (int r = 0; r < 16; ++r) {
             const int c = (r & 3) + 8 * ((r >> 2) & 1), dh = r >> 3;
-            accp[r] = stx_buf_ld1(rs, ((vmask >> r) & 1u) ? ovoff : STX_BUF_OOB, (unsigned)((dh * a.Wo + c) * ma.os * 4));
+            accp[r] = stx_buf_ld1(rs, (WHOLE || ((vmask >> r) & 1u)) ? ovoff : STX_BUF_OOB, (unsigned)((dh * a.Wo + c) * ma.os * 4));
         }
     };
     auto emit_row_plain = [&](const f32x16& done0, const f32x16& done1, const f32x16& done, int r, unsigned vmask,
                               const stx_bufrsrc& ors) {
         const int c = (r & 3) + 8 * ((r >> 2) & 1), dh = r >> 3;
-        const bool ok = EPI == 5 ? vmask != 0u : (bool)((vmask >> r) & 1u);
+        const bool ok = WHOLE ? vmask != 0u : (bool)((vmask >> r) & 1u);
         float v = BS ? (done0[r] + done1[r]) + done[r] : done[r];
         if (EPI == 2) v += accp[r];
         v = ok ? v : 0.f;
-        s1 += v;
-        s2 = fmaf(v, v, s2);
-        if (EPI != 4 && EPI != 5) {
+        if (BNS) {
+            const float zv = accp[r];
+            const float gm = (!bn_masked || fmaf(zv, sc, bs) > 0.f) ? v : 0.f;
+            t1 += gm;
+            t2 = fmaf(gm, (zv - bmu) * bis, t2);
+        } else {
+            s1 += v;
+            s2 = fmaf(v, v, s2);
+        }
+        if (!RAW) {
             v = fmaf(v, sc, bs);
             if (EPI == 3) v += accp[r];
             const float vr = fmaxf(v, 0.f);
             v = relu_on ? vr : v;
         }
-        stx_buf_st1(ors, (EPI == 5 || ok) ? ovoff : STX_BUF_OOB, (unsigned)((dh * a.Wo + c) * ma.os * 4), v);
+        stx_buf_st1(ors, (WHOLE || ok) ? ovoff : STX_BUF_OOB, (unsigned)((dh * a.Wo + c) * ma.os * 4), v);
     };
 
     auto tap_plane = [&](const float* pbuf, int kd, f32x16& acc, bool fresh, bool with_epi, const f32x16& done0, const f32x16& done1,
@@ -637,6 +651,9 @@
         if (EPI == 3)
             load_partials(vmask, stx_make_rsrc(a.residual + ((size_t)b * a.Do + (st_on ? p - 1 : 0)) * a.Ho * a.Wo * ma.os,
                                                st_on ? oplane_bytes : 0u));
+        if (BNS)
+            load_partials(vmask, stx_make_rsrc(ma.bn_z + ((size_t)b * a.Do + (st_on ? p - 1 : 0)) * a.Ho * a.Wo * ma.os,
+                                               st_on ? oplane_bytes : 0u));
         if (live && vOld) tap_plane(pbuf, 2, pC, BS != 0, false, pA, pB, pC, 0, -1, 0u, ors);
         else if (BS) pC = zero16();
         if (stage) store_plane(nbuf);
@@ -658,6 +675,7 @@
                 else emit_row(pA, pB, pC, r, p - 1);
             }
         }
+        if (BNS) { s1 += t1; s2 += t2; t1 = 0.f; t2 = 0.f; }
     };
 
     __syncthreads();
@@ -1146,6 +1164,8 @@
     case 3: return bs ? conv3d_marchw_kernel<1, 3> : conv3d_marchw_kernel<0, 3>;
     case 4: return bs ? conv3d_marchw_kernel<1, 4> : conv3d_marchw_kernel<0, 4>;
     case 5: return bs ? conv3d_marchw_kernel<1, 5> : conv3d_marchw_kernel<0, 5>;
+    case 6: return bs ? conv3d_marchw_kernel<1, 6> : conv3d_marchw_kernel<0, 6>;
+    case 7: return bs ? conv3d_marchw_kernel<1, 7> : conv3d_marchw_kernel<0, 7>;
     default: return bs ? conv3d_marchw_kernel<1, 1> : conv3d_marchw_kernel<0, 1>;
     }
 }
@@ -1240,10 +1260,11 @@
     return conv_plan(B, Di, Hi, Wi, Cin, Cout, ks, stride).rows;
 }
 
-extern "C" int stx_conv3d_fwd(const float* x, const float* wp, float* out, const float* scale, const float* bias,
-                              const float* residual, float* stats, int B, int Di, int Hi, int Wi, int Cin, int Cout,
-                              int ks, int stride, int relu, void* stream) {
-    stx_begin();
+struct ConvBnSums { const float* z; const float* scale; const float* shift; const float* mean; const float* invstd; int act; };
+
+static int conv3d_fwd_impl(const float* x, const float* wp, float* out, const float* scale, const float* bias,
+                           const float* residual, float* stats, int B, int Di, int Hi, int Wi, int Cin, int Cout,
+                           int ks, int stride, int relu, const ConvBnSums* bn, void* stream) {
     STX_REQUIRE(x && wp && out && B > 0 && Di > 0 && Hi > 0 && Wi > 0, "conv3d_fwd: bad shape");
     STX_REQUIRE(Cin % 8 == 0 && Cout >= 1 && Cout <= 128, "conv3d_fwd: Cin=%d (need %%8) Cout=%d (need <=128)", Cin, Cout);
     STX_REQUIRE((ks == 3 && (stride == 1 || stride == 2)) || (ks == 1 && stride == 1),
@@ -1259,9 +1280,12 @@
     const int NT = conv_nt(Cout);
     hipStream_t st = (hipStream_t)stream;
     const ConvPlan plan = conv_plan(B, Di, Hi, Wi, Cin, Cout, ks, stride);
+    STX_REQUIRE(!bn || plan.kind == 0, "conv3d_dgrad_bnsums: shape not served by the march kernel");
     if (plan.kind == 0) {
         MarchArgs m2;
         m2.c = a;
+        m2.bn_z = bn ? bn->z : nullptr; m2.bn_scale = bn ? bn->scale : nullptr; m2.bn_shift = bn ? bn->shift : nullptr;
+        m2.bn_mean = bn ? bn->mean : nullptr; m2.bn_invstd = bn ? bn->invstd : nullptr; m2.bn_act = bn ? bn->act : 0;
         m2.c.nHt = stx_cdiv(a.Ho, MW2_TH);
         m2.c.nWt = stx_cdiv(a.Wo, MW2_MW);
         m2.ncols = B * m2.c.nHt * m2.c.nWt;
@@ -1284,7 +1308,8 @@
                     }
                     const bool plain = epi_fast && !(m.c.residual && m.acc_in) && m.c.relu < 2;
                     const bool raw = !m.acc_in && !m.c.residual && !m.c.scale && !m.c.bias && m.c.relu == 0;
-                    const int epi = plain ? (raw ? (whole && m.ncout == 32 ? 5 : 4) : m.acc_in ? 2 : (m.c.residual ? 3 : 0)) : 1;
+                    const int epi = bn ? (whole ? 7 : 6)
+                                       : plain ? (raw ? (whole && m.ncout == 32 ? 5 : 4) : m.acc_in ? 2 : (m.c.residual ? 3 : 0)) : 1;
                     if (int rc = launch_with_lds(march_kernel(bs, epi), dim3(nb2), lds2, st, m)) return rc;
                 }
             return stx_check_launch("conv3d_fwd(march)");
@@ -1316,6 +1341,32 @@
     else rc = conv_dispatch<1, 1>(a, NT, CK, grid, st);
     if (rc) return rc;
     return stx_check_launch("conv3d_fwd");
+}
+
+extern "C" int stx_conv3d_fwd(const float* x, const float* wp, float* out, const float* scale, const float* bias,
+                              const float* residual, float* stats, int B, int Di, int Hi, int Wi, int Cin, int Cout,
+                              int ks, int stride, int relu, void* stream) {
+    stx_begin();
+    return conv3d_fwd_impl(x, wp, out, scale, bias, residual, stats, B, Di, Hi, Wi, Cin, Cout, ks, stride, relu, nullptr, stream);
+}
+
+extern "C" int stx_conv3d_dgrad_bnsums_rows(int B, int D, int H, int W, int C) {
+    stx_begin();
+    if (B < 1 || D < 1 || H < 1 || W < 1 || C != 32) return 0;
+    const ConvPlan p = conv_plan(B, D, H, W, 32, 32, 3, 1);
+    return p.kind == 0 ? (int)p.rows : 0;
+}
+
+extern "C" int stx_conv3d_dgrad_bnsums(const float* gy, const float* wp, float* gx, const float* z, const float* scale,
+                                       const float* shift, const float* mean, const float* invstd, int act, float* rows,
+                                       int B, int D, int H, int W, int C, void* stream) {
+    stx_begin();
+    STX_REQUIRE(z && scale && shift && mean && invstd && rows, "conv3d_dgrad_bnsums: null operand");
+    STX_REQUIRE(act == 0 || act == 1, "conv3d_dgrad_bnsums: activation code %d (0 or 1)", act);
+    STX_REQUIRE(stx_conv3d_dgrad_bnsums_rows(B, D, H, W, C) > 0, "conv3d_dgrad_bnsums: shape %d x %d x %d x %d x %d not served",
+                B, D, H, W, C);
+    const ConvBnSums bn{z, scale, shift, mean, invstd, act};
+    return conv3d_fwd_impl(gy, wp, gx, nullptr, nullptr, nullptr, rows, B, D, H, W, 32, 32, 3, 1, 0, &bn, stream);
 }
 
 extern "C" int stx_deconv3d_fwd(const float* x, const float* wp, float* out, const float* scale, const float* bias,
diff --git a/stereo_toolbox_amd/csrc/conv_c1.hip b/stereo_toolbox_amd/csrc/conv_c1.hip
--- a/stereo_toolbox_amd/csrc/conv_c1.hip
+++ b/stereo_toolbox_amd/csrc/conv_c1.hip
@@ -262,6 +262,101 @@
 }
 
 
+struct C1BnSums {
+    const float* z;
+    const float* scale;
+    const float* shift;
+    const float* mean;
+    const float* invstd;
+    float* rows;
+    int act;
+};
+
+__global__ __launch_bounds__(C1_THREADS) void conv_c1_dgrad_mfma_bnsums_kernel(const float* __restrict__ gy,
+                                                                               const float* __restrict__ w,
+                                                                               float* __restrict__ gx, int B, int D, int H, int W,
+                                                                               int nHt, int nWt, int ntiles, C1BnSums bn) {
+    __shared__ float gys[3 * C1D_EH * C1D_EW];
+    const int tid = threadIdx.x, lane = tid & 63, wave = tid >> 6;
+    const int i = lane & 31, half = lane >> 5;
+    float wreg[14];
+    int aoff[14];
+#pragma unroll
+    for (int j = 0; j < 14; ++j) {
+        const int tap = 2 * j + half;
+        const int tp = tap < 27 ? tap : 26;
+        const int kd = tp / 9, kh = (tp / 3) % 3, kw = tp % 3;
+        wreg[j] = tap < 27 ? w[(size_t)i * 27 + tap] : 0.f;
+        aoff[j] = ((2 - kd) * C1D_EH + (wave + 2 - kh)) * C1D_EW + i + 2 - kw;
+    }
+    const unsigned plane_bytes = (unsigned)H * (unsigned)W * 128u;
+    const float bsc = bn.scale[i], bsh = bn.shift[i], bmu = bn.mean[i], bis = bn.invstd[i];
+    const bool masked = bn.act != 0;
+    float s1 = 0.f, s2 = 0.f;
+    for (int tile = blockIdx.x; tile < ntiles; tile += gridDim.x) {
+        int r_ = tile;
+        const int wt = r_ % nWt; r_ /= nWt;
+        const int ht = r_ % nHt; r_ /= nHt;
+        const int d = r_ % D;
+        const int b = r_ / D;
+        const int h0 = ht * C1D_TH, w0 = wt * C1D_TW;
+        float zv[16];
+        {
+            const int ohz = h0 + wave;
+            const unsigned zb = ohz < H ? (unsigned)(((ohz * W + w0 + 4 * half) * 32 + i) * 4) : STX_BUF_OOB;
+            const stx_bufrsrc zrs = stx_make_rsrc(bn.z + ((size_t)b * D + d) * H * W * 32, plane_bytes);
+#pragma unroll
+            for (int r = 0; r < 16; ++r) zv[r] = stx_buf_ld1(zrs, zb + (unsigned)(((r & 3) + 8 * (r >> 2)) * 128), 0u);
+        }
+        __syncthreads();
+        for (int idx = tid; idx < 3 * C1D_EH * C1D_EW; idx += C1_THREADS) {
+            const int wx = idx % C1D_EW, hy = (idx / C1D_EW) % C1D_EH, dz = idx / (C1D_EW * C1D_EH);
+            const int gd = d - 1 + dz, gh = h0 - 1 + hy, gw = w0 - 1 + wx;
+            gys[idx] = (gd >= 0 && gd < D && gh >= 0 && gh < H && gw >= 0 && gw < W)
+                           ? gy[(((size_t)b * D + gd) * H + gh) * W + gw] : 0.f;
+        }
+        __syncthreads();
+        f32x16 acc;
+#pragma unroll
+        for (int r = 0; r < 16; ++r) acc[r] = 0.f;
+        float av[14];
+#pragma unroll
+        for (int j = 0; j < 14; ++j) av[j] = gys[aoff[j]];
+#pragma unroll
+        for (int j = 0; j < 14; ++j) acc = __builtin_amdgcn_mfma_f32_32x32x2f32(av[j], wreg[j], acc, 0, 0, 0);
+        const int oh = h0 + wave;
+        const stx_bufrsrc ors = stx_make_rsrc(gx + ((size_t)b * D + d) * H * W * 32, plane_bytes);
+        const unsigned vbase = (unsigned)((((oh < H ? oh : 0) * W + w0 + 4 * half) * 32 + i) * 4);
+#pragma unroll
+        for (int r = 0; r < 16; ++r) {
+            const int m = (r & 3) + 8 * (r >> 2);
+            const bool ok = oh < H && w0 + 4 * half + m < W;
+            stx_buf_st1(ors, ok ? vbase : STX_BUF_OOB, (unsigned)(m * 128), acc[r]);
+        }
+        float t1 = 0.f, t2 = 0.f;
+#pragma unroll
+        for (int r = 0; r < 16; ++r) {
+            const int m = (r & 3) + 8 * (r >> 2);
+            const bool on = oh < H && w0 + 4 * half + m < W && (!masked || fmaf(zv[r], bsc, bsh) > 0.f);
+            const float gm = on ? acc[r] : 0.f;
+            t1 += gm;
+            t2 = fmaf(gm, (zv[r] - bmu) * bis, t2);
+        }
+        s1 += t1;
+        s2 += t2;
+    }
+    __shared__ float red[4][2][32];
+    s1 += __shfl_xor(s1, 32);
+    s2 += __shfl_xor(s2, 32);
+    if (lane < 32) { red[wave][0][lane] = s1; red[wave][1][lane] = s2; }
+    __syncthreads();
+    if (tid < 64) {
+        const int k = tid >> 5, c = tid & 31;
+        bn.rows[(size_t)blockIdx.x * 64 + tid] = (red[0][k][c] + red[1][k][c]) + (red[2][k][c] + red[3][k][c]);
+    }
+}
+
+
 constexpr int C1M_TD = 2, C1M_TH = 8, C1M_TW = 32;
 constexpr int C1M_ED = C1M_TD + 2, C1M_EH = C1M_TH + 2, C1M_EW = C1M_TW + 2;
 constexpr int C1M_BLOCKS = 1024;
@@ -524,6 +619,8 @@
     return stx_check_launch("conv3d_c1_colsum");
 }
 
+static long long c1_dgrad_mfma_grid(long long nt) { return nt < 256 * 8 ? nt : 256 * 8; }
+
 extern "C" int stx_conv3d_c1_dgrad(const float* gy, const float* w, float* gx, int B, int D, int H, int W, int Cin,
                                    void* stream) {
     stx_begin();
@@ -532,7 +629,7 @@
     const int nHt = stx_cdiv(H, C1D_TH), nWt = stx_cdiv(W, C1D_TW);
     const long long nt = (long long)B * D * nHt * nWt;
     if (Cin == 32 && (long long)H * W * 128 < (1ll << 31) && nt < (1ll << 31)) {
-        const long long g = nt < 256 * 8 ? nt : 256 * 8;
+        const long long g = c1_dgrad_mfma_grid(nt);
         hipLaunchKernelGGL(conv_c1_dgrad_mfma_kernel, dim3((unsigned)g), dim3(C1_THREADS), 0, (hipStream_t)stream, gy, w, gx, B, D,
                            H, W, nHt, nWt, (int)nt);
         return stx_check_launch("conv3d_c1_dgrad(mfma)");
@@ -541,3 +638,27 @@
                        (hipStream_t)stream, gy, w, gx, B, D, H, W, Cin, nHt, nWt);
     return stx_check_launch("conv3d_c1_dgrad");
 }
+
+extern "C" int stx_conv3d_c1_dgrad_bnsums_rows(int B, int D, int H, int W, int Cin) {
+    stx_begin();
+    if (B < 1 || D < 1 || H < 1 || W < 1 || Cin != 32 || (long long)H * W * 128 >= (1ll << 31)) return 0;
+    const long long nt = (long long)B * D * stx_cdiv(H, C1D_TH) * stx_cdiv(W, C1D_TW);
+    return nt < (1ll << 31) ? (int)c1_dgrad_mfma_grid(nt) : 0;
+}
+
+extern "C" int stx_conv3d_c1_dgrad_bnsums(const float* gy, const float* w, float* gx, const float* z, const float* scale,
+                                          const float* shift, const float* mean, const float* invstd, int act, float* rows,
+                                          int B, int D, int H, int W, int Cin, void* stream) {
+    stx_begin();
+    STX_REQUIRE(gy && w && gx && z && scale && shift && mean && invstd && rows, "conv3d_c1_dgrad_bnsums: null operand");
+    STX_REQUIRE(act == 0 || act == 1, "conv3d_c1_dgrad_bnsums: activation code %d (0 or 1)", act);
+    const int g = stx_conv3d_c1_dgrad_bnsums_rows(B, D, H, W, Cin);
+    STX_REQUIRE(g > 0, "conv3d_c1_dgrad_bnsums: shape %d x %d x %d x %d x %d not served", B, D, H, W, Cin);
+    const int nHt = stx_cdiv(H, C1D_TH), nWt = stx_cdiv(W, C1D_TW);
+    const long long nt = (long long)B * D * nHt * nWt;
+    C1BnSums bn;
+    bn.z = z; bn.scale = scale; bn.shift = shift; bn.mean = mean; bn.invstd = invstd; bn.rows = rows; bn.act = act;
+    hipLaunchKernelGGL(conv_c1_dgrad_mfma_bnsums_kernel, dim3((unsigned)g), dim3(C1_THREADS), 0, (hipStream_t)stream, gy, w, gx,
+                       B, D, H, W, nHt, nWt, (int)nt, bn);
+    return stx_check_launch("conv3d_c1_dgrad_bnsums");
+}
diff --git a/stereo_toolbox_amd/ops.py b/stereo_toolbox_amd/ops.py
--- a/stereo_toolbox_amd/ops.py
+++ b/stereo_toolbox_amd/ops.py
@@ -1,4 +1,6 @@
 import ctypes
+import os
+import weakref
 
 import torch
 
@@ -273,11 +275,13 @@
 
 
 def bn_defer_reset_if_stale():
-    if not _BN_DEFER["armed"]:
+    if not _BN_DEFER["armed"] and not _DGRAD_SUMS_FILLED:
         return
     task_id = getattr(torch._C, "_current_graph_task_id", None)
     if task_id is None or task_id() == -1:
         _BN_DEFER["outstanding"], _BN_DEFER["armed"] = 0, False
+        while _DGRAD_SUMS_FILLED:
+            _DGRAD_SUMS_FILLED.pop().clear()
 
 
 def _take_pending_bn(g):
@@ -290,6 +294,69 @@
     return pend
 
 
+class _DgradBnSums:
+    __slots__ = ("bn", "act", "taken", "void", "gx", "gx_version", "rows")
+
+    def __init__(self, bn_ctx, act):
+        self.bn, self.act = weakref.ref(bn_ctx), int(act)
+        self.taken = self.void = False
+        self.gx = self.gx_version = self.rows = None
+
+    def take(self):
+        if self.taken:
+            self.void = True
+            return False
+        self.taken = True
+        return True
+
+    def operands(self):
+        ctx = None if self.void else self.bn()
+        if ctx is None:
+            return None
+        try:
+            z1, _, m1, i1, _, _, _, _, _, sc1, sh1, _, _ = ctx.saved_tensors
+        except RuntimeError:
+            return None
+        if sc1 is None:
+            sc1 = sh1 = m1
+        return z1, sc1, sh1, m1, i1
+
+    def fill(self, gx, rows):
+        self.gx, self.gx_version, self.rows = gx, gx._version, rows
+        _DGRAD_SUMS_FILLED.append(self)
+
+    def usable(self, gy):
+        g = self.gx
+        if self.void or g is None or self.rows is None or gy is None:
+            return False
+        return (gy.device == g.device and gy.dtype == g.dtype and gy.shape == g.shape and gy.stride() == g.stride()
+                and gy.storage_offset() == g.storage_offset()
+                and gy.untyped_storage().data_ptr() == g.untyped_storage().data_ptr() and gy._version == self.gx_version)
+
+    def clear(self):
+        self.gx = self.gx_version = self.rows = None
+        if self in _DGRAD_SUMS_FILLED:
+            _DGRAD_SUMS_FILLED.remove(self)
+
+
+_DGRAD_SUMS_FILLED = []
+
+
+def bn_sums_in_dgrad_enabled():
+    return os.environ.get("STX_BN_SUMS_IN_DGRAD", "1") != "0"
+
+
+def _dgrad_bnsums_rows(w, ks, stride, transposed, x):
+    if transposed or ks != 3 or stride != 1 or x.dim() != 5 or x.shape[-1] != 32 or w.shape[1] != 32:
+        return 0
+    B, D, H, W, _ = x.shape
+    if _is_c1(w, ks, stride, transposed):
+        return get_lib().raw("stx_conv3d_c1_dgrad_bnsums_rows")(B, D, H, W, 32)
+    if w.shape[0] == 32:
+        return get_lib().raw("stx_conv3d_dgrad_bnsums_rows")(B, D, H, W, 32)
+    return 0
+
+
 def _is_c1(w, ks, stride, transposed):
     return (not transposed) and ks == 3 and stride == 1 and w.shape[0] == 1 and w.shape[1] % 16 == 0 and w.shape[1] <= 64
 
@@ -311,10 +378,29 @@
     return dw
 
 
-def conv3d_c1_dgrad(gy, w, Cin):
+def conv3d_c1_dgrad(gy, w, Cin, rec=None, bn=None):
     B, D, H, W, _ = gy.shape
     gx = torch.empty(B, D, H, W, Cin, dtype=torch.float32, device=gy.device)
+    if rec is not None:
+        z, scale, shift, mean, invstd = bn
+        rows = torch.empty(get_lib().raw("stx_conv3d_c1_dgrad_bnsums_rows")(B, D, H, W, Cin), 2, Cin, dtype=torch.float32,
+                           device=gy.device)
+        _call("stx_conv3d_c1_dgrad_bnsums", _p(gy), _p(w), _p(gx), _p(z), _p(scale), _p(shift), _p(mean), _p(invstd), rec.act,
+              _p(rows), B, D, H, W, Cin)
+        rec.fill(gx, rows)
+        return gx
     _call("stx_conv3d_c1_dgrad", _p(gy), _p(w), _p(gx), B, D, H, W, Cin)
+    return gx
+
+
+def conv3d_dgrad_bnsums(gy, wp, rec, bn):
+    B, D, H, W, C = gy.shape
+    z, scale, shift, mean, invstd = bn
+    gx = torch.empty_like(gy)
+    rows = torch.empty(get_lib().raw("stx_conv3d_dgrad_bnsums_rows")(B, D, H, W, C), 2, C, dtype=torch.float32, device=gy.device)
+    _call("stx_conv3d_dgrad_bnsums", _p(gy), _p(wp), _p(gx), _p(z), _p(scale), _p(shift), _p(mean), _p(invstd), rec.act,
+          _p(rows), B, D, H, W, C)
+    rec.fill(gx, rows)
     return gx
 
 
@@ -325,6 +411,8 @@
         _chk(x, "x", 5)
         ctx.cin_true = None
         ctx.x_prepadded = False
+        rec = getattr(x, "_stx_dgrad_bnsums", None)
+        ctx.dgrad_sums = rec if (rec is not None and rec.take() and _dgrad_bnsums_rows(w, ks, stride, transposed, x) > 0) else None
         if not transposed and x.shape[-1] != w.shape[1]:
             if x.shape[-1] != (w.shape[1] + 7) // 8 * 8:
                 raise StxError(f"conv: input has {x.shape[-1]} channels, weight expects {w.shape[1]}")
@@ -382,9 +470,15 @@
                 gz_k = _pad_channels(gz, Cp)
                 w_k = w.new_zeros(Cp, *w.shape[1:])
                 w_k[:Co] = w
+            rec = ctx.dgrad_sums
+            bn = rec.operands() if rec is not None else None
+            if bn is None:
+                rec = None
             if ctx.needs_input_grad[0]:
                 if c1:
-                    gx = conv3d_c1_dgrad(gz, w.contiguous(), Ci)
+                    gx = conv3d_c1_dgrad(gz, w.contiguous(), Ci, rec, bn)
+                elif rec is not None:
+                    gx = conv3d_dgrad_bnsums(gz_k, pack_weight(w_k, 1), rec, bn)
                 elif stride == 1 and Ci > 128:
                     parts = []
                     for lo in range(0, Ci, 128):
@@ -427,6 +521,10 @@
         for (ks, stride, want), w in zip(cfgs, ws):
             if x.shape[-1] != w.shape[1] or w.shape[1] % 8 or w.shape[0] % 8 or _is_c1(w, ks, stride, False):
                 raise StxError(f"SharedInputConvsFn: weight {tuple(w.shape)} on an input of {x.shape[-1]} channels")
+            rec = getattr(x, "_stx_dgrad_bnsums", None)
+            if rec is not None:
+                rec.take()
+                rec.void = True
             z, stats = conv3d_forward(x, pack_weight(w, 0), w.shape[0], ks, stride, want_stats=want)
             if stats is None:
                 stats = x.new_empty(0)
@@ -796,6 +894,10 @@
         ctx.train2 = bn2["training"] if two else False
         ctx.sync = bn1.get("sync") or (bn2.get("sync") if two else None)
         ctx.remask = bool(relu) and residual is None
+        ctx.dgrad_sums = None
+        if (not two and residual is None and G == 1 and ctx.train1 and not ctx.sync and relu in (0, 1) and z1.dim() == 5
+                and z1.shape[-1] % 32 == 0 and bn_sums_in_dgrad_enabled()):
+            ctx.dgrad_sums = y._stx_dgrad_bnsums = _DgradBnSums(ctx, relu)
         keep_y = y if (relu and not ctx.remask) else None
         ctx.save_for_backward(z1, gamma1, m1, i1, z2, gamma2, m2, i2, keep_y, sc1 if ctx.remask else None,
                               sh1 if ctx.remask else None, sc2 if (ctx.remask and two) else None,
@@ -805,6 +907,10 @@
     @staticmethod
     def backward(ctx, gy):
         z1, gamma1, m1, i1, z2, gamma2, m2, i2, y, sc1, sh1, sc2, sh2 = ctx.saved_tensors
+        rec = ctx.dgrad_sums
+        rows = rec.rows if (rec is not None and rec.usable(gy)) else None
+        if rec is not None:
+            rec.clear()
         gy = gy.contiguous()
         G = ctx.groups
         C = z1.shape[-1]
@@ -814,9 +920,12 @@
         part = _WS.get("bnred", G * NB * 3 * C, z1.device)
         sums_all = torch.empty(G + (1 if G > 1 else 0), 3, C, dtype=torch.float32, device=z1.device)
         sums = sums_all[:G]
-        _call("stx_bn_bwd_reduce2", _p(gy), _p(y), _p(z1), _p(m1), _p(i1), _p(z2) if ctx.two else None,
-              _p(m2) if ctx.two else None, _p(i2) if ctx.two else None, _p(sc1), _p(sh1), _p(sc2), _p(sh2), _p(part),
-              _p(sums_all), nvox, C, int(ctx.relu), G)
+        if rows is not None:
+            _call("stx_bn_colsum", _p(rows), rows.shape[0], 2 * C, _p(sums_all))
+        else:
+            _call("stx_bn_bwd_reduce2", _p(gy), _p(y), _p(z1), _p(m1), _p(i1), _p(z2) if ctx.two else None,
+                  _p(m2) if ctx.two else None, _p(i2) if ctx.two else None, _p(sc1), _p(sh1), _p(sc2), _p(sh2), _p(part),
+                  _p(sums_all), nvox, C, int(ctx.relu), G)
         if not ctx.needs_input_grad[0] and not ctx.two and not ctx.has_res:
             tot = sums_all[G] if G > 1 else sums_all[0]
             return (None, tot[1], tot[0], None, None, None, None, None, None, None, None, None)
```

Result: no change. 0.1784 pairs/s (+0.0%).
